# CMB-BNU/PloidyFrost

Hardware: AMD Instinct MI355X
Metric: unitigs/s through superbubble+SeqAlign (k=25, z=8) (higher is better)
Workload: dtype u64

## Files before the change

### include/ploidyfrost_hip.h

```cpp
#ifndef PLOIDYFROST_HIP_H_
#define PLOIDYFROST_HIP_H_

#include <stddef.h>
#include <stdint.h>

#ifdef __cplusplus
extern "C" {
#endif

#define PF_NONE 0xFFFFFFFFu

enum pf_status {
    PF_OK = 0,
    PF_ERR_ARG = 1,
    PF_ERR_HIP = 2,
    PF_ERR_NO_DEVICE = 3,
    PF_ERR_OVERFLOW = 4,
    PF_ERR_MISSING_KMER = 5
};

typedef struct pf_ctx pf_ctx;

int pf_create(int device, pf_ctx **out);
int pf_warmup(int device);
// ... 190 lines not shown
                                uint64_t bytes_used[2], pf_trim_stats trim_stats[2], pf_count_stats *stats, uint64_t *bad_record);
int pf_maskcount_fastq_trimmed(pf_ctx *, const char *text, uint64_t n_bytes, int final, const pf_trim_plan *plan, uint32_t low, uint32_t up,
                               uint64_t *bytes_used, pf_trim_stats *trim_stats, pf_maskcount_stats *stats, uint64_t *bad_record);
int pf_maskcount_fastq_pair_trimmed(pf_ctx *, const char *text1, uint64_t n1, const char *text2, uint64_t n2, int final, const pf_trim_plan *plan,
                                    uint32_t low, uint32_t up, uint64_t bytes_used[2], pf_trim_stats trim_stats[2], pf_maskcount_stats *stats,
                                    uint64_t *bad_record);
typedef struct pf_clip_stats {
    uint64_t reads_clipped[2];
    uint64_t reads_dropped[2];
    uint64_t bases_clipped[2];
    uint64_t candidates_scored[2];
} pf_clip_stats;
int pf_clip_begin(pf_ctx *, const char *bases, const uint32_t *adapter_off, const uint8_t *side, uint32_t n_adapters, uint32_t seed, uint32_t score);
int pf_clip_stats_get(pf_ctx *, pf_clip_stats *stats);
int pf_clip_last_ends(pf_ctx *, int file, uint32_t *clip_end, uint64_t n_records);
int pf_clip_end(pf_ctx *);
typedef struct pf_clip_pair_stats {
    uint64_t pairs_clipped;
    uint64_t pairs_dropped;
    uint64_t pairs_too_long;
    uint64_t candidates_scored;
    uint64_t bases_clipped[2];
} pf_clip_pair_stats;
int pf_clip_begin_pairs(pf_ctx *, const char *bases, const uint32_t *adapter_off, const uint8_t *side, uint32_t n_adapters ,
                        const char *prefix_bases, const uint32_t *prefix_off , uint32_t n_pairs,
                        uint32_t seed, uint32_t score, uint32_t pair_score, uint32_t pair_min, int keep_both);
int pf_clip_pair_stats_get(pf_ctx *, pf_clip_pair_stats *stats);
#define PF_QC_TABLE_WORDS 9515u
#define PF_QC_CLIP_WORDS 1025u
enum { PF_QC_RAW = 0, PF_QC_KEPT = 1 };
int pf_qc_begin(pf_ctx *, uint32_t phred);
int pf_qc_get(pf_ctx *, int side, int stage, uint64_t *words);
int pf_qc_clip_get(pf_ctx *, int side, uint64_t *words);
int pf_qc_fastq(pf_ctx *, int side, const char *text, uint64_t n_bytes, int final, uint64_t *bytes_used, uint64_t *n_records, uint64_t *bad_record);
int pf_qc_end(pf_ctx *);
typedef struct pf_inflate_stats {
    uint64_t members, bytes_in, bytes_out, blocks_stored, blocks_fixed, blocks_dynamic;
} pf_inflate_stats;
int pf_inflate_bgzf(pf_ctx *, const uint8_t *comp, uint64_t n_bytes, const uint64_t *member_off, uint64_t n_members,
                    char *out, uint64_t out_cap, uint64_t *out_bytes, pf_inflate_stats *stats, uint64_t *bad_member);

typedef struct pf_deflate_stats { uint64_t members, bytes_in, bytes_out, blocks_stored, blocks_fixed, blocks_dynamic, literals, matches; } pf_deflate_stats;
int pf_deflate_bgzf(pf_ctx *, const char *text, uint64_t n_bytes, uint32_t member_text, uint8_t *out, uint64_t out_cap,
                    uint64_t *out_bytes, uint64_t *member_off, pf_deflate_stats *stats);

typedef struct pf_gunzip_result {
    uint64_t out_bytes;
    uint64_t end_bit;
    uint32_t final;
    uint32_t n_window;
    uint32_t crc_raw;
    uint32_t clause;
    uint64_t clause_bit;
} pf_gunzip_result;
typedef struct pf_gunzip_stats {
    uint64_t pieces_found, pieces_live, pieces_dead, markers, blocks_stored, blocks_fixed, blocks_dynamic, bytes_in, bytes_out;
    double stage_ms[5];
} pf_gunzip_stats;
int pf_inflate_gzip(pf_ctx *, const uint8_t *comp, uint64_t n_bytes, uint64_t start_bit, const uint8_t *window, uint32_t n_window,
                    uint32_t piece_bytes, char *out, uint64_t out_cap, uint8_t *new_window, pf_gunzip_result *res, pf_gunzip_stats *stats);

typedef struct pf_hetpair_stats {
    uint64_t kmers;
    uint64_t in_range;
    uint64_t one_partner;
    uint64_t many_partners;
    uint64_t pairs;
} pf_hetpair_stats;
int pf_hetpairs(pf_ctx *, const uint64_t *kmers, const uint32_t *counts, uint64_t n, uint32_t k, uint32_t lo, uint32_t hi,
                uint64_t *table, uint64_t **pair_x_dev, uint64_t **pair_y_dev, uint32_t **cov_x_dev, uint32_t **cov_y_dev,
                uint64_t *n_pairs, pf_hetpair_stats *stats);
int pf_hetpair_table(pf_ctx *, const uint32_t *cov_x_dev, const uint32_t *cov_y_dev, uint64_t n_pairs, uint32_t lo, uint32_t hi, uint64_t *table);

int pf_copy_to_host(pf_ctx *, void *dst, const void *src_dev, size_t bytes);
int pf_device_alloc(pf_ctx *, size_t bytes, void **out);
int pf_copy(pf_ctx *, void *dst, const void *src, size_t bytes);

int pf_upload_counts(pf_ctx *, const uint64_t *kmers, const uint32_t *counts, uint64_t n, uint32_t k, uint64_t min_count,
                     uint64_t max_count, int both_strands);
int pf_release_counts(pf_ctx *);
int pf_join_counts(pf_ctx *);
int pf_join_counts_begin(pf_ctx *);
int pf_join_counts_end(pf_ctx *);
int pf_lookup_kmers(pf_ctx *, const uint64_t *kmers, uint64_t n, uint32_t *counts, uint8_t *found);

int pf_unitig_cov(pf_ctx *, uint32_t u0, uint32_t u1, uint64_t *sum, uint32_t *min, uint8_t *miss);
int pf_unitig_cov_probe(pf_ctx *, uint32_t u0, uint32_t u1, uint64_t *sum, uint32_t *min, uint8_t *miss);
int pf_unitig_cov_exact(pf_ctx *, uint32_t u0, uint32_t u1, int reverse, uint64_t *sum, uint32_t *min, uint8_t *miss);

typedef struct pf_bfs_record {
    uint32_t entrance;
    uint32_t exit;
    uint32_t n_seen;
    uint32_t n_list;
    uint64_t list_off;
    uint8_t outcome;
    uint8_t flag_cycle;
    uint8_t flag_tip;
    uint8_t strict;
    uint32_t pad_;
} pf_bfs_record;

enum pf_bfs_outcome {
    PF_BFS_NONE = 0,
    PF_BFS_CYCLE_EXIT = 1,
    PF_BFS_REJECT = 2,
    PF_BFS_ACCEPT = 3
};

int pf_count_candidates(pf_ctx *, uint32_t u0, uint32_t u1, uint64_t *n_candidates);
int pf_bfs_candidates(pf_ctx *, uint32_t u0, uint32_t u1, pf_bfs_record *records, uint64_t rec_cap,
                      uint32_t *pool, uint64_t pool_cap, uint64_t *n_records, uint64_t *pool_used);
int pf_bfs_candidates_split(pf_ctx *, uint32_t u0, uint32_t u1, pf_bfs_record *records, uint64_t rec_cap, uint32_t *pool,
                            uint64_t pool_cap, uint64_t *n_records, uint64_t *pool_used, uint32_t *deferred, uint64_t deferred_cap,
                            uint64_t *n_deferred);
int pf_bfs_candidates_begin(pf_ctx *, uint32_t u0, uint32_t u1, pf_bfs_record *records, uint64_t rec_cap, uint32_t *pool, uint64_t pool_cap,
                            uint64_t *n_records, uint64_t *pool_used, uint32_t *deferred, uint32_t *deferred_entrance, uint64_t deferred_cap,
                            uint64_t *n_deferred);
int pf_bfs_candidates_end(pf_ctx *);

typedef struct pf_align_job {
    uint64_t a_off, b_off;
    uint32_t a_len, b_len;
} pf_align_job;

typedef struct pf_align_hit {
    uint64_t text_off;
    uint64_t gap_off;
    uint32_t len;
    uint32_t n_gaps;
    int64_t score;
    uint32_t n_pos;
    uint32_t n_indel;
} pf_align_hit;

int pf_align_batch(pf_ctx *, const char *text, uint64_t text_len, const pf_align_job *jobs, uint32_t n_jobs,
                   double match, double mismatch, double gap, uint64_t *hit_first, uint32_t *hit_count,
                   pf_align_hit *hits, uint64_t hit_cap, char *out_text, uint64_t text_cap, uint32_t *out_gaps,
                   uint64_t gap_cap, uint64_t used[3]);

typedef struct pf_bubble_path {
    uint64_t text_off;
    uint32_t len;
    uint32_t ov;
} pf_bubble_path;

typedef struct pf_bubble_task {
    uint64_t path_first;
    uint32_t n_paths;
    uint32_t pad_;
} pf_bubble_task;

typedef struct pf_bubble_site {
    uint32_t col;
    uint8_t is_indel;
    uint8_t maxnum;
    uint16_t pad_;
} pf_bubble_site;

typedef struct pf_bubble_result {
    uint64_t rows_off;
    uint64_t site_off;
    uint64_t group_off;
    uint64_t ilen_off;
    uint32_t n_rows;
    uint32_t n_cols;
// ... 178 lines not shown
```

### ploidyfrost_amd/csrc/host/pf_cdbg.hpp

```cpp
#pragma once
#include <chrono>
#include <memory>
#include <condition_variable>
#include <mutex>

#include "pf_bfs_host.hpp"
#include <cstdint>
#include <memory>
#include <string>
#include <thread>
#include <utility>
#include <vector>

#include "pf_gmm_model.hpp"
#include "pf_host_colors.hpp"
#include "pf_host_graph.hpp"
#include "pf_pinned.hpp"
#include "pf_replay_par.hpp"
#include "pf_state.hpp"
#include "ploidyfrost_hip.h"

namespace pfh {

struct Scoring {
// ... 97 lines not shown
    bool model_was_each_color() const { return last_each_; }
    const std::vector<GmmModel::Fit> &model_fits() const { return model_fits_; }
    double model_ploidy() const { return model_ploidy_; }
    const std::string &model_last_line() const { return model_last_line_; }
    uint64_t model_count() const { return model_n_; }
    uint64_t text_bytes_fetched() const { return text_fetched_; }
    int find_shard(uint32_t u0, uint32_t u1);
    const std::vector<pf_bfs_record> &shard_records() const { return shard_rec_; }
    const std::vector<uint32_t> &shard_pool() const { return shard_pool_; }
    int find_replay(const std::string &outpre, uint32_t n_shards, const pf_bfs_record *const *records, const uint64_t *n_records,
                    const uint32_t *const *pools, bool write_file, const uint64_t *pool_lens = nullptr,
                    const pf_bfs_record *const *dev_records = nullptr, const uint32_t *const *dev_pools = nullptr);
    void set_replay_threads(int t) { replay_threads_ = t; }
    void set_write_super_bubble(bool on) { write_sb_ = on; }
    int ploidy_select(int lower, int upper, uint64_t &n_bubbles);
    int ploidy_select(const std::vector<std::pair<int, int>> &cutoff, uint64_t &n_bubbles);
    int ploidy_align(uint64_t t0, uint64_t t1, uint64_t &n_called);
    int ploidy_text(uint64_t var_count_base, uint64_t sizes[PF_CALL_STREAMS], uint64_t counters[8]);
    int ploidy_write(const std::string &outpre, const uint64_t offsets[PF_CALL_STREAMS], const uint64_t totals[PF_CALL_STREAMS], bool truncate);
    pf_ctx *device() { return ctx_; }
    const PhaseTimes &times() const { return times_; }
    uint64_t allele_sites(int arity) const { return allele_[arity - 2]; }
    uint64_t core_cov() const { return core_cov_; }
    uint64_t core_num() const { return core_num_; }
    uint64_t n_superbubbles() const { return n_super_bubble_; }
    const std::vector<uint8_t> &state_flags() { sync_state_to_host(); return flags_; }
    const std::vector<uint32_t> &state_plus() { sync_state_to_host(); return plus_; }
    const std::vector<uint32_t> &state_minus() { sync_state_to_host(); return minus_; }
    int sync_state_to_host();
    uint64_t output_bytes() const { return out_bytes_; }
    const std::string &last_allele_frequency() const;

protected:
    struct NoCounts {};
    CDBG(UnitigSet &graph, const size_t &complexsize, double &m, double &d, double &g, int device, bool quiet, NoCounts, pf_ctx *adopt = nullptr);
    int init_device(int device, pf_ctx *adopt = nullptr, bool colored = false);
    void start_prealloc();
    int ploidy_estimation(const std::string &outpre, const std::vector<std::pair<int, int>> &cutoff, const size_t &thr);
    int ploidy_estimation_resident(const std::string &outpre, const std::vector<std::pair<int, int>> &cutoff, const size_t &thr);
    int call_select(const std::vector<std::pair<int, int>> &cutoff, uint64_t &n_tasks);
    bool resident_path() const { return resident_ && (col_ == nullptr || colored_resident_); }
    const ColorSets *col_ = nullptr;
    const char *tag_ = "CDBG";

    struct Task;
    using clk_time = std::chrono::steady_clock::time_point;
    int finish_find(const std::string &outpre, const FindTrace &tr, bool write_file, bool timing_lines);
    std::vector<pf_bfs_record> shard_rec_;
    std::vector<uint32_t> shard_pool_;
    ModelOptions model_;
    unsigned density_points_ = 0;
    double density_adjust_ = 1.0;
    Density density_;
    bool density_done_ = false;
    std::vector<int> color_no_density_;
    bool filter_on_ = false;
    pf_filter_opts filter_ = {};
    bool multi_on_ = false, multi_each_ = false;
    pf_filter_multi_opts multi_ = {};
    std::vector<ColorFit> color_fits_;
    std::vector<int> color_none_, color_empty_;
    std::vector<double> pooled_values_;
    bool last_each_ = false;
    std::vector<GmmModel::Fit> model_fits_;
    double model_ploidy_ = 0;
    std::string model_last_line_;
    uint64_t model_n_ = 0, text_fetched_ = 0;
    pf_call_result slice_res_ = {};
    uint64_t slice_nb_ = 0, slice_var_base_ = 0;
    int fail(int st, const std::string &msg);
    int join_pending_write();
    int join_pending_ids();
    std::thread prealloc_, prealloc_walkers_, prealloc_call_, prealloc_align_;
    void join_prealloc() {
        if (prealloc_.joinable()) prealloc_.join();
        if (prealloc_walkers_.joinable()) prealloc_walkers_.join();
        if (prealloc_call_.joinable()) prealloc_call_.join();
        if (prealloc_align_.joinable()) prealloc_align_.join();
    }
    std::thread pending_ids_;
    int pending_ids_rc_ = 0;
    uint64_t ids_bytes_ = 0;
    int launch_coverage();
    uint64_t find_passes_ = 0;
    bool cov_ready_ = false;
    std::string cov_err_;
    bool overlap_output_ = false;
    std::thread pending_write_;
    int pending_rc_ = 0;
    int ensure_dir();
    int write_file(const std::string &name, const std::string &data);
    int write_pieces(const std::string &name, const std::vector<const std::string *> &pieces, uint64_t &bytes) const;
    int write_many(const std::vector<std::pair<std::string, std::vector<const std::string *>>> &files, unsigned threads);
    void replay(const pf_bfs_record &r, const uint32_t *list) { st_.replay(r, list); }

    UnitigSet &g_;
    size_t complex_size_;
    Scoring sc_;
    std::string outdir_ = "PloidyFrost_output";
    pf_ctx *ctx_ = nullptr;
    int status_ = 0;
    std::string err_;
    bool quiet_ = false, write_files_ = true;
    bool both_strands_ = true;
    unsigned threads_ = 0;
    int replay_threads_ = -1;
    bool write_sb_ = true;
    bool state_host_stale_ = false;
    bool colours_on_device_ = false;
    bool colored_resident_ = false;
    std::vector<uint8_t> big_f2_;
    bool commits_on_device() const;
    ParallelReplay par_;
    unsigned replay_threads(size_t thr) const;
    size_t host_threads(size_t thr) const;
    unsigned walk_threads(size_t thr) const;
    void set_record_stats(const ReplayStats &s);
    struct EarlyWalks; struct DeviceFind; struct SlicedFind;
    int find_superbubbles_device(const std::string &outpre, const size_t &thr);
    int traverse_resident(EarlyWalks &early, DeviceFind &df, const FindTrace &tr);
    void walk_remaining(EarlyWalks &early, DeviceFind &df, const FindTrace &tr, unsigned threads);
    void walked_into_candidate_order(DeviceFind &df);
    int commit_large_on_host(DeviceFind &df, const FindTrace &tr, unsigned threads);
    int patch_device_state(const std::vector<uint32_t> &sides, const FindTrace &tr, unsigned threads);
    void traverse_slices(SlicedFind &sf, const FindTrace &tr);
    int traverse_slice(SlicedFind &sf, int i, const FindTrace &tr);
    void walk_long(const FindTrace &tr, bool say_start, uint32_t entrance, pf_bfs_record &r, std::vector<uint32_t> &out);
    template <class Call> int with_deferred(uint64_t &n_deferred, Call call);
    template <class ListOf> void replay_sequential(const pf_bfs_record *rec, uint64_t n, ListOf list_of, ReplayStats &stats);
    bool third_tier_on_host_ = true;
    WalkerPool walkers_;
    std::vector<uint32_t> deferred_;
    std::vector<uint32_t> deferred_ent_;
    std::vector<std::vector<uint32_t>> huge_lists_[4];

    std::vector<uint32_t> succ_, pred_;
    UnitigState st_;
    std::vector<uint8_t> &flags_ = st_.flags;
    std::vector<uint32_t> &plus_ = st_.plus, &minus_ = st_.minus;

    struct AlignExchange {
        PinnedBuf<char> text, otext;
        PinnedBuf<pf_bubble_path> paths;
        PinnedBuf<pf_bubble_task> tasks;
        PinnedBuf<pf_bubble_result> res;
        PinnedBuf<pf_bubble_site> osites;
        PinnedBuf<uint8_t> ogroups;
        PinnedBuf<uint32_t> oilen;
        void release_all() {
            text.release(); otext.release(); paths.release(); tasks.release(); res.release(); osites.release();
            ogroups.release(); oilen.release();
        }
    } ax_[3];
    size_t batch_bubbles_ = 32768, align_pieces_ = 64;
    struct BubbleExchange {
        PinnedBuf<pf_bfs_record> bfs_rec;
        PinnedBuf<uint32_t> bfs_pool;
        PinnedBuf<uint32_t> bfs_order;
        PinnedBuf<uint64_t> cov_sum;
        PinnedBuf<uint32_t> cov_min;
        PinnedBuf<uint8_t> cov_miss;
        PinnedBuf<uint32_t> cov_max;
        void release_all() {
            cov_max.release();
            bfs_rec.release(); bfs_pool.release(); bfs_order.release(); cov_sum.release(); cov_min.release();
            cov_miss.release();
// ... 65 lines not shown
```

### ploidyfrost_amd/csrc/host/pf_cdbg_call.cpp

```cpp
#include <fcntl.h>
#include <sys/stat.h>
#include <unistd.h>

#include <algorithm>
#include <atomic>
#include <condition_variable>
#include <cstdio>
#include <cstring>
#include <ctime>
#include <deque>
#include <memory>
#include <mutex>
#include <sstream>
#include <thread>

#include "../pf_alnpack.hpp"
#include "../pf_nibble.hpp"
#include "pf_cdbg_impl.hpp"
#include "pf_parallel.hpp"

namespace pfh {

namespace {
const char *kStreamSuffix[PF_CALL_STREAMS] = {"_allele_frequency.txt", "_alignseq.txt", "_bifre.txt",    "_trifre.txt",   "_tetrafre.txt",
// ... 136 lines not shown
    std::vector<pf_call_result> pres((size_t)n_pieces);
    uint64_t running[PF_CALL_STREAMS];
    for (int s = 0; s < PF_CALL_STREAMS; ++s) running[s] = offsets[s];
    last_allfre_.clear();
    last_allfre_file_.clear();
    int st = PF_OK;
    auto format = [&](uint64_t i) {
        const uint64_t first = i * CHUNK, count = std::min<uint64_t>(CHUNK, slice_nb_ - first);
        return pf_call_text_range_lane(ctx_, 0, (int)(i % PF_CALL_SLABS), first, count, slice_var_base_, &pres[(size_t)i]);
    };
    auto piece_bytes = [&](uint64_t i) {
        uint64_t all = 0;
        for (int s = 0; s < PF_CALL_STREAMS; ++s) all += pres[(size_t)i].text_len[s];
        return all;
    };
    auto fetch = [&](uint64_t i) {
        PinnedBuf<char> &hb = cx_.slab[i & 1];
        const uint64_t all = piece_bytes(i);
        hb.ensure(ctx_, std::max<uint64_t>(all, 1));
        return pf_call_fetch_range(ctx_, (int)(i % PF_CALL_SLABS), 0, hb.p, all, (int)(i & 1));
    };
    if (n_pieces) st = format(0);
    if (st == PF_OK && n_pieces) st = fetch(0);
    for (uint64_t i = 0; i < n_pieces && st == PF_OK; ++i) {
        if (i + 1 < n_pieces) st = format(i + 1);
        if (st == PF_OK) st = pf_call_fetch_wait(ctx_, (int)(i & 1));
        if (st == PF_OK && i + 1 < n_pieces) st = fetch(i + 1);
        if (st != PF_OK) break;
        const pf_call_result &r = pres[(size_t)i];
        const char *src = cx_.slab[i & 1].p;
        CopySpan spans[PF_CALL_STREAMS];
        size_t n_spans = 0;
        uint64_t at = 0;
        for (int s = 0; s < PF_CALL_STREAMS; ++s) {
            const uint64_t len = r.text_len[s];
            if (len) {
                char *dst = maps[s].prepare(running[s], len);
                if (dst) spans[n_spans++] = CopySpan{dst, src + at, len};
                else rc |= maps[s].write(running[s], src + at, len, T);
            }
            if (s == 0) last_allfre_.append(src + at, len);
            running[s] += len;
            at += len;
            out_bytes_ += len;
        }
        copy_spans(spans, n_spans, T);
    }
    if (st != PF_OK) return fail(st, std::string(tag_) + "::PloidyEstimation(): " + pf_last_error(ctx_));
    for (int s = 0; s < PF_CALL_STREAMS; ++s)
        if (running[s] - offsets[s] != (slice_nb_ ? slice_res_.text_len[s] : 0)) return fail(PF_ERR_ARG, std::string(tag_) + "::PloidyEstimation(): the pieces of a slice do not add up to its size");
    times_.write_s = since(t);
    if (rc) return fail(PF_ERR_ARG, "CDBG:: write error on the result files");
    return 0;
}

int CDBG::ploidy_estimation_resident(const std::string &outpre, const std::vector<std::pair<int, int>> &cutoff, const size_t &thr) {
    const auto t_all = clk::now();
    clock_t c0 = clock();
    if (!quiet_) printf("%s::PloidyEstimation():  Analyzing superbubbles to generate sites' information\n", tag_);
    if (write_files_ && ensure_dir()) return status_;
    if (model_.on && ((col_ && !multi_on_) || !write_files_))
        return fail(PF_ERR_ARG, std::string(tag_) + "::PloidyEstimation(): the model in the same run needs the single-sample path (the colored one: a multi filter in front of it, set_filter_multi) and an output directory");
    const bool write_ten = write_files_ && !model_.only;
    model_fits_.clear();
    model_last_line_.clear();
    model_ploidy_ = 0;
    model_n_ = 0;
    color_fits_.clear();
    color_none_.clear();
    color_empty_.clear();
    color_no_density_.clear();
    density_done_ = false;
    pooled_values_.clear();
    last_each_ = false;
    const uint64_t fetched_before = pf_call_fetched_bytes(ctx_);
    const unsigned T = threads_ ? threads_ : (unsigned)std::max<size_t>(thr, 1);
    times_.cov_device_s = times_.tasks_s = times_.align_s = times_.sites_s = times_.format_s = times_.write_s = 0;
    times_.tasks = times_.align_jobs = times_.site_strings = 0;
    times_.snp_jobs = times_.pair_jobs = times_.wave_jobs = times_.stack_jobs = 0;
    times_.align_build_s = times_.align_device_s = times_.align_post_s = times_.align_choose_s = times_.scan_s = 0;
    allele_[0] = allele_[1] = allele_[2] = allele_[3] = 0;
    core_cov_ = core_num_ = 0;
    const bool trace = getenv("PF_TRACE_PLOIDY") != nullptr;
    auto tp = [&](const char *what) { if (trace) fprintf(stderr, "[ploidy] %-28s %.2f ms\n", what, since(t_all) * 1e3); };

    struct OutFile {
        std::string name;
        uint64_t bytes = 0;
        int rc = 0;
    };
    std::vector<OutFile> files(PF_CALL_STREAMS);
    for (int s = 0; s < PF_CALL_STREAMS; ++s) files[(size_t)s].name = outpre + kStreamSuffix[s];
    MappedOut *maps = out_maps_.get();
    int open_failed = -1;
    std::thread opener;
    if (write_ten)
        opener = std::thread([&] {
            for (size_t i = 0; i < files.size(); ++i)
                if (maps[i].open_for(outdir_ + "/" + files[i].name)) { open_failed = (int)i; return; }
        });
    struct OpenerGuard {
        std::thread &t;
        ~OpenerGuard() { if (t.joinable()) t.join(); }
    } opener_guard{opener};

    uint64_t n_tasks = 0;
    if (call_select(cutoff, n_tasks)) return status_;
    tp("scan + selection done");
    if (opener.joinable()) opener.join();
    if (open_failed >= 0) return fail(PF_ERR_ARG, "CDBG:: Open " + files[(size_t)open_failed].name + " file error");
    last_allfre_.clear();
    last_allfre_file_.clear();
    std::thread prefault0;
    std::atomic<bool> prefault0_stop{false};
    struct Prefault0Guard {
        std::thread &t;
        std::atomic<bool> &stop;
        ~Prefault0Guard() { stop.store(true); if (t.joinable()) t.join(); }
    } prefault0_guard{prefault0, prefault0_stop};
    if (write_ten && n_tasks) {
        const double nbub = 1.1 * (double)n_tasks;
        const double per_bubble[PF_CALL_STREAMS] = {20, 2.0 * (2 * g_.k + 26), 20, 0.5, 0.25, 0, 34, 0.75, 0.25, 0};
        std::vector<std::pair<int, uint64_t>> fresh;
        for (int s = 0; s < PF_CALL_STREAMS; ++s) {
            const uint64_t est = (uint64_t)(per_bubble[s] * nbub);
            if (est >= (1u << 20) && maps[s].reserve(est) == 0) fresh.push_back({s, est});
        }
        if (!fresh.empty())
            prefault0 = std::thread([maps, fresh, T, &prefault0_stop] {
                constexpr uint64_t STEP = 4u << 20;
                std::vector<std::pair<int, uint64_t>> spans;
                uint64_t longest = 0;
                for (auto &f : fresh) longest = std::max(longest, f.second);
                for (uint64_t at = 0; at < longest; at += STEP)
                    for (auto &f : fresh)
                        if (at < f.second) spans.push_back({f.first, at});
                parallel_chunks(spans.size(), 1, std::max(2u, T), [&](size_t i, size_t, size_t) {
                    if (prefault0_stop.load(std::memory_order_relaxed)) return;
                    const int s = spans[i].first;
                    uint64_t end = spans[i].second + STEP;
                    for (auto &f : fresh) if (f.first == s) end = std::min(end, f.second);
                    maps[s].populate(spans[i].second, end);
                });
            });
    }

    const bool aln_packed = !getenv("PF_ALIGNSEQ_ASCII");
    if (pf_call_set_alignseq_packed(ctx_, aln_packed ? 1 : 0) != PF_OK) return fail(PF_ERR_HIP, std::string(tag_) + "::PloidyEstimation(): " + pf_last_error(ctx_));
    const bool num_packed = !getenv("PF_NUMERIC_ASCII");
    if (pf_call_set_numeric_packed(ctx_, num_packed ? 1 : 0) != PF_OK) return fail(PF_ERR_HIP, std::string(tag_) + "::PloidyEstimation(): " + pf_last_error(ctx_));
    if (model_.on && (pf_call_model_begin(ctx_, model_.source, model_.q) != PF_OK || (filter_on_ && pf_call_model_filter(ctx_, &filter_) != PF_OK) ||
                      (multi_on_ && pf_call_model_filter_multi(ctx_, &multi_, multi_each_ ? 1 : 0) != PF_OK)))
        return fail(PF_ERR_ARG, std::string(tag_) + "::PloidyEstimation(): " + pf_last_error(ctx_));
    struct PackGuard {
        pf_ctx *c;
        ~PackGuard() { (void)pf_call_set_alignseq_packed(c, 0); (void)pf_call_set_numeric_packed(c, 0); }
    } pack_guard{ctx_};
    auto slab_len = [](const pf_call_result &r, int s) -> uint64_t {
        const uint64_t aln = (s == PF_OUT_ALIGNSEQ && r.alignseq_packed_len) ? r.alignseq_packed_len : r.text_len[s];
        if (!r.numeric_packed) return aln;
        return s == PF_OUT_ALIGNSEQ ? ((aln + 15) & ~15ull) : PF_NUMERIC_PACKED_LEN(r.text_len[s]);
    };

    const size_t batch_env = [] { const char *e = getenv("PF_BATCH_BUBBLES"); return e ? (size_t)std::max(1, atoi(e)) : (size_t)0; }();
    const size_t batch_now = batch_env ? batch_env : batch_bubbles_;
    const size_t CHUNK = std::min<size_t>(std::max<size_t>(batch_now ? batch_now * 4 : 1, 1), (size_t)1 << 24);
    struct Done {
// ... 470 lines not shown
```

### ploidyfrost_amd/csrc/host/pf_cdbg_find.cpp

```cpp
#include <algorithm>
#include <atomic>
#include <condition_variable>
#include <cstdio>
#include <cstring>
#include <mutex>
#include <stdexcept>
#include <thread>
#include <unordered_map>

#include "pf_cdbg_impl.hpp"
#include "pf_parallel.hpp"

namespace pfh {

size_t CDBG::host_threads(size_t thr) const { return threads_ ? threads_ : std::max<size_t>(thr, 1); }
unsigned CDBG::walk_threads(size_t thr) const {
    return (unsigned)std::max<uint64_t>(1, std::min<uint64_t>(host_threads(thr), (4ull << 30) / (4ull * std::max<uint32_t>(g_.n(), 1))));
}

unsigned CDBG::replay_threads(size_t thr) const {
    if (col_ != nullptr) return 0;
    static const char *env = getenv("PF_REPLAY");
    if (env && !strcmp(env, "seq")) return 0;
    static const int env_t = [] { const char *e = getenv("PF_REPLAY_THREADS"); return e ? atoi(e) : -1; }();
// ... 157 lines not shown
    }
    df.walked.swap(w2);
    std::copy(d2.begin(), d2.end(), deferred_.begin());
}

int CDBG::commit_large_on_host(DeviceFind &df, const FindTrace &tr, unsigned threads) {
    const uint32_t N = g_.n();
    const size_t n_big = (size_t)df.n_big, n_walked = (size_t)df.n_deferred;
    std::vector<uint32_t> big_idx(n_big);
    std::vector<pf_bfs_record> big_rec(n_big);
    std::vector<uint32_t> big_pool((size_t)df.big_entries + 1);
    const int st = pf_replay_big_fetch(ctx_, big_idx.data(), big_rec.data(), big_pool.data());
    if (st != PF_OK) return st;
    tr.step("large components fetched");
    if (big_f2_.size() != 2 * (size_t)N) big_f2_.assign(2 * (size_t)N, 0);
    if (!state_host_stale_)
        parallel_chunks(N, 1u << 19, threads, [&](size_t, size_t b, size_t e) {
            memset(plus_.data() + b, 0, (e - b) * 4);
            memset(minus_.data() + b, 0, (e - b) * 4);
        });
    const FlagsPerSideLogged acc{FlagsPerSide{big_f2_.data(), plus_.data(), minus_.data()}, &df.p_sides};
    Commits<FlagsPerSideLogged> cm{acc, complex_size_, NoColours{}};
    Commits<FlagsPerSideLogged, ColourGate> cmc{acc, complex_size_, col_ ? st_.colour_gate() : ColourGate{}};
    ReplayStats stats;
    auto commit = [&](const pf_bfs_record &r, const uint32_t *list) {
        const bool effective = record_effective(r) && cm.gate_open(r.entrance);
        stats.note(r, effective);
        if (effective) { if (col_) cmc.replay(r, list); else cm.replay(r, list); }
        return effective;
    };
    double t[2] = {0, 0};
    uint64_t eff[2] = {0, 0}, ent[2] = {0, 0};
    size_t a = 0, b = 0;
    while (a < n_big || b < n_walked) {
        const bool w = a >= n_big || (b < n_walked && deferred_[b] < big_idx[a]);
        const auto tc = tr.find ? clk::now() : clk::time_point();
        const pf_bfs_record &r = w ? df.walked[b++] : big_rec[a++];
        if (commit(r, (w ? df.xpool.data() : big_pool.data()) + r.list_off)) { ent[w] += r.n_list; ++eff[w]; }
        if (tr.find) t[w] += since(tc);
    }
    set_record_stats(stats);
    if (tr.find)
        fprintf(stderr, "[find]   replayed here: %zu walked records (%llu take effect, %llu list entries) %.3f ms, %llu records of large components (%llu, %llu) %.3f ms\n",
                n_walked, (unsigned long long)eff[1], (unsigned long long)ent[1], t[1] * 1e3, (unsigned long long)df.n_big, (unsigned long long)eff[0], (unsigned long long)ent[0], t[0] * 1e3);
    tr.step("large components replayed");
    return PF_OK;
}

int CDBG::patch_device_state(const std::vector<uint32_t> &sides, const FindTrace &tr, unsigned threads) {
    std::vector<uint32_t> links(sides.size());
    std::vector<uint8_t> bytes(sides.size());
    parallel_chunks(sides.size(), 1u << 14, threads, [&](size_t, size_t b, size_t e) {
        for (size_t i = b; i < e; ++i) {
            const uint32_t s = sides[i];
            links[i] = (s & 1) ? minus_[s >> 1] : plus_[s >> 1];
            bytes[i] = big_f2_[s];
        }
    });
    tr.step("patch gathered");
    std::thread undo([&] {
        parallel_chunks(sides.size(), 1u << 14, threads, [&](size_t, size_t b, size_t e) {
            for (size_t i = b; i < e; ++i) {
                const uint32_t s = sides[i];
                __atomic_store_n(&((s & 1) ? minus_ : plus_)[s >> 1], 0u, __ATOMIC_RELAXED);
                __atomic_store_n(&big_f2_[s], (uint8_t)0, __ATOMIC_RELAXED);
            }
        });
    });
    const int st = pf_replay_finish(ctx_, sides.data(), links.data(), bytes.data(), sides.size());
    undo.join();
    return st;
}

int CDBG::find_superbubbles_device(const std::string &outpre, const size_t &thr) {
    const FindTrace tr;
    auto failed = [&](int st) { return fail(st, std::string("CDBG::findSuperBubble(): ") + pf_last_error(ctx_)); };
    out_bytes_ = 0;
    state_on_device_ = false;
    cov_ready_ = false;
    for (auto &hl : huge_lists_) hl.clear();
    const unsigned wt = walk_threads(thr), few = (unsigned)std::min<size_t>(host_threads(thr), 8);
    DeviceFind df;
    EarlyWalks early(*this, tr, wt);
    int st = traverse_resident(early, df, tr);
    if (st != PF_OK) return failed(st);
    tr.step("traversed on the device");
    df.walked.resize((size_t)df.n_deferred);
    df.lists.resize((size_t)df.n_deferred);
    std::string walk_err;
    std::thread walk([&] { try { walk_remaining(early, df, tr, wt); } catch (const std::exception &e) { walk_err = e.what(); } });
    st = pf_side_components(ctx_, 1, nullptr, df.n_rec, nullptr, 0, nullptr, 0, nullptr, 0);
    tr.step("  components of the device's records");
    if (st == PF_OK && overlap_output_) cov_ready_ = launch_coverage() == PF_OK;
    tr.step("  coverage launched");
    walk.join();
    if (!walk_err.empty()) return fail(PF_ERR_HIP, "CDBG::findSuperBubble(): walk of a long traversal: " + walk_err);
    if (st != PF_OK) return failed(st);
    tr.step("long traversals walked");
    walked_into_candidate_order(df);
    tr.step("  walked records in candidate order");
    if (!df.walked.empty()) st = pf_side_components(ctx_, 0, nullptr, df.n_rec, nullptr, 0, df.walked.data(), df.walked.size(), df.xpool.data(), df.xpool.size());
    tr.step("  their components");
    static const uint32_t small_limit = [] { const char *e = getenv("PF_REPLAY_SMALL_LIMIT"); return e ? (uint32_t)atoi(e) : 256u; }();
    if (st == PF_OK) st = pf_replay_device(ctx_, (uint32_t)std::min<size_t>(complex_size_, 0xFFFFFFFFu), small_limit, &df.n_big, &df.big_entries);
    if (st != PF_OK) return failed(st);
    tr.step("components + commits on the device");
    st = commit_large_on_host(df, tr, few);
    if (st != PF_OK) return failed(st);
    st = patch_device_state(df.p_sides, tr, few);
    if (st != PF_OK) return failed(st);
    if (tr.find) fprintf(stderr, "[find] %zu sides patched on the device %.2f ms\n", df.p_sides.size(), since(tr.t_all) * 1e3);
    state_host_stale_ = true;
    state_on_device_ = true;
    tr.step("large components committed here");
    times_.bfs_device_s = since(tr.t_all);
    times_.candidates = df.n_rec;
    times_.bfs_deferred = df.n_deferred;
    times_.host_commit_records = df.n_big + df.n_deferred;
    times_.host_walk_vertices = 0;
    for (const auto &w : df.walked) times_.host_walk_vertices += w.n_seen;
    times_.replay_s = 0;
    return finish_find(outpre, tr, write_sb_, true);
}

struct CDBG::SlicedFind {
    static constexpr int kMaxSlices = 4;
    int n_slices = 1;
    unsigned rt = 0, walk_threads = 1;
    uint32_t u0[kMaxSlices + 1];
    uint64_t rec0[kMaxSlices + 1], pool0[kMaxSlices + 1], n_rec[kMaxSlices], used[kMaxSlices];
    uint32_t class_off[kMaxSlices][kReplayClasses + 1];
    std::unique_ptr<PinnedBuf<uint32_t>> own_pool[kMaxSlices];
    const uint32_t *pool[kMaxSlices];
    std::mutex mu; std::condition_variable cv;
    int done = 0, dev_st = PF_OK;
    std::string dev_err;
    double bfs_s = 0;
    uint64_t n_deferred_total = 0;
};

int CDBG::traverse_slice(SlicedFind &sf, int i, const FindTrace &tr) {
    const auto tb = clk::now();
    pf_bfs_record *rec = bx_.bfs_rec.p + sf.rec0[i];
    const uint64_t rec_cap = sf.rec0[i + 1] - sf.rec0[i];
    uint32_t *pl = bx_.bfs_pool.p + sf.pool0[i];
    uint64_t cap = sf.pool0[i + 1] - sf.pool0[i];
    uint64_t n_deferred = 0;
    int st1;
    for (;;) {
        if (third_tier_on_host_)
            st1 = with_deferred(n_deferred, [&] {
                return pf_bfs_candidates_begin(ctx_, sf.u0[i], sf.u0[i + 1], rec, rec_cap, pl, cap, &sf.n_rec[i], &sf.used[i], deferred_.data(), deferred_ent_.data(), deferred_.size(), &n_deferred);
            });
        else
            st1 = pf_bfs_candidates(ctx_, sf.u0[i], sf.u0[i + 1], rec, rec_cap, pl, cap, &sf.n_rec[i], &sf.used[i]);
        if (st1 != PF_ERR_OVERFLOW || sf.used[i] <= cap) break;
        sf.own_pool[i] = std::make_unique<PinnedBuf<uint32_t>>();
        sf.own_pool[i]->ensure(ctx_, sf.used[i] + sf.used[i] / 8);
        pl = sf.own_pool[i]->p;
        cap = sf.own_pool[i]->cap;
    }
    sf.pool[i] = pl;
    sf.n_deferred_total += n_deferred;
    if (tr.bfs) fprintf(stderr, "[bfs] device tiers of slice %d: %.2f ms, %llu candidates left for the third tier\n", i, since(tb) * 1e3, (unsigned long long)n_deferred);
    std::vector<pf_bfs_record> walked((size_t)n_deferred);
    std::string walk_err;
    std::thread walk;
    if (st1 == PF_OK && n_deferred) {
        huge_lists_[i].assign((size_t)n_deferred, std::vector<uint32_t>());
        walk = std::thread([&] {
            try {
                parallel_chunks((size_t)n_deferred, 1, sf.walk_threads, [&](size_t d, size_t, size_t) {
                    walk_long(tr, false, deferred_ent_[d], walked[d], huge_lists_[i][d]);
                    walked[d].list_off = d; walked[d].pad_ = 1;
                });
            } catch (const std::exception &e) { walk_err = e.what(); }
        });
    }
    if (st1 == PF_OK && sf.rt) st1 = pf_side_components(ctx_, i == 0, nullptr, sf.n_rec[i], nullptr, 0, nullptr, 0, nullptr, 0);
    if (walk.joinable()) walk.join();
    if (!walk_err.empty()) throw std::runtime_error("walk of a long traversal: " + walk_err);
    if (third_tier_on_host_) {
        const int ste = pf_bfs_candidates_end(ctx_);
        if (st1 == PF_OK) st1 = ste;
    }
    if (st1 == PF_OK)
        for (uint64_t d = 0; d < n_deferred; ++d) rec[deferred_[d]] = walked[(size_t)d];
    const auto t_cc = clk::now();
    if (tr.find) fprintf(stderr, "[find]   slice %d traversed (%llu records, %llu walked on host cores) %.2f ms (+%.2f)\n", i, (unsigned long long)sf.n_rec[i],
                         (unsigned long long)n_deferred, since(tr.t_all) * 1e3, since(tb) * 1e3);
    if (st1 == PF_OK && sf.rt) {
        std::vector<pf_bfs_record> xrec;
        std::vector<uint32_t> xpool;
        for (uint64_t d = 0; d < n_deferred; ++d) {
            pf_bfs_record r = rec[deferred_[d]];
            const std::vector<uint32_t> &l = huge_lists_[i][(size_t)d];
            r.list_off = xpool.size();
// ... 206 lines not shown
    return 0;
}

int CDBG::find_replay(const std::string &outpre, uint32_t n_shards, const pf_bfs_record *const *records, const uint64_t *n_records,
                      const uint32_t *const *pools, bool write_file, const uint64_t *pool_lens, const pf_bfs_record *const *dev_records,
                      const uint32_t *const *dev_pools) {
    if (status_) return status_;
    if (join_pending_write()) return status_;
    if (write_file && write_files_ && ensure_dir()) return status_;
    const FindTrace tr;
    out_bytes_ = 0;
    state_on_device_ = false;
    state_host_stale_ = false;
    std::fill(flags_.begin(), flags_.end(), 0);
    std::fill(plus_.begin(), plus_.end(), 0);
    std::fill(minus_.begin(), minus_.end(), 0);
    cov_ready_ = false;
    ReplayStats stats;
    set_record_stats(stats);
    const auto t0 = clk::now();
    uint64_t total = 0;
    uint32_t last = 0;
    const unsigned rt = pool_lens ? replay_threads(1) : 0;
    if (rt) par_.begin(g_.n(), plus_.data(), minus_.data(), complex_size_, rt);
    std::vector<uint32_t> order;
    std::vector<const pf_bfs_record *> h_rec(n_shards);
    std::vector<const uint32_t *> h_pool(n_shards);
    {
        uint64_t need_rec = 0, need_pool = 0;
        for (uint32_t sh = 0; sh < n_shards; ++sh) {
            h_rec[sh] = records ? records[sh] : nullptr;
            h_pool[sh] = pools ? pools[sh] : nullptr;
            if (!h_rec[sh] || !h_pool[sh]) {
                if (!pool_lens || !dev_records || !dev_pools || !dev_records[sh] || !dev_pools[sh])
                    return fail(PF_ERR_ARG, "CDBG::find_replay(): a shard has neither host nor device arrays");
                need_rec += n_records[sh];
                need_pool += pool_lens[sh];
            }
        }
        if (need_rec) {
            bx_.bfs_rec.ensure(ctx_, need_rec + 1);
            bx_.bfs_pool.ensure(ctx_, need_pool + 1);
            uint64_t ar = 0, ap = 0;
            for (uint32_t sh = 0; sh < n_shards; ++sh) {
                if (h_rec[sh] && h_pool[sh]) continue;
                int st = pf_fetch(ctx_, bx_.bfs_rec.p + ar, dev_records[sh], n_records[sh] * sizeof(pf_bfs_record));
                if (st == PF_OK) st = pf_fetch(ctx_, bx_.bfs_pool.p + ap, dev_pools[sh], pool_lens[sh] * 4);
                if (st != PF_OK) return fail(st, std::string("CDBG::find_replay(): ") + pf_last_error(ctx_));
                h_rec[sh] = bx_.bfs_rec.p + ar;
                h_pool[sh] = bx_.bfs_pool.p + ap;
                ar += n_records[sh];
                ap += pool_lens[sh];
            }
        }
    }
    for (uint32_t sh = 0; sh < n_shards; ++sh) {
        const pf_bfs_record *rec = h_rec[sh];
        const uint32_t *pool = h_pool[sh];
        const uint64_t n = n_records[sh];
        total += n;
        for (uint64_t i = 0; i < n; ++i) {
            const pf_bfs_record &r = rec[i];
            if ((r.entrance >> 1) >= g_.n() || r.entrance < last) return fail(PF_ERR_ARG, "CDBG::find_replay(): records out of order");
            last = r.entrance;
        }
        auto list_of = [&](const pf_bfs_record &r) { return pool + r.list_off; };
        if (!rt) { replay_sequential(rec, n, list_of, stats); continue; }
        const bool on_dev = dev_records && dev_pools && dev_records[sh] && dev_pools[sh];
        int st = pf_side_components(ctx_, sh == 0, on_dev ? dev_records[sh] : rec, n, on_dev ? dev_pools[sh] : pool, pool_lens[sh], nullptr, 0, nullptr, 0);
        uint32_t class_off[kReplayClasses + 1];
        order.resize(std::max<uint64_t>(n, 1));
        if (st == PF_OK) st = pf_replay_order(ctx_, kReplayClasses, order.data(), class_off, nullptr);
        if (st != PF_OK) return fail(st, std::string("CDBG::find_replay(): ") + pf_last_error(ctx_));
        par_.run(rec, list_of, order.data(), class_off, kReplayClasses, rt, stats);
    }
    if (rt) par_.finish(flags_.data(), rt);
    stats.large_used = stats.large_used_max = 0;
    set_record_stats(stats);
    times_.replay_s = since(t0);
    times_.candidates = total;
    return finish_find(outpre, tr, write_file, false);
}

int CDBG::launch_coverage() {
    if (resident_path()) {
        const int st = pf_call_coverage(ctx_);
        if (st != PF_OK) cov_err_ = pf_last_error(ctx_);
        return st;
    }
    const uint32_t N = g_.n();
    const uint32_t C = col_ ? col_->n_colors : (both_strands_ ? 1 : 2);
    bx_.cov_sum.ensure(ctx_, (size_t)N * C);
    bx_.cov_min.ensure(ctx_, (size_t)N * C);
    bx_.cov_miss.ensure(ctx_, (size_t)N * C);
    if (col_) bx_.cov_max.ensure(ctx_, (size_t)N * C);
    int st;
    if (col_) st = pf_unitig_cov_colored(ctx_, 0, N, bx_.cov_sum.p, bx_.cov_min.p, bx_.cov_max.p, bx_.cov_miss.p);
    else if (both_strands_) st = pf_unitig_cov(ctx_, 0, N, bx_.cov_sum.p, bx_.cov_min.p, bx_.cov_miss.p);
    else {
        st = pf_unitig_cov_exact(ctx_, 0, N, 0, bx_.cov_sum.p, bx_.cov_min.p, bx_.cov_miss.p);
        if (st == PF_OK || st == PF_ERR_MISSING_KMER) st = pf_unitig_cov_exact(ctx_, 0, N, 1, bx_.cov_sum.p + N, bx_.cov_min.p + N, bx_.cov_miss.p + N);
    }
    if (st != PF_OK && st != PF_ERR_MISSING_KMER) { cov_err_ = pf_last_error(ctx_); return st; }
    return PF_OK;
}

}
```

### ploidyfrost_amd/csrc/pf_bfs.hip

```cpp
#include <hip/hip_runtime.h>

#include <algorithm>
#include <cstring>

#include "pf_bfs.hpp"
#include "pf_bfs_huge.hpp"
#include "pf_ctx.hpp"

using namespace pf;


constexpr uint32_t BFS_LDS_CAP = 128;
constexpr uint32_t BFS_BIG_CAP = 1u << 12;

struct BfsOut {
    pf_bfs_record *rec;
    uint32_t *pool;
    uint64_t pool_cap;
    unsigned long long *pool_head;
    uint32_t *deferred;
    unsigned int *n_deferred;
    uint32_t *deferred2;
    unsigned int *n_deferred2;
    unsigned long long *live;
// ... 220 lines not shown
    pf_bfs_record *records; uint64_t rec_cap;
    uint32_t *pool; uint64_t pool_cap;
    uint64_t *n_records, *pool_used;
    uint32_t *deferred, *deferred_entrance; uint64_t deferred_cap, *n_deferred;
};

struct BfsCounters {
    unsigned long long pool_head;
    unsigned int n_deferred;
    unsigned int n_deferred2;
    unsigned int n_wave_list;
    unsigned int n_live;
};

struct BfsPlan {
    uint64_t c0, c1, n;
    BfsOut o;
    BfsCounters *d_cnt; uint32_t *d_wlist;
};

void cand_range(const pf_ctx *ctx, uint32_t u0, uint32_t u1, uint64_t *c0, uint64_t *c1) {
    const auto &v = ctx->h_cand;
    *c0 = std::lower_bound(v.begin(), v.end(), u0 * 2) - v.begin();
    *c1 = std::lower_bound(v.begin(), v.end(), u1 * 2) - v.begin();
}

uint32_t env_hint_at() { const char *e = getenv("PF_BFS_HINT_AT"); return e ? (uint32_t)std::max(9, atoi(e)) : 48u; }
uint32_t env_wave_cap() { const char *e = getenv("PF_BFS_WAVE_CAP"); return e ? (uint32_t)std::max(16, std::min((int)BFS_LDS_CAP, atoi(e))) : BFS_LDS_CAP; }

int want_host_records(pf_ctx *ctx, const void *records, const char *entry_point) {
    if (!ctx || !is_device_ptr(records)) return PF_OK;
    pf::CtxErr{ctx} = std::string(entry_point) + " fills host records";
    return PF_ERR_ARG;
}

void mark_deferred(const pf_ctx *ctx, pf_bfs_record *records, uint64_t c0, const uint32_t *deferred, uint64_t n_deferred) {
    for (uint64_t d = 0; d < n_deferred; ++d) {
        pf_bfs_record &r = records[deferred[d]];
        memset(&r, 0, sizeof r);
        r.entrance = ctx->h_cand[c0 + deferred[d]];
        r.exit = NONE;
    }
}

int bfs_plan(pf_ctx *ctx, const BfsRequest &q, BfsPlan &p) {
    cand_range(ctx, q.u0, q.u1, &p.c0, &p.c1);
    const uint64_t n = p.n = p.c1 - p.c0;
    *q.n_records = n; *q.pool_used = 0;
    if (n > q.rec_cap) { pf::CtxErr{ctx} = "record buffer too small"; return PF_ERR_OVERFLOW; }
    if (n == 0) return PF_OK;
    pf_bfs_record *d_rec = q.records; uint32_t *d_pool = q.pool;
    if (q.mode.deliver != Deliver::ON_DEVICE) {
        d_rec = (pf_bfs_record *)ctx_ws(ctx, WS_BFS_REC, n * sizeof(pf_bfs_record));
        d_pool = (uint32_t *)ctx_ws(ctx, WS_BFS_POOL, (q.pool_cap ? q.pool_cap : 1) * 4);
    }
    BfsCounters *c = p.d_cnt = (BfsCounters *)ctx_ws(ctx, WS_BFS_SMALL, sizeof(BfsCounters));
    uint32_t *d_def = (uint32_t *)ctx_ws(ctx, WS_BFS_DEF, (n * 2 + 8) * 4);
    p.d_wlist = (uint32_t *)ctx_ws(ctx, WS_BFS_WLIST, (n + 8) * 4);
    if (!d_rec || !d_pool || !c || !d_def || !p.d_wlist) return PF_ERR_HIP;
    PF_HIP(hipMemsetAsync(c, 0, sizeof(BfsCounters), ctx->stream));
    p.o = BfsOut{d_rec, d_pool, q.pool_cap, &c->pool_head, d_def, &c->n_deferred, d_def + n + 4, &c->n_deferred2, nullptr, 0, &c->n_live, 0};
    return PF_OK;
}

void bfs_arm_live(pf_ctx *ctx, const BfsRequest &q, BfsPlan &p) {
    ctx->bfs_live_n = 0;
    if (!ctx->h_live || q.mode.long_walks != LongWalks::BY_CALLER) return;
    p.o.live = ctx->h_live; p.o.live_cap = (uint32_t)ctx->live_cap; p.o.hint_at = env_hint_at();
}

int bfs_read_counters(pf_ctx *ctx, const BfsPlan &p, BfsCounters &cnt) {
    PF_HIP(hipMemcpyAsync(&cnt, p.d_cnt, sizeof cnt, hipMemcpyDeviceToHost, ctx->stream));
    PF_HIP(hipStreamSynchronize(ctx->stream));
    return PF_OK;
}

int bfs_short_tiers(pf_ctx *ctx, const BfsPlan &p, BfsCounters &cnt) {
    ctx_begin(ctx, PF_K_BFS_THREAD);
    k_bfs_thread<<<(unsigned)((p.n + 255) / 256), 256, 0, ctx->stream>>>(ctx->d_succ, ctx->d_pred, ctx->d_cand, p.c0, p.c1, p.o, p.d_wlist, &p.d_cnt->n_wave_list);
    ctx_end(ctx);
    ctx_begin(ctx, PF_K_BFS);
    k_bfs<<<ctx_grid(ctx, (p.n / 4 + 64) * 64, 256, 8), 256, 0, ctx->stream>>>(ctx->d_succ, ctx->d_pred, ctx->d_cand, p.c0, p.c1, p.o, p.d_wlist, &p.d_cnt->n_wave_list, env_wave_cap());
    ctx_end(ctx);
    if (const int st = bfs_read_counters(ctx, p, cnt)) return st;
    ctx->bfs_live_n = cnt.n_live;
    ctx_units(ctx, PF_K_BFS, cnt.n_wave_list);
    ctx_units(ctx, PF_K_BFS_THREAD, p.n);
    return PF_OK;
}

int bfs_long_tiers(pf_ctx *ctx, const BfsPlan &p, BfsCounters &cnt) {
    const unsigned int waves = std::min<unsigned int>(cnt.n_deferred, 256);
    DevTmp<uint32_t> sc32; DevTmp<uint8_t> sc8;
    PF_HIP(sc32.alloc((size_t)waves * 3 * BFS_BIG_CAP * 4));
    PF_HIP(sc8.alloc((size_t)waves * BFS_BIG_CAP));
    ctx_begin(ctx, PF_K_BFS_BIG);
    k_bfs_big<<<waves, 64, 0, ctx->stream>>>(ctx->d_succ, ctx->d_pred, ctx->d_cand, p.c0, cnt.n_deferred, sc32.p, sc8.p, p.o);
    ctx_end(ctx);
    const int st = bfs_read_counters(ctx, p, cnt);
    if (st != PF_OK || cnt.n_deferred2 == 0) return st;
    const unsigned int hw = (unsigned int)std::max<size_t>(1, std::min<size_t>(std::min<size_t>(cnt.n_deferred2, 64), (16ull << 30) / (36 * (size_t)ctx->N + 64)));
    const size_t per = 9 * (size_t)ctx->N + 16;
    DevTmp<uint32_t> hs;
    PF_HIP(hs.alloc(per * hw * 4));
    PF_HIP(hipMemsetAsync(hs.p, 0, per * hw * 4, ctx->stream));
    ctx_begin(ctx, PF_K_BFS_BIG);
    if (!ctx->d_pred16) {
        PF_HIP(hipMalloc(&ctx->d_pred16, (size_t)ctx->N * 2 * 16 * 4));
        k_pred16<<<ctx_grid(ctx, (uint64_t)ctx->N * 8, 256, 8), 256, 0, ctx->stream>>>(ctx->d_succ, ctx->d_pred, ctx->N * 2, ctx->d_pred16);
    }
    k_bfs_huge<<<hw, 64, 0, ctx->stream>>>(ctx->d_succ, ctx->d_pred16, ctx->d_cand, p.c0, cnt.n_deferred2, hs.p, ctx->N, p.o);
    ctx_end(ctx);
    return bfs_read_counters(ctx, p, cnt);
}

void bfs_publish(pf_ctx *ctx, const BfsRequest &q, const BfsPlan &p) {
    ctx->bfs_last_rec = p.o.rec; ctx->bfs_last_pool = p.o.pool; ctx->bfs_last_n = p.n; ctx->bfs_last_pool_len = q.pool_cap;
    ctx->bfs_call_id++;
}

int bfs_deliver(pf_ctx *ctx, const BfsRequest &q, const BfsPlan &p, uint64_t pool_used) {
    const uint64_t n_deferred = q.n_deferred ? *q.n_deferred : 0;
    const size_t rec_bytes = p.n * sizeof(pf_bfs_record), pool_bytes = (size_t)pool_used * 4;
    if (q.mode.deliver == Deliver::TO_HOST) {
        PF_HIP(hipMemcpy(q.records, p.o.rec, rec_bytes, hipMemcpyDeviceToHost));
        PF_HIP(hipMemcpy(q.pool, p.o.pool, pool_bytes, hipMemcpyDeviceToHost));
        mark_deferred(ctx, q.records, p.c0, q.deferred, n_deferred);
        if (std::any_of(q.records, q.records + p.n, [](const pf_bfs_record &r) { return r.outcome == BFS_TOO_LARGE; })) {
            pf::CtxErr{ctx} = "a traversal exceeded the direct-indexed tier (internal limit)";
            return PF_ERR_OVERFLOW;
        }
    } else if (q.mode.deliver == Deliver::TO_HOST_ASYNC) {
        if (!ctx->copy_stream) PF_HIP(hipStreamCreateWithFlags(&ctx->copy_stream, hipStreamNonBlocking));
        PF_HIP(hipMemcpyAsync(q.records, p.o.rec, rec_bytes, hipMemcpyDeviceToHost, ctx->copy_stream));
        PF_HIP(hipMemcpyAsync(q.pool, p.o.pool, pool_bytes, hipMemcpyDeviceToHost, ctx->copy_stream));
        ctx->bfs_pending.active = true; ctx->bfs_pending.records = q.records; ctx->bfs_pending.c0 = p.c0;
        ctx->bfs_pending.deferred.assign(q.deferred, q.deferred + n_deferred);
    }
    if (q.deferred_entrance) for (uint64_t d = 0; d < n_deferred; ++d) q.deferred_entrance[d] = ctx->h_cand[p.c0 + q.deferred[d]];
    return PF_OK;
}

int bfs_run(pf_ctx *ctx, const BfsRequest &q) {
    if (!ctx || !ctx->has_adj || q.u0 > q.u1 || q.u1 > ctx->N || !q.records || !q.pool || !q.n_records || !q.pool_used) return PF_ERR_ARG;
    if (ctx->bfs_pending.active) { pf::CtxErr{ctx} = "pf_bfs_candidates_end first"; return PF_ERR_ARG; }
    if (q.n_deferred) *q.n_deferred = 0;
    PF_HIP(hipSetDevice(ctx->device));
    BfsPlan p; BfsCounters cnt;
    int st = bfs_plan(ctx, q, p), status = PF_OK;
    if (st != PF_OK || p.n == 0) return st;
    bfs_arm_live(ctx, q, p);
    if ((st = bfs_short_tiers(ctx, p, cnt)) != PF_OK) return st;
    if (cnt.n_deferred && q.mode.long_walks == LongWalks::BY_CALLER) {
        *q.n_deferred = cnt.n_deferred;
        if (cnt.n_deferred > q.deferred_cap) { pf::CtxErr{ctx} = "deferred-candidate buffer too small"; status = PF_ERR_OVERFLOW; }
        else PF_HIP(hipMemcpy(q.deferred, p.o.deferred, (size_t)cnt.n_deferred * 4, hipMemcpyDeviceToHost));
    } else if (cnt.n_deferred) {
        if ((st = bfs_long_tiers(ctx, p, cnt)) != PF_OK) return st;
    }
    bfs_publish(ctx, q, p);
    *q.pool_used = cnt.pool_head;
    if (cnt.pool_head > q.pool_cap) { pf::CtxErr{ctx} = "vertex pool too small"; status = PF_ERR_OVERFLOW; }
    return status == PF_OK ? bfs_deliver(ctx, q, p, cnt.pool_head) : status;
}

}

extern "C" {

int pf_count_candidates(pf_ctx *ctx, uint32_t u0, uint32_t u1, uint64_t *n) {
    if (!ctx || !ctx->has_adj || u0 > u1 || u1 > ctx->N || !n) return PF_ERR_ARG;
    uint64_t c0, c1;
    cand_range(ctx, u0, u1, &c0, &c1);
    *n = c1 - c0;
    return PF_OK;
}

int pf_bfs_candidates(pf_ctx *ctx, uint32_t u0, uint32_t u1, pf_bfs_record *records, uint64_t rec_cap, uint32_t *pool,
                      uint64_t pool_cap, uint64_t *n_records, uint64_t *pool_used) {
    return bfs_run(ctx, {{is_device_ptr(records) ? Deliver::ON_DEVICE : Deliver::TO_HOST, LongWalks::ON_DEVICE}, u0, u1, records, rec_cap, pool, pool_cap,
                         n_records, pool_used, nullptr, nullptr, 0, nullptr});
}

int pf_bfs_candidates_split(pf_ctx *ctx, uint32_t u0, uint32_t u1, pf_bfs_record *records, uint64_t rec_cap, uint32_t *pool,
                            uint64_t pool_cap, uint64_t *n_records, uint64_t *pool_used, uint32_t *deferred, uint64_t deferred_cap,
                            uint64_t *n_deferred) {
    if (!deferred || !n_deferred) return PF_ERR_ARG;
    if (want_host_records(ctx, records, "pf_bfs_candidates_split")) return PF_ERR_ARG;
    return bfs_run(ctx, {{Deliver::TO_HOST, LongWalks::BY_CALLER}, u0, u1, records, rec_cap, pool, pool_cap, n_records, pool_used,
                         deferred, nullptr, deferred_cap, n_deferred});
}

int pf_bfs_candidates_begin(pf_ctx *ctx, uint32_t u0, uint32_t u1, pf_bfs_record *records, uint64_t rec_cap, uint32_t *pool,
                            uint64_t pool_cap, uint64_t *n_records, uint64_t *pool_used, uint32_t *deferred, uint32_t *deferred_entrance,
                            uint64_t deferred_cap, uint64_t *n_deferred) {
    if (!deferred || !deferred_entrance || !n_deferred) return PF_ERR_ARG;
    if (want_host_records(ctx, records, "pf_bfs_candidates_begin")) return PF_ERR_ARG;
    return bfs_run(ctx, {{Deliver::TO_HOST_ASYNC, LongWalks::BY_CALLER}, u0, u1, records, rec_cap, pool, pool_cap, n_records, pool_used,
                         deferred, deferred_entrance, deferred_cap, n_deferred});
}

int pf_bfs_candidates_end(pf_ctx *ctx) {
    if (!ctx) return PF_ERR_ARG;
    auto &pending = ctx->bfs_pending;
    if (!pending.active) return PF_OK;
    pending.active = false;
    PF_HIP(hipSetDevice(ctx->device));
    PF_HIP(hipStreamSynchronize(ctx->copy_stream));
    mark_deferred(ctx, pending.records, pending.c0, pending.deferred.data(), pending.deferred.size());
    return PF_OK;
}

int pf_bfs_candidates_resident(pf_ctx *ctx, uint32_t u0, uint32_t u1, uint64_t *n_records, uint64_t *pool_used, uint32_t *deferred,
                               uint32_t *deferred_entrance, uint64_t deferred_cap, uint64_t *n_deferred) {
    if (!ctx || !n_records || !pool_used || !deferred || !deferred_entrance || !n_deferred || !ctx->has_adj || u0 > u1 || u1 > ctx->N) return PF_ERR_ARG;
    uint64_t c0, c1;
    cand_range(ctx, u0, u1, &c0, &c1);
    const uint64_t n = c1 - c0;
    uint64_t cap = std::max<uint64_t>(ctx->bfs_res_pool_cap, n * 6 + (1u << 20));
    for (int attempt = 0; attempt < 4; ++attempt) {
        pf_bfs_record *d_rec = (pf_bfs_record *)ctx_ws(ctx, WS_BFS_RES_REC, (n + 1) * sizeof(pf_bfs_record));
        uint32_t *d_pool = (uint32_t *)ctx_ws(ctx, WS_BFS_RES_POOL, (cap + 1) * 4);
        if (!d_rec || !d_pool) return PF_ERR_HIP;
        const int st = bfs_run(ctx, {{Deliver::ON_DEVICE, LongWalks::BY_CALLER}, u0, u1, d_rec, n + 1, d_pool, cap, n_records, pool_used,
                                     deferred, deferred_entrance, deferred_cap, n_deferred});
        if (st == PF_ERR_OVERFLOW && *pool_used > cap) { cap = *pool_used + *pool_used / 8 + 1024; continue; }
        if (st == PF_OK) ctx->bfs_res_pool_cap = cap;
        return st;
    }
    pf::CtxErr{ctx} = "pf_bfs_candidates_resident: the vertex pool does not converge";
    return PF_ERR_OVERFLOW;
}

// ... 26 lines not shown
```

### ploidyfrost_amd/csrc/pf_call.hip

```cpp
#include "pf_call_kernels.hpp"
#include "pf_scan.hpp"

using namespace pf;

#define PF_TRY(call) do { const int s_ = (call); if (s_ != PF_OK) return s_; } while (0)

using namespace pf_call;

struct Need { DevBuf *buf; size_t bytes; };
static int need(pf_ctx *ctx, const char *who, std::initializer_list<Need> list) {
    for (const Need &n : list)
        if (!n.buf->ensure(n.bytes)) { pf::CtxErr{ctx} = std::string(who) + ": out of device memory"; return PF_ERR_HIP; }
    return PF_OK;
}

namespace pf {

void call_state_create(pf_ctx *ctx) { (void)state_of(ctx); }
void call_destroy(pf_ctx *ctx) {
    if (!ctx->call) return;
    ctx->call->release_all();
    delete ctx->call;
    ctx->call = nullptr;
}
// ... 182 lines not shown
    }
    PF_HIP(hipSetDevice(ctx->device));
    CallState *S = ctx->call;
    PF_HIP(hipMemcpyAsync(S->col_low.p, lower, (size_t)n_colors * 4, hipMemcpyDefault, ctx->stream));
    PF_HIP(hipMemcpyAsync(S->col_up.p, upper, (size_t)n_colors * 4, hipMemcpyDefault, ctx->stream));
    PF_HIP(hipStreamSynchronize(ctx->stream));
    return PF_OK;
}

int pf_call_coverage(pf_ctx *ctx) {
    if (ctx && ctx->call && ctx->call->n_colors) {
        if (!ctx->d_seq || !ctx->d_ctab) { pf::CtxErr{ctx} = "pf_call_coverage: graph and count tables first"; return PF_ERR_ARG; }
        PF_HIP(hipSetDevice(ctx->device));
        CallState *S = ctx->call;
        const size_t n = (size_t)ctx->N * S->n_colors;
        if (!S->ccov_sum.ensure(n * 8) || !S->ccov_min.ensure(n * 4) || !S->ccov_max.ensure(n * 4) || !S->ccov_miss.ensure(n)) {
            pf::CtxErr{ctx} = "pf_call_coverage: out of device memory";
            return PF_ERR_HIP;
        }
        const int st = pf_unitig_cov_colored(ctx, 0, ctx->N, S->ccov_sum.as<uint64_t>(), S->ccov_min.as<uint32_t>(), S->ccov_max.as<uint32_t>(), S->ccov_miss.as<uint8_t>());
        if (st != PF_OK) return st;
        S->per_strand = false;
        S->have_cov = true;
        return PF_OK;
    }
    if (!ctx || !ctx->d_seq || !ctx->d_tab) { if (ctx) pf::CtxErr{ctx} = "pf_call_coverage: graph and count table first"; return PF_ERR_ARG; }
    PF_HIP(hipSetDevice(ctx->device));
    CallState *S = state_of(ctx);
    const size_t N = ctx->N;
    const int slots = ctx->tab_exact ? 2 : 1;
    if (!S->cov_sum.ensure(N * slots * 8) || !S->cov_min.ensure(N * slots * 4) || !S->cov_miss.ensure(N * slots)) {
        pf::CtxErr{ctx} = "pf_call_coverage: out of device memory";
        return PF_ERR_HIP;
    }
    int st;
    if (!ctx->tab_exact) {
        st = pf_unitig_cov(ctx, 0, (uint32_t)N, S->cov_sum.as<uint64_t>(), S->cov_min.as<uint32_t>(), S->cov_miss.as<uint8_t>());
    } else {
        st = pf_unitig_cov_exact(ctx, 0, (uint32_t)N, 0, S->cov_sum.as<uint64_t>(), S->cov_min.as<uint32_t>(), S->cov_miss.as<uint8_t>());
        if (st == PF_OK || st == PF_ERR_MISSING_KMER)
            st = pf_unitig_cov_exact(ctx, 0, (uint32_t)N, 1, S->cov_sum.as<uint64_t>() + N, S->cov_min.as<uint32_t>() + N, S->cov_miss.as<uint8_t>() + N);
    }
    if (st != PF_OK && st != PF_ERR_MISSING_KMER) return st;
    S->per_strand = ctx->tab_exact;
    S->have_cov = true;
    return PF_OK;
}

int pf_call_scan(pf_ctx *ctx, uint32_t lower, uint32_t upper, uint64_t *n_sides) {
    if (!ctx || !n_sides) return PF_ERR_ARG;
    CallState *S = ctx->call;
    if (!S || !S->have_state || !S->have_cov) { pf::CtxErr{ctx} = "pf_call_scan: pf_call_set_state and pf_call_coverage first"; return PF_ERR_ARG; }
    PF_HIP(hipSetDevice(ctx->device));
    hipStream_t st = ctx->stream;
    const uint32_t N = ctx->N;
    if (!S->side_cnt.ensure(((size_t)N + 1) * 4) || !S->side_base.ensure(((size_t)N + 1) * 4)) { pf::CtxErr{ctx} = "pf_call_scan: out of device memory"; return PF_ERR_HIP; }
    k_call_count_sides<<<(N + 1 + 255) / 256, 256, 0, st>>>(S->flags.as<uint8_t>(), N, S->side_cnt.as<uint32_t>());
    if (!S->scan_tmp.ensure(scan_scratch_bytes((uint64_t)N + 1))) { pf::CtxErr{ctx} = "pf_call_scan: out of device memory"; return PF_ERR_HIP; }
    PF_HIP(scan_exclusive_u32(S->side_cnt.as<uint32_t>(), S->side_base.as<uint32_t>(), (uint64_t)N + 1, S->scan_tmp.p, st));
    uint32_t total = 0;
    PF_HIP(hipMemcpyAsync(&total, S->side_base.as<uint32_t>() + N, 4, hipMemcpyDeviceToHost, st));
    PF_HIP(hipStreamSynchronize(st));
    S->n_sides = total;
    S->n_tasks = 0;
    S->low = lower;
    S->up = upper;
    *n_sides = total;
    if (total == 0) return PF_OK;
    if (!S->sides.ensure((size_t)total * sizeof(pf_call_side)) || !S->ctask.ensure((size_t)total * sizeof(CallTask)) ||
        !S->target.ensure((size_t)total * 4)) {
        pf::CtxErr{ctx} = "pf_call_scan: out of device memory";
        return PF_ERR_HIP;
    }
    ScanArgs a;
    a.flags = S->flags.as<uint8_t>(); a.plus = S->plus.as<uint32_t>(); a.minus = S->minus.as<uint32_t>();
    a.succ = ctx->d_succ; a.pred = ctx->d_pred; a.seq = ctx->d_seq; a.off = ctx->d_off; a.len = ctx->d_len; a.N = N; a.k = ctx->k;
    a.cov_sum = S->cov_sum.as<uint64_t>(); a.cov_min = S->cov_min.as<uint32_t>(); a.cov_miss = S->cov_miss.as<uint8_t>();
    a.per_strand = S->per_strand; a.low = lower; a.up = upper;
    a.side_base = S->side_base.as<uint32_t>(); a.sides = S->sides.as<pf_call_side>(); a.tasks = S->ctask.as<CallTask>();
    a.target = S->target.as<uint32_t>();
    a.n_colors = S->n_colors;
    a.ccov_sum = S->ccov_sum.as<uint64_t>(); a.ccov_min = S->ccov_min.as<uint32_t>(); a.ccov_max = S->ccov_max.as<uint32_t>(); a.ccov_miss = S->ccov_miss.as<uint8_t>();
    a.clow = S->col_low.as<uint32_t>(); a.cup = S->col_up.as<uint32_t>(); a.full = S->col_full.as<uint64_t>(); a.cwords = S->col_words; a.size_total = S->col_size.as<uint64_t>();
    ctx_begin(ctx, PF_K_CALL_SCAN);
    if (S->n_colors) k_call_sides<true><<<(N + 255) / 256, 256, 0, st>>>(a);
    else k_call_sides<false><<<(N + 255) / 256, 256, 0, st>>>(a);
    ctx_end(ctx);
    ctx_units(ctx, PF_K_CALL_SCAN, N);
    PF_HIP(hipGetLastError());
    return PF_OK;
}

int pf_call_resolve(pf_ctx *ctx, uint64_t *n_bubbles, uint32_t *err, uint32_t *err_unitig) {
    if (!ctx || !ctx->call || !n_bubbles || !err || !err_unitig) return PF_ERR_ARG;
    CallState *S = ctx->call;
    *n_bubbles = 0;
    *err = 0;
    *err_unitig = 0;
    S->n_tasks = 0;
    const uint64_t n = S->n_sides;
    if (n == 0) return PF_OK;
    PF_HIP(hipSetDevice(ctx->device));
    hipStream_t st = ctx->stream;
    if (!S->pending.ensure(n * 4) || !S->killed.ensure(n) || !S->rstate.ensure(n) || !S->rflag.ensure(n * 4) || !S->rsmall.ensure(64) ||
        !S->kept.ensure(n * 4)) {
        pf::CtxErr{ctx} = "pf_call_resolve: out of device memory";
        return PF_ERR_HIP;
    }
    PF_HIP(hipMemsetAsync(S->pending.p, 0, n * 4, st));
    PF_HIP(hipMemsetAsync(S->killed.p, 0, n, st));
    PF_HIP(hipMemsetAsync(S->rstate.p, 0, n, st));
    unsigned int *small = S->rsmall.as<unsigned int>();
    ResolveArgs a;
    a.sides = S->sides.as<pf_call_side>(); a.target = S->target.as<uint32_t>(); a.n = (uint32_t)n; a.pending = S->pending.as<int>();
    a.killed = S->killed.as<uint8_t>(); a.state = S->rstate.as<uint8_t>(); a.flag = S->rflag.as<uint32_t>();
    a.undecided = small; a.first_err = small + 1;
    const unsigned int init[3] = {0, 0xFFFFFFFFu, 0};
    PF_HIP(hipMemcpyAsync(small, init, 12, hipMemcpyHostToDevice, st));
    const unsigned grid = (unsigned)((n + 255) / 256);
    k_call_pending<<<grid, 256, 0, st>>>(a);
    for (uint64_t round = 0;; ++round) {
        if (round > n + 2) { pf::CtxErr{ctx} = "pf_call_resolve: the driver pass does not settle"; return PF_ERR_ARG; }
        k_call_resolve<<<grid, 256, 0, st>>>(a);
        PF_HIP(hipMemsetAsync(small, 0, 4, st));
        k_call_resolve<<<grid, 256, 0, st>>>(a);
        unsigned int h[2];
        PF_HIP(hipMemcpyAsync(h, small, 8, hipMemcpyDeviceToHost, st));
        PF_HIP(hipStreamSynchronize(st));
        if (h[1] != 0xFFFFFFFFu && h[0] == 0) {
            pf_call_side bad;
            PF_HIP(hipMemcpy(&bad, S->sides.as<pf_call_side>() + h[1], sizeof(bad), hipMemcpyDeviceToHost));
            *err = bad.err;
            *err_unitig = bad.err_unitig;
            return PF_OK;
        }
        if (h[0] == 0) break;
    }
    if (!S->scan_tmp.ensure(scan_scratch_bytes(n))) { pf::CtxErr{ctx} = "pf_call_resolve: out of device memory"; return PF_ERR_HIP; }
    PF_HIP(select_flagged_u32(S->rflag.as<uint32_t>(), S->kept.as<uint32_t>(), small + 2, nullptr, n, S->scan_tmp.p, st));
    unsigned int sel = 0;
    PF_HIP(hipMemcpyAsync(&sel, small + 2, 4, hipMemcpyDeviceToHost, st));
    PF_HIP(hipStreamSynchronize(st));
    S->n_tasks = sel;
    *n_bubbles = sel;
    return PF_OK;
}

int pf_call_sides(pf_ctx *ctx, pf_call_side *out, uint64_t cap) {
    if (!ctx || !ctx->call) return PF_ERR_ARG;
    CallState *S = ctx->call;
    if (cap < S->n_sides || (S->n_sides && !out)) return PF_ERR_OVERFLOW;
    if (S->n_sides == 0) return PF_OK;
    PF_HIP(hipSetDevice(ctx->device));
    PF_HIP(hipMemcpyAsync(out, S->sides.p, (size_t)S->n_sides * sizeof(pf_call_side), hipMemcpyDefault, ctx->stream));
    PF_HIP(hipStreamSynchronize(ctx->stream));
    return PF_OK;
}

int pf_call_select(pf_ctx *ctx, const uint32_t *side_index, uint64_t n_tasks) {
    if (!ctx || !ctx->call || (n_tasks && !side_index)) return PF_ERR_ARG;
    CallState *S = ctx->call;
    if (n_tasks > S->n_sides) { pf::CtxErr{ctx} = "pf_call_select: more bubbles than open sides"; return PF_ERR_ARG; }
    PF_HIP(hipSetDevice(ctx->device));
    if (!S->kept.ensure(std::max<size_t>(n_tasks, 1) * 4)) { pf::CtxErr{ctx} = "pf_call_select: out of device memory"; return PF_ERR_HIP; }
    if (n_tasks) PF_HIP(hipMemcpyAsync(S->kept.p, side_index, (size_t)n_tasks * 4, hipMemcpyDefault, ctx->stream));
    PF_HIP(hipStreamSynchronize(ctx->stream));
// ... 818 lines not shown
```

### ploidyfrost_amd/csrc/pf_colored.hip

```cpp
#include <hip/hip_runtime.h>

#include <algorithm>
#include <cstdlib>
#include <cstring>
#include <string>
#include <vector>

#include "pf_colored_dev.hpp"
#include "pf_cov_stream.hpp"
#include "pf_ctx.hpp"
#include "pf_device_common.hpp"
#include "ploidyfrost_hip.h"

using namespace pf;

namespace {

constexpr uint32_t MISSING = pf::CTAB_MISSING;

__global__ void k_ctab_build(uint8_t *base, uint64_t mask, uint32_t line_bytes, int k, const uint64_t *__restrict__ kmers,
                             const uint32_t *__restrict__ counts, uint64_t n, uint64_t min_count, uint64_t max_count, uint32_t colour,
                             unsigned int *noncanon) {
    uint64_t i = (uint64_t)blockIdx.x * blockDim.x + threadIdx.x;
    const uint64_t stride = (uint64_t)gridDim.x * blockDim.x;
// ... 204 lines not shown
            bool open;
            const int at = line_slot(s4_keys, s4_first, open);
            s5_miss = at < 0;
            s5_fwd = s4_fwd;
            const uint32_t *cnt = ctab_counts(t, s4_line, at < 0 ? 0 : at);
#pragma unroll
            for (int c = 0; c < JOINC_MAX; ++c) s5_val[c] = (uint32_t)c < n_colors ? cnt[LINE_KEYS * c] : 0;
        }
        {
            uint64_t x = s3_w0 << s3_s;
            x |= s3_s ? s3_w1 >> (64 - s3_s) : 0;
            const uint64_t fwd = x >> (64 - 2 * k);
            const uint64_t rc = rc_kmer(fwd, k);
            const LineSeq sq = kmer_lines(fwd, rc, k, t.mask);
            s4_first = rc < fwd ? rc : fwd;
            s4_fwd = fwd;
            s4_line = sq.line;
            s4_keys = ctab_keys(t, sq.line);
        }
        {
            uint64_t g = row_of(it - 1) * 64 + lane;
            g = g < n_kmers ? g : n_kmers - 1;
            const uint32_t p = (uint32_t)(g - s2_pre);
            const uint64_t *w = seq + s2_wo + (p >> 5);
            s3_s = (int)(p & 31) * 2;
            s3_w0 = w[0];
            s3_w1 = w[1];
        }
        {
            const uint64_t r = row_of(it);
            uint64_t hd = s1_hd & below;
            hd &= r == n_rows - 1 ? (2ull << ((n_kmers - 1) & 63)) - 1 : ~0ull;
            const uint32_t u = s1_kr + (uint32_t)__popcll(hd);
            s2_pre = kpre[u];
            s2_wo = off[u];
        }
        {
            s1_hd = s0_hd;
            s1_kr = s0_kr;
            const uint64_t r = row_of(it + 2);
            s0_hd = khead[r];
            s0_kr = krow[r];
        }
    }
    if (lane == 0) rest_n[wave] = n_rest;
}

__global__ __launch_bounds__(256) void k_cov_join_colored_rest(CTab t, int k, uint32_t n_colors, const JoinRestC *__restrict__ rest,
                                                               const uint32_t *__restrict__ rest_n, uint32_t rest_cap, uint32_t *__restrict__ gcov,
                                                               uint64_t g_stride, const uint64_t *__restrict__ seq, const uint64_t *__restrict__ off,
                                                               const uint64_t *__restrict__ kpre, const uint64_t *__restrict__ khead,
                                                               const uint32_t *__restrict__ krow, uint64_t n_kmers, uint32_t rows_per_wave) {
    const uint64_t wave = ((uint64_t)blockIdx.x * blockDim.x + threadIdx.x) >> 6;
    const int lane = lane_id();
    const uint32_t n = rest_n[wave];
    auto look_up = [&](uint64_t g, uint64_t fwd) {
        for (uint32_t c0 = 0; c0 < n_colors; c0 += CPP) {
            const uint32_t n_here = min((uint32_t)CPP, n_colors - c0);
            uint32_t cnt[CPP];
            colored_counts(t, fwd, k, true, c0, n_here, cnt);
#pragma unroll
            for (int j = 0; j < CPP; ++j)
                if ((uint32_t)j < n_here) gcov[(uint64_t)(c0 + j) * g_stride + g] = cnt[j];
        }
    };
    if (n > rest_cap) {
        const uint64_t n_rows = (n_kmers + 63) >> 6;
        const uint64_t below = lane == 63 ? ~1ull : (((2ull << lane) - 1) & ~1ull);
        for (uint64_t r = wave * rows_per_wave; r < (wave + 1) * rows_per_wave && r < n_rows; ++r) {
            const uint64_t g = r * 64 + lane;
            if (g >= n_kmers) break;
            const uint32_t u = krow[r] + (uint32_t)__popcll(khead[r] & below);
            look_up(g, kmer_at(seq + off[u], (uint32_t)(g - kpre[u]), k));
        }
        return;
    }
    const JoinRestC *mine = rest + wave * (rest_cap + 1);
    for (uint32_t e = lane; e < n; e += WAVE) look_up(mine[e].g, mine[e].fwd);
}

}

namespace pf {
int join_graph_counts_colored_begin(pf_ctx *ctx) {
    ctx->gcov_c_valid = false;
    ctx->join_c_inflight = false;
    if (!ctx->d_seq || !ctx->d_ctab || !ctx->n_colors || !ctx->d_kpre || ctx->n_kmers == 0 || ctx->ctab_max_count >= MISSING) return PF_OK;
    PF_HIP(hipSetDevice(ctx->device));
    const uint64_t stride = (ctx->n_krow + 4) * 64;
    if (!ctx->d_gcov_c || ctx->gcov_c_stride != stride) {
        if (ctx->d_gcov_c) { (void)hipFree(ctx->d_gcov_c); ctx->d_gcov_c = nullptr; }
        if (hipMalloc(reinterpret_cast<void **>(&ctx->d_gcov_c), stride * ctx->n_colors * sizeof(uint32_t)) != hipSuccess) {
            (void)hipGetLastError();
            ctx->d_gcov_c = nullptr;
            return PF_OK;
        }
        ctx->gcov_c_stride = stride;
    }
    const CTab t{ctx->d_ctab, ctx->ctab_cap - 1, ctx->ctab_line_bytes};
    if (!ctx->join_c_done) PF_HIP(hipEventCreateWithFlags(&ctx->join_c_done, hipEventDisableTiming));
    const hipStream_t st = join_stream(ctx);
    size_t at = 0;
    if (ctx->ctab_one_strand && ctx->n_colors <= (uint32_t)JOINC_MAX && ctx->ctab_unread == 0) {
        constexpr uint32_t ROWS = 64;
        const uint64_t n_rows = (ctx->n_kmers + 63) / 64;
        const uint64_t n_waves = ((n_rows + ROWS - 1) / ROWS + 3) / 4 * 4;
        const int blocks = (int)(n_waves / 4);
        const uint32_t rest_cap = ROWS * 64 / 2;
        JoinRestC *rest = (JoinRestC *)ctx_ws(ctx, WS_JOIN_REST, n_waves * (rest_cap + 1) * sizeof(JoinRestC));
        uint32_t *rest_n = (uint32_t *)ctx_ws(ctx, WS_JOIN_REST_N, n_waves * 4);
        if (!rest || !rest_n) { pf::CtxErr{ctx} = "no room for K-COV-C-JOIN's hand-over list"; return PF_ERR_HIP; }
        (void)ctx_begin_at(ctx, PF_K_COV_JOIN, st, &at);
#define PF_JOINC_LAUNCH(KK) k_cov_join_colored<KK><<<blocks, 256, 0, st>>>(t, ctx->k, ctx->d_seq, ctx->d_off, ctx->d_kpre, ctx->d_khead, ctx->d_krow, \
        ctx->n_colors, ctx->n_kmers, ctx->d_gcov_c, stride, rest, rest_n, rest_cap, ROWS)
        if (ctx->k == 25) PF_JOINC_LAUNCH(25);
        else if (ctx->k == 31) PF_JOINC_LAUNCH(31);
        else PF_JOINC_LAUNCH(0);
#undef PF_JOINC_LAUNCH
        ctx_end_at(ctx, at, st);
        (void)ctx_begin_at(ctx, PF_K_COV_JOIN_REST, st, &at);
        k_cov_join_colored_rest<<<blocks, 256, 0, st>>>(t, ctx->k, ctx->n_colors, rest, rest_n, rest_cap, ctx->d_gcov_c, stride, ctx->d_seq, ctx->d_off,
                                                                  ctx->d_kpre, ctx->d_khead, ctx->d_krow, ctx->n_kmers, ROWS);
        ctx_end_at(ctx, at, st);
    } else {
        (void)ctx_begin_at(ctx, PF_K_COV_JOIN, st, &at);
        k_cov_colored<<<ctx_grid(ctx, (uint64_t)ctx->N * 64, 256, 16), 256, 0, st>>>(t, ctx->d_seq, ctx->d_off, ctx->d_len, ctx->k, ctx->ctab_one_strand,
                                                                                            ctx->n_colors, 0, ctx->N, ctx->d_unread, nullptr, nullptr,
                                                                                            nullptr, nullptr, ctx->d_kpre, ctx->d_gcov_c, stride);
        ctx_end_at(ctx, at, st);
    }
    PF_HIP(hipGetLastError());
    PF_HIP(hipEventRecord(ctx->join_c_done, st));
    ctx->join_c_inflight = true;
    return PF_OK;
}

int join_colored_finish(pf_ctx *ctx) {
    if (!ctx->join_c_inflight) return PF_OK;
    ctx->join_c_inflight = false;
    PF_HIP(hipSetDevice(ctx->device));
    PF_HIP(hipEventSynchronize(ctx->join_c_done));
    ctx->gcov_c_valid = true;
    return PF_OK;
}

int join_graph_counts_colored(pf_ctx *ctx) {
    const int rc = join_graph_counts_colored_begin(ctx);
    return rc ? rc : join_colored_finish(ctx);
}
}

extern "C" {

uint32_t pf_num_colors(const pf_ctx *ctx) { return ctx ? ctx->n_colors : 0; }

int pf_upload_counts_colored(pf_ctx *ctx, uint32_t n_colors, const uint64_t *const *kmers, const uint32_t *const *counts,
                             const uint64_t *n, const uint64_t *min_count, const uint64_t *max_count, const int *both_strands) {
    if (!ctx || n_colors == 0 || !kmers || !counts || !n || !min_count || !max_count || !both_strands) return PF_ERR_ARG;
    if (n_colors > PF_MAX_COLORS_TABLE) { pf::CtxErr{ctx} = "more colours than the device table holds (PF_MAX_COLORS_TABLE)"; return PF_ERR_ARG; }
    if (!ctx->d_seq || !ctx->k) { pf::CtxErr{ctx} = "pf_upload_counts_colored: the graph comes first (the table is addressed by minimizers of length-k keys)"; return PF_ERR_ARG; }
    uint64_t total = 0, biggest = 0;
    for (uint32_t c = 0; c < n_colors; ++c) {
        if (n[c] && (!kmers[c] || !counts[c])) return PF_ERR_ARG;
        if (!both_strands[c]) continue;
        total += n[c];
        biggest = std::max(biggest, n[c]);
    }
    ctx->ctab_unread = 0;
    ctx->ctab_max_count = 0;
    std::vector<uint8_t> unread(n_colors, 0);
    for (uint32_t c = 0; c < n_colors; ++c) {
        if (!both_strands[c]) { unread[c] = 1; if (c < 64) ctx->ctab_unread |= 1ull << c; }
        else ctx->ctab_max_count = std::max<uint64_t>(ctx->ctab_max_count, max_count[c]);
    }
    (void)join_colored_finish(ctx);
    if (ctx->d_gcov_c) { (void)hipFree(ctx->d_gcov_c); ctx->d_gcov_c = nullptr; }
    ctx->gcov_c_valid = false;
    PF_HIP(hipSetDevice(ctx->device));
    if (ctx->d_ctab) { (void)hipFree(ctx->d_ctab); ctx->d_ctab = nullptr; }
    if (ctx->d_unread) { (void)hipFree(ctx->d_unread); ctx->d_unread = nullptr; }
    PF_HIP(hipMalloc(reinterpret_cast<void **>(&ctx->d_unread), n_colors));
    PF_HIP(hipMemcpy(ctx->d_unread, unread.data(), n_colors, hipMemcpyHostToDevice));
    ctx->n_colors = 0;
    uint64_t cap = 128;
    while (cap * 4 < biggest || cap * LINE_KEYS < total + total / 4 + 1) cap <<= 1;
    const uint32_t line_bytes = ctab_line_bytes(n_colors);
    PF_HIP(hipMalloc(reinterpret_cast<void **>(&ctx->d_ctab), cap * line_bytes));
    PF_HIP(hipMemsetAsync(ctx->d_ctab, 0xFF, cap * line_bytes, ctx->stream));
    ctx->ctab_cap = cap;
    ctx->ctab_line_bytes = line_bytes;
    DevTmp<unsigned int> noncanon_;
    PF_HIP(noncanon_.alloc(4));
    PF_HIP(hipMemsetAsync(noncanon_.p, 0, 4, ctx->stream));
    for (uint32_t c = 0; c < n_colors; ++c) {
        if (!n[c] || !both_strands[c]) continue;
        DevTmp<uint64_t> dk_;
        DevTmp<uint32_t> dc_;
        const uint64_t *pk = kmers[c];
        const uint32_t *pc = counts[c];
        if (!on_device(kmers[c])) {
            PF_HIP(dk_.alloc(n[c] * 8));
            PF_HIP(dc_.alloc(n[c] * 4));
            PF_HIP(hipMemcpyAsync(dk_.p, kmers[c], n[c] * 8, hipMemcpyDefault, ctx->stream));
            PF_HIP(hipMemcpyAsync(dc_.p, counts[c], n[c] * 4, hipMemcpyDefault, ctx->stream));
            pk = dk_.p;
            pc = dc_.p;
        }
        ctx_begin(ctx, PF_K_TABLE_BUILD);
        k_ctab_build<<<ctx_grid(ctx, n[c], 256, 8), 256, 0, ctx->stream>>>(ctx->d_ctab, cap - 1, line_bytes, ctx->k, pk, pc, n[c], min_count[c],
                                                                           max_count[c], c, noncanon_.p);
        ctx_end(ctx);
        PF_HIP(hipStreamSynchronize(ctx->stream));
    }
    {
        unsigned int h_noncanon = 0, h_flag = 0;
        PF_HIP(hipMemcpyAsync(&h_noncanon, noncanon_.p, 4, hipMemcpyDeviceToHost, ctx->stream));
        PF_HIP(hipStreamSynchronize(ctx->stream));
        if (total && h_noncanon) {
            DevTmp<unsigned int> flag_;
            PF_HIP(flag_.alloc(4));
            PF_HIP(hipMemsetAsync(flag_.p, 0, 4, ctx->stream));
            k_ctab_two_strands<<<ctx_grid(ctx, cap * LINE_KEYS, 256, 8), 256, 0, ctx->stream>>>(ctx->d_ctab, cap, line_bytes, ctx->k, flag_.p);
            PF_HIP(hipMemcpyAsync(&h_flag, flag_.p, 4, hipMemcpyDeviceToHost, ctx->stream));
            PF_HIP(hipStreamSynchronize(ctx->stream));
        }
        ctx->ctab_one_strand = total ? h_flag == 0 : false;
    }
    ctx->n_colors = n_colors;
    return join_graph_counts_colored(ctx);
}

static int unitig_cov_colored_impl(pf_ctx *ctx, uint32_t u0, uint32_t u1, uint64_t *sum, uint32_t *mn, uint32_t *mx, uint8_t *miss, bool probe) {
    if (!ctx || !ctx->d_seq || !ctx->d_ctab || !ctx->n_colors || u0 > u1 || u1 > ctx->N || !sum || !mn || !mx || !miss) return PF_ERR_ARG;
    if (u0 == u1) return PF_OK;
    PF_HIP(hipSetDevice(ctx->device));
    const size_t n = (size_t)(u1 - u0) * ctx->n_colors;
    const bool dev_out = on_device(sum);
    uint64_t *ds = sum;
    uint32_t *dlo = mn, *dhi = mx;
    uint8_t *dx = miss;
    if (!dev_out) {
        ds = (uint64_t *)ctx_ws(ctx, WS_CCOV_SUM, n * 8);
        dlo = (uint32_t *)ctx_ws(ctx, WS_CCOV_MIN, n * 4);
        dhi = (uint32_t *)ctx_ws(ctx, WS_CCOV_MAX, n * 4);
        dx = (uint8_t *)ctx_ws(ctx, WS_CCOV_MISS, n);
        if (!ds || !dlo || !dhi || !dx) return PF_ERR_HIP;
    }
    constexpr bool env_probe = false;
    probe = probe || env_probe;
    { const int rc = join_colored_finish(ctx); if (rc) return rc; }
    if (!probe && !ctx->gcov_c_valid) {
        const int rc = join_graph_counts_colored(ctx);
        if (rc) return rc;
    }
    const bool stream = !probe && ctx->gcov_c_valid;
    uint64_t g_range[2] = {0, 0};
    if (stream) {
        PF_HIP(hipMemcpyAsync(&g_range[0], ctx->d_kpre + u0, 8, hipMemcpyDeviceToHost, ctx->stream));
        PF_HIP(hipMemcpyAsync(&g_range[1], ctx->d_kpre + u1, 8, hipMemcpyDeviceToHost, ctx->stream));
        PF_HIP(hipStreamSynchronize(ctx->stream));
    }
    ctx_begin(ctx, PF_K_COV_COLORED);
    if (stream) {
        k_ccov_init<<<ctx_grid(ctx, n, 256, 8), 256, 0, ctx->stream>>>(n, ds, dlo, dhi, dx);
        Kc4Args a{ctx->d_gcov_c, ctx->gcov_c_stride, ctx->d_unread, ctx->d_khead, ctx->d_krow, u0, u1 - u0, g_range[0], g_range[1],
                  g_range[0] / 256, (g_range[1] + 255) / 256, ds, dlo, dhi, dx};
        const int rc = launch_cov_stream(ctx, a, ctx->n_colors, ctx->ctab_max_count >= (1ull << 20), true);
        if (rc) return rc;
    } else {
        const CTab t{ctx->d_ctab, ctx->ctab_cap - 1, ctx->ctab_line_bytes};
        const int grid = ctx_grid(ctx, (uint64_t)(u1 - u0) * 64, 256, 16);
        k_cov_colored<<<grid, 256, 0, ctx->stream>>>(t, ctx->d_seq, ctx->d_off, ctx->d_len, ctx->k, ctx->ctab_one_strand, ctx->n_colors, u0, u1,
                                                     ctx->d_unread, ds, dlo, dhi, dx, nullptr, nullptr, 0);
    }
    ctx_end(ctx);
    if (!dev_out) {
        PF_HIP(hipMemcpyAsync(sum, ds, n * 8, hipMemcpyDeviceToHost, ctx->stream));
        PF_HIP(hipMemcpyAsync(mn, dlo, n * 4, hipMemcpyDeviceToHost, ctx->stream));
        PF_HIP(hipMemcpyAsync(mx, dhi, n * 4, hipMemcpyDeviceToHost, ctx->stream));
        PF_HIP(hipMemcpyAsync(miss, dx, n, hipMemcpyDeviceToHost, ctx->stream));
        PF_HIP(hipStreamSynchronize(ctx->stream));
    }
    return PF_OK;
}

int pf_unitig_cov_colored(pf_ctx *ctx, uint32_t u0, uint32_t u1, uint64_t *sum, uint32_t *mn, uint32_t *mx, uint8_t *miss) {
    return unitig_cov_colored_impl(ctx, u0, u1, sum, mn, mx, miss, false);
}

int pf_unitig_cov_colored_probe(pf_ctx *ctx, uint32_t u0, uint32_t u1, uint64_t *sum, uint32_t *mn, uint32_t *mx, uint8_t *miss) {
    return unitig_cov_colored_impl(ctx, u0, u1, sum, mn, mx, miss, true);
}

int pf_string_cov_colored(pf_ctx *ctx, const char *text, const uint64_t *str_off, uint32_t n_str, const uint32_t *low,
                          const uint32_t *up, uint64_t *sum, uint8_t *ok) {
    if (!ctx || !ctx->d_ctab || !ctx->n_colors || !low || !up || (n_str && (!text || !str_off || !sum || !ok))) return PF_ERR_ARG;
    if (n_str == 0) return PF_OK;
    PF_HIP(hipSetDevice(ctx->device));
    const uint32_t C = ctx->n_colors;
    uint64_t total = 0;
    PF_HIP(hipMemcpy(&total, str_off + n_str, 8, hipMemcpyDefault));
    char *dt = (char *)ctx_ws(ctx, WS_STR_TEXT, (size_t)total + 1);
    uint64_t *doff = (uint64_t *)ctx_ws(ctx, WS_STR_OFF, ((size_t)n_str + 1) * 8);
    uint64_t *ds = (uint64_t *)ctx_ws(ctx, WS_STR_SUM, (size_t)n_str * C * 8);
    uint8_t *dk = (uint8_t *)ctx_ws(ctx, WS_STR_OK, (size_t)n_str * C);
    uint32_t *dcut = (uint32_t *)ctx_ws(ctx, WS_STR_MISS, (size_t)C * 8);
    if (!dt || !doff || !ds || !dk || !dcut) return PF_ERR_HIP;
    PF_HIP(hipMemcpyAsync(dt, text, (size_t)total, hipMemcpyDefault, ctx->stream));
    PF_HIP(hipMemcpyAsync(doff, str_off, ((size_t)n_str + 1) * 8, hipMemcpyDefault, ctx->stream));
    PF_HIP(hipMemcpyAsync(dcut, low, (size_t)C * 4, hipMemcpyDefault, ctx->stream));
    PF_HIP(hipMemcpyAsync(dcut + C, up, (size_t)C * 4, hipMemcpyDefault, ctx->stream));
    const CTab t{ctx->d_ctab, ctx->ctab_cap - 1, ctx->ctab_line_bytes};
    ctx_begin(ctx, PF_K_STRCOV_COLORED);
    k_strcov_colored<<<ctx_grid(ctx, (uint64_t)n_str * C, 256, 8), 256, 0, ctx->stream>>>(t, ctx->k, ctx->ctab_one_strand, C, ctx->d_unread, dt, doff, n_str,
                                                                                          dcut, dcut + C, ds, dk);
    ctx_end(ctx);
    PF_HIP(hipMemcpyAsync(sum, ds, (size_t)n_str * C * 8, hipMemcpyDefault, ctx->stream));
    PF_HIP(hipMemcpyAsync(ok, dk, (size_t)n_str * C, hipMemcpyDefault, ctx->stream));
    PF_HIP(hipStreamSynchronize(ctx->stream));
    return PF_OK;
}

}
```

### ploidyfrost_amd/csrc/pf_ctx.hpp

```cpp
#pragma once
#include <hip/hip_runtime.h>
#include <stdint.h>

#include <mutex>
#include <string>
#include <vector>

#include "pf_device_common.hpp"
#include "ploidyfrost_hip.h"

namespace pf {
template <typename T>
struct DevTmp {
    T *p = nullptr;
    DevTmp() = default;
    DevTmp(const DevTmp &) = delete;
    DevTmp &operator=(const DevTmp &) = delete;
    ~DevTmp() { if (p) (void)hipFree(p); }
    hipError_t alloc(size_t bytes) { return hipMalloc(reinterpret_cast<void **>(&p), bytes ? bytes : 1); }
};

struct TimedLaunch {
    int kernel;
    hipEvent_t a, b;
    bool closed;
};
struct CallState;

inline bool is_device_ptr(const void *p) {
    hipPointerAttribute_t at;
    const bool dev = p && hipPointerGetAttributes(&at, p) == hipSuccess && at.type == hipMemoryTypeDevice;
    (void)hipGetLastError();
    return dev;
}
}

struct pf_ctx {
    int device = 0;
    int n_cu = 256;
    std::string name;
    std::string err;
    hipStream_t own_stream = nullptr, stream = nullptr;

    uint64_t *d_seq = nullptr;
    uint64_t *d_off = nullptr;
    uint32_t *d_len = nullptr;
    uint32_t N = 0;
    int k = 0;
    uint64_t n_words = 0, n_kmers = 0;
    uint64_t *d_kpre = nullptr;
    uint32_t *d_kwin = nullptr;
    uint64_t n_kwin = 0;
    uint32_t *d_succ = nullptr, *d_pred = nullptr;
    uint32_t *d_pred16 = nullptr;
    bool has_adj = false;
    uint32_t *d_cand = nullptr;
    std::vector<uint32_t> h_cand;
    std::vector<uint32_t> h_len;

    pf::CountLine *d_tab = nullptr;
    uint64_t tab_cap = 0, tab_n = 0;
    hipStream_t join_stream = nullptr;
    hipEvent_t join_done = nullptr;
    bool join_inflight = false;
    hipEvent_t join_c_done = nullptr;
    bool join_c_inflight = false;
    int tab_k = 0;
    bool tab_one_strand = false;
    bool tab_exact = false;
    uint64_t tab_max_count = 0;

    uint32_t *d_gcov = nullptr;
    uint64_t *d_khead = nullptr;
    uint32_t *d_krow = nullptr;
    uint64_t n_krow = 0;
    bool gcov_valid = false;

    uint8_t *d_ctab = nullptr;
    uint64_t ctab_cap = 0;
    uint32_t ctab_line_bytes = 128, n_colors = 0;
    bool ctab_one_strand = false;
    uint64_t ctab_unread = 0;
    uint8_t *d_unread = nullptr;
    uint64_t ctab_max_count = 0;
    uint32_t *d_gcov_c = nullptr;
    uint64_t gcov_c_stride = 0;
    bool gcov_c_valid = false;

    uint64_t *d_cov_sum = nullptr;
    uint32_t *d_cov_min = nullptr;
    uint8_t *d_cov_miss = nullptr;
    uint32_t cov_cap = 0;

    uint64_t gmm_n = 0;
    bool gmm_loaded = false;

    pf::CallState *call = nullptr;
    hipStream_t bub_streams[PF_CALL_LANES][12] = {};
    hipEvent_t bub_events[PF_CALL_LANES][13] = {};

    void *cc = nullptr;
    void *gfa = nullptr;
    void *count = nullptr;
    void *clip = nullptr;
    void *qc = nullptr;
    void *unitig = nullptr;
    void *comm = nullptr;
    const void *cc_rec = nullptr;
    const uint32_t *cc_pool = nullptr;
    const pf_bfs_record *bfs_last_rec = nullptr;
    const uint32_t *bfs_last_pool = nullptr;
    uint64_t bfs_last_n = 0, bfs_last_pool_len = 0;
    uint64_t bfs_call_id = 0;
    uint64_t bfs_res_pool_cap = 0;
    hipStream_t copy_stream = nullptr;
    struct {
        bool active = false;
        pf_bfs_record *records = nullptr;
        uint64_t c0 = 0;
        std::vector<uint32_t> deferred;
    } bfs_pending;

    unsigned int bfs_live_n = 0;
    unsigned long long *h_live = nullptr;
    uint64_t live_cap = 0;

    std::vector<std::pair<void *, size_t>> ws;

    bool timing = false;
    uint64_t timing_mask = ~0ull;
    std::vector<hipEvent_t> event_pool;
    std::vector<pf::TimedLaunch> launches;
    size_t side_launch = (size_t)-1;
    size_t main_launch = (size_t)-1;
    std::mutex launch_mu;
    uint64_t units[PF_K_COUNT_] = {};
};

namespace pf {
struct CtxErr {
    pf_ctx *c;
    void operator=(std::string s) const {
        std::lock_guard<std::mutex> lk(c->launch_mu);
        c->err = std::move(s);
    }
};
#define PF_HIP(call)                                                                         \
    do {                                                                                     \
        hipError_t e_ = (call);                                                              \
        if (e_ != hipSuccess) {                                                              \
            pf::CtxErr{ctx} = std::string(#call) + ": " + hipGetErrorString(e_);                   \
            return PF_ERR_HIP;                                                               \
        }                                                                                    \
    } while (0)
struct Kc4Args;
int launch_cov_stream(pf_ctx *ctx, Kc4Args a, uint32_t n_colors, bool wide, bool colored);
int ctx_begin(pf_ctx *ctx, int kernel);
void ctx_end(pf_ctx *ctx);
int ctx_begin_on(pf_ctx *ctx, int kernel, hipStream_t stream);
void ctx_end_on(pf_ctx *ctx, hipStream_t stream);
int ctx_begin_at(pf_ctx *ctx, int kernel, hipStream_t stream, size_t *at);
void ctx_end_at(pf_ctx *ctx, size_t at, hipStream_t stream);
struct Timed {
    pf_ctx *ctx;
    Timed(pf_ctx *c, int kernel) : ctx(c) { ctx_begin(ctx, kernel); }
    ~Timed() { ctx_end(ctx); }
};
inline void ctx_units(pf_ctx *ctx, int kernel, uint64_t n) { if (ctx->timing) __atomic_fetch_add(&ctx->units[kernel], n, __ATOMIC_RELAXED); }
int ctx_grid(const pf_ctx *ctx, uint64_t work_items, int block, int per_cu);
inline size_t up256(size_t n) { return (n + 255) & ~(size_t)255; }
int join_graph_counts(pf_ctx *ctx);
int join_graph_counts_begin(pf_ctx *ctx);
int join_finish(pf_ctx *ctx);
int join_graph_counts_colored_begin(pf_ctx *ctx);
int join_colored_finish(pf_ctx *ctx);
hipStream_t join_stream(pf_ctx *ctx);
int join_graph_counts_colored(pf_ctx *ctx);
void *ctx_ws(pf_ctx *ctx, int slot, size_t bytes);
hipError_t lane_stream_create(hipStream_t *s, int lane);
struct DevLoadTrace {
    bool on = getenv("PF_TRACE_LOAD") != nullptr;
    std::chrono::steady_clock::time_point t = std::chrono::steady_clock::now();
    void mark(const char *what) {
        if (!on) return;
        const auto now = std::chrono::steady_clock::now();
        fprintf(stderr, "[load]   . %-42s %.3fs\n", what, std::chrono::duration<double>(now - t).count());
        t = now;
    }
};
void call_state_create(pf_ctx *ctx);
void call_destroy(pf_ctx *ctx);
void cc_destroy(pf_ctx *ctx);
void gfa_destroy(pf_ctx *ctx);
void comm_destroy(pf_ctx *ctx);
void count_destroy(pf_ctx *ctx);
void unitig_destroy(pf_ctx *ctx);
void clip_destroy(pf_ctx *ctx);
void qc_destroy(pf_ctx *ctx);
void call_invalidate(pf_ctx *ctx);
int call_state_arrays(pf_ctx *ctx, uint8_t **flags, uint32_t **plus, uint32_t **minus);
void call_state_resident(pf_ctx *ctx);
enum WsSlot {
    WS_ALN_TEXT = 0, WS_ALN_JOBS, WS_ALN_SMALL, WS_ALN_RETRY, WS_ALN_IDX, WS_ALN_OFIRST, WS_ALN_OCOUNT, WS_ALN_OHITS, WS_ALN_OTEXT,
    WS_ALN_OGAPS, WS_ALN_STTEXT, WS_ALN_STGAPS, WS_ALN_STHITS, WS_ALN_WORK, WS_BFS_REC, WS_BFS_POOL, WS_BFS_SMALL, WS_BFS_DEF, WS_BFS_WLIST,
    WS_BFS_RES_REC, WS_BFS_RES_POOL,
    WS_STR_TEXT, WS_STR_OFF, WS_STR_SUM, WS_STR_OK, WS_STR_MISS,
    WS_BUB_TEXT, WS_BUB_PATHS, WS_BUB_TASKS, WS_BUB_SMALL, WS_BUB_RETRY, WS_BUB_IDX, WS_BUB_RES, WS_BUB_OTEXT, WS_BUB_OSITES,
    WS_BUB_OGROUPS, WS_BUB_OILEN, WS_BUB_SCRATCH, WS_BUB_WORK, WS_BUB_IDX2, WS_CCOV_SUM, WS_CCOV_MIN, WS_CCOV_MAX, WS_CCOV_MISS, WS_GMM_X, WS_GMM_STATE, WS_GMM_PART,
    WS_JOIN_REST, WS_JOIN_REST_N,
    WS_DENSITY,
    WS_MASK_TEXT, WS_MASK_OUT, WS_MASK_BITS, WS_MASK_TABLE, WS_MASK_INDEX,
    WS_TRIM_TEXT2, WS_TRIM_INDEX2, WS_TRIM_TABLE2, WS_TRIM_WORK, WS_TRIM_OUT,
    WS_FASTA_WORK, WS_FASTA_LINES, WS_FASTA_TEXT, WS_FASTA_TABLE,
    WS_HETPAIR,
    WS_BUB_LANES,
    WS_COUNT_ = WS_BUB_LANES + 5 * (PF_CALL_LANES - 1)
};
inline int bub_ws(int slot, int lane) {
    if (lane == 0) return slot;
    const int j = slot == WS_BUB_SMALL ? 0 : slot == WS_BUB_RETRY ? 1 : slot == WS_BUB_SCRATCH ? 2 : slot == WS_BUB_WORK ? 3 : 4;
    return WS_BUB_LANES + 5 * (lane - 1) + j;
}
}
```

### ploidyfrost_amd/csrc/pf_device.hip

```cpp
#include <hip/hip_runtime.h>
#include <sys/mman.h>

#include <algorithm>
#include <cstdio>
#include <cstring>
#include <string>
#include <type_traits>
#include <vector>

#include "pf_cov_stream.hpp"
#include "pf_ctx.hpp"
#include "pf_device_common.hpp"
#include "pf_scan.hpp"
#include "ploidyfrost_hip.h"

using namespace pf;

static std::string g_create_err;


__global__ void k_fill_slots(Slot *t, uint64_t n) {
    uint64_t i = (uint64_t)blockIdx.x * blockDim.x + threadIdx.x;
    const uint64_t stride = (uint64_t)gridDim.x * blockDim.x;
    for (; i < n; i += stride) {
// ... 436 lines not shown
    }
    constexpr unsigned ev_flags = hipEventDisableSystemFence;
    if (!tl.a && (hipEventCreateWithFlags(&tl.a, ev_flags) != hipSuccess || hipEventCreateWithFlags(&tl.b, ev_flags) != hipSuccess)) return (size_t)-1;
    hipEventRecord(tl.a, stream);
    tl.closed = false;
    std::lock_guard<std::mutex> lk(ctx->launch_mu);
    ctx->launches.push_back(tl);
    return ctx->launches.size() - 1;
}
static void launch_close(pf_ctx *ctx, size_t at, hipStream_t stream) {
    hipEvent_t b;
    {
        std::lock_guard<std::mutex> lk(ctx->launch_mu);
        if (at >= ctx->launches.size()) return;
        b = ctx->launches[at].b;
        ctx->launches[at].closed = true;
    }
    hipEventRecord(b, stream);
}
int ctx_begin(pf_ctx *ctx, int kernel) {
    if (!ctx->timing) return 0;
    ctx->main_launch = launch_push(ctx, kernel, ctx->stream);
    return ctx->main_launch == (size_t)-1;
}
void ctx_end(pf_ctx *ctx) {
    if (!ctx->timing) return;
    launch_close(ctx, ctx->main_launch, ctx->stream);
}
int ctx_begin_on(pf_ctx *ctx, int kernel, hipStream_t stream) {
    if (!ctx->timing) return 0;
    ctx->side_launch = launch_push(ctx, kernel, stream);
    return ctx->side_launch == (size_t)-1;
}
void ctx_end_on(pf_ctx *ctx, hipStream_t stream) {
    if (!ctx->timing) return;
    launch_close(ctx, ctx->side_launch, stream);
    ctx->side_launch = (size_t)-1;
}
int ctx_begin_at(pf_ctx *ctx, int kernel, hipStream_t stream, size_t *at) {
    *at = (size_t)-1;
    if (!ctx->timing) return 0;
    *at = launch_push(ctx, kernel, stream);
    return *at == (size_t)-1;
}
void ctx_end_at(pf_ctx *ctx, size_t at, hipStream_t stream) {
    if (!ctx->timing) return;
    launch_close(ctx, at, stream);
}

void *ctx_ws(pf_ctx *ctx, int slot, size_t bytes) {
    {
        std::lock_guard<std::mutex> lk(ctx->launch_mu);
        if (ctx->ws.size() < (size_t)WS_COUNT_) ctx->ws.resize(WS_COUNT_, {nullptr, 0});
    }
    auto &w = ctx->ws[slot];
    if (w.second >= bytes && w.first) return w.first;
    if (w.first) { hipFree(w.first); w.first = nullptr; w.second = 0; }
    const size_t want = bytes + bytes / 4 + 256;
    void *p = nullptr;
    if (hipMalloc(&p, want) != hipSuccess) { pf::CtxErr{ctx} = "hipMalloc of a workspace failed"; return nullptr; }
    w.first = p;
    w.second = want;
    return p;
}

hipError_t lane_stream_create(hipStream_t *s, int lane) {
    if (lane == 0) return hipStreamCreateWithFlags(s, hipStreamNonBlocking);
    int least = 0, greatest = 0;
    const hipError_t e = hipDeviceGetStreamPriorityRange(&least, &greatest);
    if (e != hipSuccess) return e;
    return hipStreamCreateWithPriority(s, hipStreamNonBlocking, least);
}

int ctx_grid(const pf_ctx *ctx, uint64_t work_items, int block, int per_cu) {
    uint64_t want = (work_items + block - 1) / block;
    uint64_t cap = (uint64_t)ctx->n_cu * per_cu;
    if (want < 1) want = 1;
    return (int)std::min<uint64_t>(want, cap);
}

}

namespace pf {
int launch_cov_stream(pf_ctx *ctx, Kc4Args a, uint32_t n_colors, bool wide, bool colored) {
    const uint64_t n_sr = a.sr_end - a.sr_begin;
    const dim3 grid((unsigned)(((n_sr + KC4_SR - 1) / KC4_SR + 3) / 4), n_colors);
    if (colored) {
        if (wide) k_cov_stream4<true, true><<<grid, 256, 0, ctx->stream>>>(a);
        else k_cov_stream4<false, true><<<grid, 256, 0, ctx->stream>>>(a);
    } else {
        if (wide) k_cov_stream4<true, false><<<grid, 256, 0, ctx->stream>>>(a);
        else k_cov_stream4<false, false><<<grid, 256, 0, ctx->stream>>>(a);
    }
    PF_HIP(hipGetLastError());
    return PF_OK;
}
}

namespace pf {
hipStream_t join_stream(pf_ctx *ctx) {
    if (!ctx->join_stream) {
        int least = 0, greatest = 0;
        (void)hipDeviceGetStreamPriorityRange(&least, &greatest);
        if (hipStreamCreateWithPriority(&ctx->join_stream, hipStreamNonBlocking, least) != hipSuccess) { (void)hipGetLastError(); ctx->join_stream = nullptr; }
    }
    return ctx->join_stream ? ctx->join_stream : ctx->stream;
}

int join_graph_counts_begin(pf_ctx *ctx) {
    ctx->gcov_valid = false;
    ctx->join_inflight = false;
    if (!ctx->d_seq || !ctx->d_tab || ctx->tab_exact || ctx->tab_max_count >= GCOV_MISSING || ctx->n_kmers == 0) return PF_OK;
    PF_HIP(hipSetDevice(ctx->device));
    if (!ctx->d_gcov && hipMalloc(&ctx->d_gcov, ((ctx->n_krow + 4) * 64) * sizeof(uint32_t)) != hipSuccess) {
        (void)hipGetLastError();
        ctx->d_gcov = nullptr;
        return PF_OK;
    }
    constexpr uint32_t JOIN_ROWS_PER_WAVE = 64;
    const uint64_t n_rows = (ctx->n_kmers + 63) / 64;
    const uint64_t n_waves = ((n_rows + JOIN_ROWS_PER_WAVE - 1) / JOIN_ROWS_PER_WAVE + 3) / 4 * 4;
    const int blocks = (int)(n_waves / 4);
    const uint32_t rest_cap = JOIN_ROWS_PER_WAVE * 64 / 2;
    JoinRest *rest = (JoinRest *)ctx_ws(ctx, WS_JOIN_REST, n_waves * (rest_cap + 1) * sizeof(JoinRest));
    uint32_t *rest_n = (uint32_t *)ctx_ws(ctx, WS_JOIN_REST_N, n_waves * 4);
    if (!rest || !rest_n) { pf::CtxErr{ctx} = "no room for K-COV-JOIN's hand-over list"; return PF_ERR_HIP; }
    if (!ctx->join_done) PF_HIP(hipEventCreateWithFlags(&ctx->join_done, hipEventDisableTiming));
    const hipStream_t st = join_stream(ctx);
    size_t at = 0;
    (void)ctx_begin_at(ctx, PF_K_COV_JOIN, st, &at);
#define PF_JOIN_LAUNCH(KK) k_cov_join<KK><<<blocks, 256, 0, st>>>(ctx->d_tab, ctx->tab_cap - 1, ctx->k, ctx->d_seq, ctx->d_off, ctx->d_kpre, ctx->d_khead, \
        ctx->d_krow, ctx->tab_one_strand, ctx->n_kmers, ctx->d_gcov, rest, rest_n, rest_cap, JOIN_ROWS_PER_WAVE)
    if (ctx->k == 25) PF_JOIN_LAUNCH(25);
    else if (ctx->k == 31) PF_JOIN_LAUNCH(31);
    else PF_JOIN_LAUNCH(0);
#undef PF_JOIN_LAUNCH
    ctx_end_at(ctx, at, st);
    (void)ctx_begin_at(ctx, PF_K_COV_JOIN_REST, st, &at);
    k_cov_join_rest<<<blocks, 256, 0, st>>>(ctx->d_tab, ctx->tab_cap - 1, ctx->k, ctx->tab_one_strand, rest, rest_n, rest_cap, ctx->d_gcov, ctx->d_seq, ctx->d_off,
                                            ctx->d_kpre, ctx->d_khead, ctx->d_krow, ctx->n_kmers, JOIN_ROWS_PER_WAVE);
    ctx_end_at(ctx, at, st);
    PF_HIP(hipGetLastError());
    PF_HIP(hipEventRecord(ctx->join_done, st));
    ctx->join_inflight = true;
    return PF_OK;
}

int join_finish(pf_ctx *ctx) {
    if (!ctx->join_inflight) return PF_OK;
    ctx->join_inflight = false;
    PF_HIP(hipSetDevice(ctx->device));
    PF_HIP(hipEventSynchronize(ctx->join_done));
    ctx->gcov_valid = true;
    return PF_OK;
}

int join_graph_counts(pf_ctx *ctx) {
    const int rc = join_graph_counts_begin(ctx);
    return rc ? rc : join_finish(ctx);
}
}

template <typename T>
static int stage_in(pf_ctx *ctx, const T *src, size_t n, T **dev, bool *owned) {
    *owned = false;
    if (n == 0) { *dev = nullptr; return PF_OK; }
    if (is_device_ptr(src)) {
        *dev = const_cast<T *>(src);
        return PF_OK;
    }
    PF_HIP(hipMalloc(dev, n * sizeof(T)));
    *owned = true;
    PF_HIP(hipMemcpyAsync(*dev, src, n * sizeof(T), hipMemcpyDefault, ctx->stream));
    return PF_OK;
}

extern "C" {

const char *pf_kernel_name(int kernel) { return (kernel >= 0 && kernel < PF_K_COUNT_) ? kKernelNames[kernel] : "?"; }

const char *pf_last_error(const pf_ctx *ctx) {
    if (!ctx) return g_create_err.c_str();
    static thread_local std::string mine;
    {
        std::lock_guard<std::mutex> lk(const_cast<pf_ctx *>(ctx)->launch_mu);
        mine = ctx->err;
    }
    return mine.c_str();
}

int pf_warmup(int device) {
    if (hipSetDevice(device) != hipSuccess) { (void)hipGetLastError(); return PF_ERR_NO_DEVICE; }
    if (hipFree(nullptr) != hipSuccess) { (void)hipGetLastError(); return PF_ERR_HIP; }
    return PF_OK;
}

int pf_create(int device, pf_ctx **out) {
    if (!out) return PF_ERR_ARG;
    *out = nullptr;
    int n = 0;
    if (hipGetDeviceCount(&n) != hipSuccess || n <= 0) {
        g_create_err = "no HIP device visible: the PloidyFrost device layer has no CPU fallback";
        return PF_ERR_NO_DEVICE;
    }
    if (device < 0 || device >= n) { g_create_err = "device index out of range"; return PF_ERR_ARG; }
    hipDeviceProp_t prop;
    if (hipSetDevice(device) != hipSuccess || hipGetDeviceProperties(&prop, device) != hipSuccess) {
        g_create_err = "hipSetDevice / hipGetDeviceProperties failed";
        return PF_ERR_HIP;
    }
    if (std::string(prop.gcnArchName).rfind("gfx950", 0) != 0) {
        g_create_err = std::string("device is ") + prop.gcnArchName + ", this library is built for gfx950 only";
        return PF_ERR_NO_DEVICE;
    }
    pf_ctx *ctx = new pf_ctx();
    ctx->device = device;
    ctx->n_cu = prop.multiProcessorCount;
    ctx->name = prop.name;
    if (hipStreamCreateWithFlags(&ctx->own_stream, hipStreamNonBlocking) != hipSuccess) {
        g_create_err = "hipStreamCreate failed";
        delete ctx;
        return PF_ERR_HIP;
    }
    ctx->stream = ctx->own_stream;
    ctx->ws.resize(WS_COUNT_, {nullptr, 0});
    call_state_create(ctx);
    *out = ctx;
    return PF_OK;
}

static void free_graph(pf_ctx *ctx) {
    call_invalidate(ctx);
    hipFree(ctx->d_seq); hipFree(ctx->d_off); hipFree(ctx->d_len); hipFree(ctx->d_succ); hipFree(ctx->d_pred);
    hipFree(ctx->d_cand);
    hipFree(ctx->d_pred16);
    hipFree(ctx->d_kpre);
    hipFree(ctx->d_kwin);
    hipFree(ctx->d_gcov); hipFree(ctx->d_khead); hipFree(ctx->d_krow); hipFree(ctx->d_gcov_c);
    ctx->d_gcov = nullptr;
    ctx->d_gcov_c = nullptr;
    ctx->gcov_c_valid = false;
    ctx->d_khead = nullptr;
    ctx->d_krow = nullptr;
    ctx->gcov_valid = false;
    ctx->d_kpre = nullptr;
    ctx->d_kwin = nullptr;
    ctx->d_pred16 = nullptr;
    ctx->d_seq = ctx->d_off = nullptr;
    ctx->d_len = ctx->d_succ = ctx->d_pred = ctx->d_cand = nullptr;
    ctx->h_cand.clear();
    ctx->has_adj = false;
}

void pf_destroy(pf_ctx *ctx) {
    if (!ctx) return;
    hipSetDevice(ctx->device);
    hipStreamSynchronize(ctx->stream);
    if (ctx->join_stream) { hipStreamSynchronize(ctx->join_stream); hipStreamDestroy(ctx->join_stream); }
    if (ctx->join_done) hipEventDestroy(ctx->join_done);
    if (ctx->join_c_done) hipEventDestroy(ctx->join_c_done);
    for (auto &tl : ctx->launches) { hipEventDestroy(tl.a); hipEventDestroy(tl.b); }
    for (auto &e : ctx->event_pool) hipEventDestroy(e);
    call_destroy(ctx);
    cc_destroy(ctx);
    gfa_destroy(ctx);
    comm_destroy(ctx);
    count_destroy(ctx);
    unitig_destroy(ctx);
    clip_destroy(ctx);
    qc_destroy(ctx);
    free_graph(ctx);
    hipFree(ctx->d_tab);
    hipFree(ctx->d_ctab);
    hipFree(ctx->d_unread);
    hipFree(ctx->d_cov_sum); hipFree(ctx->d_cov_min); hipFree(ctx->d_cov_miss);
    for (auto &w : ctx->ws) hipFree(w.first);
    if (ctx->h_live) hipHostFree(ctx->h_live);
    if (ctx->copy_stream) { hipStreamSynchronize(ctx->copy_stream); hipStreamDestroy(ctx->copy_stream); }
    for (auto &lane : ctx->bub_streams) for (auto &s : lane) if (s) hipStreamDestroy(s);
    for (auto &lane : ctx->bub_events) for (auto &e : lane) if (e) hipEventDestroy(e);
    hipStreamDestroy(ctx->own_stream);
    delete ctx;
}

int pf_set_stream(pf_ctx *ctx, void *s) {
    if (!ctx) return PF_ERR_ARG;
    ctx->stream = s ? (hipStream_t)s : ctx->own_stream;
    return PF_OK;
}

int pf_synchronize(pf_ctx *ctx) {
    if (!ctx) return PF_ERR_ARG;
    PF_HIP(hipStreamSynchronize(ctx->stream));
    return PF_OK;
}

int pf_enable_timing(pf_ctx *ctx, int on) {
    if (!ctx) return PF_ERR_ARG;
    ctx->timing = on != 0;
    return PF_OK;
}

int pf_timing_select(pf_ctx *ctx, uint64_t kernel_mask) {
    if (!ctx) return PF_ERR_ARG;
    ctx->timing_mask = kernel_mask;
    return PF_OK;
}

int pf_reset_timing(pf_ctx *ctx) {
    if (!ctx) return PF_ERR_ARG;
    PF_HIP(hipSetDevice(ctx->device));
    PF_HIP(hipDeviceSynchronize());
    std::lock_guard<std::mutex> lk(ctx->launch_mu);
    for (auto &tl : ctx->launches) { ctx->event_pool.push_back(tl.a); ctx->event_pool.push_back(tl.b); }
    ctx->launches.clear();
    memset(ctx->units, 0, sizeof(ctx->units));
    return PF_OK;
}

int pf_kernel_units(pf_ctx *ctx, int kernel, uint64_t *units) {
    if (!ctx || kernel < 0 || kernel >= PF_K_COUNT_ || !units) return PF_ERR_ARG;
    *units = ctx->units[kernel];
    return PF_OK;
}

int pf_kernel_time(pf_ctx *ctx, int kernel, double *total_ms, uint64_t *launches) {
    if (!ctx || kernel < 0 || kernel >= PF_K_COUNT_) return PF_ERR_ARG;
    PF_HIP(hipStreamSynchronize(ctx->stream));
    double tot = 0;
    uint64_t n = 0;
    for (auto &tl : ctx->launches) {
        if (tl.kernel != kernel || !tl.closed) continue;
        float ms = 0;
        PF_HIP(hipEventElapsedTime(&ms, tl.a, tl.b));
        tot += ms;
        n++;
    }
    if (total_ms) *total_ms = tot;
    if (launches) *launches = n;
    return PF_OK;
}

static int busy_union(pf_ctx *ctx, uint64_t kernel_mask, double *busy_ms, double *span_ms) {
// ... 308 lines not shown
    PF_HIP(flag_.alloc(4));
    PF_HIP(hipMemsetAsync(flag_.p, 0, 4, ctx->stream));
    k_table_two_strands<<<ctx_grid(ctx, ctx->tab_cap * LINE_KEYS, 256, 8), 256, 0, ctx->stream>>>(ctx->d_tab, ctx->tab_cap, ctx->tab_k, flag_.p);
    PF_HIP(hipMemcpyAsync(&h_flag, flag_.p, 4, hipMemcpyDeviceToHost, ctx->stream));
    PF_HIP(hipStreamSynchronize(ctx->stream));
    ctx->tab_one_strand = h_flag == 0;
    return PF_OK;
}

int pf_upload_counts(pf_ctx *ctx, const uint64_t *kmers, const uint32_t *counts, uint64_t n, uint32_t k, uint64_t min_count,
                     uint64_t max_count, int both_strands) {
    if (!ctx || (n && (!kmers || !counts)) || k < 3 || k > 31) return PF_ERR_ARG;
    if (ctx->d_seq && (int)k != ctx->k) { pf::CtxErr{ctx} = "pf_upload_counts: k differs from the k of the resident graph"; return PF_ERR_ARG; }
    (void)join_finish(ctx);
    ctx->tab_exact = !both_strands;
    ctx->tab_max_count = max_count;
    call_invalidate(ctx);
    PF_HIP(hipSetDevice(ctx->device));
    hipFree(ctx->d_tab);
    ctx->d_tab = nullptr;
    hipFree(ctx->d_gcov);
    ctx->d_gcov = nullptr;
    ctx->gcov_valid = false;
    uint64_t cap = 128;
    while (cap * 4 < n) cap <<= 1;
    PF_HIP(hipMalloc(&ctx->d_tab, cap * sizeof(CountLine)));
    ctx->tab_cap = cap;
    ctx->tab_n = n;
    ctx->tab_k = (int)k;
    PF_HIP(hipMemsetAsync(ctx->d_tab, 0xFF, cap * sizeof(CountLine), ctx->stream));
    const bool on_dev = n && is_device_ptr(kmers);
    DevTmp<uint64_t> dk_;
    DevTmp<uint32_t> dc_;
    const uint64_t *pk = kmers;
    const uint32_t *pc = counts;
    if (!on_dev && n) {
        PF_HIP(dk_.alloc(n * 8));
        PF_HIP(dc_.alloc(n * 4));
        PF_HIP(hipMemcpyAsync(dk_.p, kmers, n * 8, hipMemcpyDefault, ctx->stream));
        PF_HIP(hipMemcpyAsync(dc_.p, counts, n * 4, hipMemcpyDefault, ctx->stream));
        pk = dk_.p;
        pc = dc_.p;
    }
    DevTmp<unsigned int> noncanon_;
    unsigned int h_noncanon = 0;
    PF_HIP(noncanon_.alloc(4));
    PF_HIP(hipMemsetAsync(noncanon_.p, 0, 4, ctx->stream));
    if (n) {
        ctx_begin(ctx, PF_K_TABLE_BUILD);
        k_table_build<<<ctx_grid(ctx, n, 256, 8), 256, 0, ctx->stream>>>(ctx->d_tab, cap - 1, (int)k, pk, pc, n, min_count, max_count, noncanon_.p);
        ctx_end(ctx);
    }
    PF_HIP(hipMemcpyAsync(&h_noncanon, noncanon_.p, 4, hipMemcpyDeviceToHost, ctx->stream));
    PF_HIP(hipStreamSynchronize(ctx->stream));
    const int rc = check_table_strands(ctx, h_noncanon == 0);
    if (rc) return rc;
    if (ctx->d_seq && !ctx->tab_exact) return pf::join_graph_counts(ctx);
    return PF_OK;
}

int pf_release_counts(pf_ctx *ctx) {
    if (!ctx) return PF_ERR_ARG;
    (void)join_finish(ctx);
    call_invalidate(ctx);
    PF_HIP(hipSetDevice(ctx->device));
    hipFree(ctx->d_tab);
    ctx->d_tab = nullptr;
    hipFree(ctx->d_gcov);
    ctx->d_gcov = nullptr;
    ctx->gcov_valid = false;
    ctx->tab_cap = ctx->tab_n = 0;
    return PF_OK;
}

int pf_join_counts_begin(pf_ctx *ctx) {
    if (!ctx || !ctx->d_seq) return PF_ERR_ARG;
    const bool single = ctx->d_tab && !ctx->tab_exact, colored = ctx->d_ctab && ctx->n_colors;
    if (!single && !colored) { pf::CtxErr{ctx} = "pf_join_counts: no canonical count table resident"; return PF_ERR_ARG; }
    { const int rc = pf::join_finish(ctx); if (rc) return rc; }
    { const int rc = pf::join_colored_finish(ctx); if (rc) return rc; }
    if (single) {
        const int rc = pf::join_graph_counts_begin(ctx);
        if (rc) return rc;
        if (!ctx->join_inflight) { pf::CtxErr{ctx} = "pf_join_counts: no joined coverage array for this table (max_count = 2^32 - 1, or no room)"; return PF_ERR_ARG; }
    }
    if (colored) {
        const int rc = pf::join_graph_counts_colored_begin(ctx);
        if (rc) return rc;
        if (!ctx->join_c_inflight) { pf::CtxErr{ctx} = "pf_join_counts: no joined coverage array for these databases (max_count = 2^32 - 1, or no room)"; return PF_ERR_ARG; }
    }
    return PF_OK;
}

int pf_join_counts_end(pf_ctx *ctx) {
    if (!ctx) return PF_ERR_ARG;
    const int rc = pf::join_finish(ctx);
    return rc ? rc : pf::join_colored_finish(ctx);
}

int pf_join_counts(pf_ctx *ctx) {
    const int rc = pf_join_counts_begin(ctx);
    return rc ? rc : pf_join_counts_end(ctx);
}

int pf_lookup_kmers(pf_ctx *ctx, const uint64_t *kmers, uint64_t n, uint32_t *counts, uint8_t *found) {
    if (!ctx || !ctx->d_tab || !kmers || !counts || !found) return PF_ERR_ARG;
    if (n == 0) return PF_OK;
    PF_HIP(hipSetDevice(ctx->device));
    uint64_t *dk;
    bool own;
    int rc = stage_in(ctx, kmers, n, &dk, &own);
    if (rc) return rc;
    DevTmp<uint64_t> own_;
    if (own) own_.p = dk;
    DevTmp<uint32_t> dc_;
    DevTmp<uint8_t> df_;
    PF_HIP(dc_.alloc(n * 4));
    PF_HIP(df_.alloc(n));
    uint32_t *dc = dc_.p;
    uint8_t *df = df_.p;
    k_lookup<<<ctx_grid(ctx, n, 256, 8), 256, 0, ctx->stream>>>(ctx->d_tab, ctx->tab_cap - 1, ctx->tab_k, ctx->tab_one_strand, dk, n, dc, df);
    PF_HIP(hipMemcpyAsync(counts, dc, n * 4, hipMemcpyDefault, ctx->stream));
    PF_HIP(hipMemcpyAsync(found, df, n, hipMemcpyDefault, ctx->stream));
    PF_HIP(hipStreamSynchronize(ctx->stream));
    return PF_OK;
}

static int unitig_cov_impl(pf_ctx *ctx, uint32_t u0, uint32_t u1, int exact, uint64_t *sum, uint32_t *mn, uint8_t *miss, bool probe = false) {
    if (!ctx || !ctx->d_seq || !ctx->d_tab || u0 > u1 || u1 > ctx->N || !sum || !mn || !miss) return PF_ERR_ARG;
    if (u0 == u1) return PF_OK;
    PF_HIP(hipSetDevice(ctx->device));
    const uint32_t n = u1 - u0;
    const bool dev_out = is_device_ptr(sum);
    uint64_t *ds = sum;
    uint32_t *dm = mn;
    uint8_t *dx = miss;
    if (!dev_out) {
        if (ctx->cov_cap < n) {
            hipFree(ctx->d_cov_sum); hipFree(ctx->d_cov_min); hipFree(ctx->d_cov_miss);
            ctx->d_cov_sum = nullptr; ctx->d_cov_min = nullptr; ctx->d_cov_miss = nullptr;
            PF_HIP(hipMalloc(&ctx->d_cov_sum, (size_t)n * 8));
            PF_HIP(hipMalloc(&ctx->d_cov_min, (size_t)n * 4));
            PF_HIP(hipMalloc(&ctx->d_cov_miss, (size_t)n));
            ctx->cov_cap = n;
        }
        ds = ctx->d_cov_sum; dm = ctx->d_cov_min; dx = ctx->d_cov_miss;
    }
    uint64_t g_range[2];
    PF_HIP(hipMemcpyAsync(&g_range[0], ctx->d_kpre + u0, 8, hipMemcpyDeviceToHost, ctx->stream));
    PF_HIP(hipMemcpyAsync(&g_range[1], ctx->d_kpre + u1, 8, hipMemcpyDeviceToHost, ctx->stream));
    PF_HIP(hipStreamSynchronize(ctx->stream));
    const uint64_t w_begin = g_range[0] / KCOV_WIN, w_end = (g_range[1] + KCOV_WIN - 1) / KCOV_WIN;
    static const bool env_probe = [] { const char *e = getenv("PF_KCOV_SCAN"); return e && !strcmp(e, "probe"); }();
    probe = probe || env_probe;
    { const int rc = join_finish(ctx); if (rc) return rc; }
    if (!exact && !probe && !ctx->gcov_valid) {
        const int rc = join_graph_counts(ctx);
        if (rc) return rc;
    }
    ctx_begin(ctx, PF_K_COV);
    k_cov_init<<<ctx_grid(ctx, n, 256, 8), 256, 0, ctx->stream>>>(n, ds, dm, dx);
    if (!exact && !probe && ctx->gcov_valid) {
        Kc4Args a{ctx->d_gcov, 0, nullptr, ctx->d_khead, ctx->d_krow, u0, n, g_range[0], g_range[1], g_range[0] / 256, (g_range[1] + 255) / 256,
                  ds, dm, nullptr, dx};
        const bool wide = ctx->tab_max_count >= (1ull << 20);
        const int rc = launch_cov_stream(ctx, a, 1, wide, false);
        if (rc) return rc;
    } else {
        k_cov<<<ctx_grid(ctx, (w_end - w_begin) * 64, 256, 16), 256, 0, ctx->stream>>>(ctx->d_tab, ctx->tab_cap - 1, ctx->k, ctx->d_seq, ctx->d_off, ctx->d_kpre,
                                                                                     ctx->d_kwin, ctx->N, ctx->tab_one_strand, exact, u0, g_range[0],
                                                                                     g_range[1], w_begin, w_end - w_begin, ds, dm, dx, nullptr);
    }
    ctx_end(ctx);
    if (!dev_out) {
        PF_HIP(hipMemcpyAsync(sum, ds, (size_t)n * 8, hipMemcpyDeviceToHost, ctx->stream));
        PF_HIP(hipMemcpyAsync(mn, dm, (size_t)n * 4, hipMemcpyDeviceToHost, ctx->stream));
        PF_HIP(hipMemcpyAsync(miss, dx, (size_t)n, hipMemcpyDeviceToHost, ctx->stream));
        PF_HIP(hipStreamSynchronize(ctx->stream));
        for (uint32_t i = 0; i < n; ++i)
            if (miss[i]) { pf::CtxErr{ctx} = "a k-mer of the graph is missing from the count table"; return PF_ERR_MISSING_KMER; }
    }
    return PF_OK;
}

int pf_unitig_cov(pf_ctx *ctx, uint32_t u0, uint32_t u1, uint64_t *sum, uint32_t *mn, uint8_t *miss) {
    if (ctx && ctx->tab_exact) {
        pf::CtxErr{ctx} = "the count database was built without canonical counting: pf_unitig_cov_exact gives its per-orientation coverage";
        return PF_ERR_ARG;
    }
    return unitig_cov_impl(ctx, u0, u1, 0, sum, mn, miss);
}

int pf_unitig_cov_probe(pf_ctx *ctx, uint32_t u0, uint32_t u1, uint64_t *sum, uint32_t *mn, uint8_t *miss) {
    if (ctx && ctx->tab_exact) {
        pf::CtxErr{ctx} = "the count database was built without canonical counting: pf_unitig_cov_exact gives its per-orientation coverage";
        return PF_ERR_ARG;
    }
    return unitig_cov_impl(ctx, u0, u1, 0, sum, mn, miss, true);
}

int pf_unitig_cov_exact(pf_ctx *ctx, uint32_t u0, uint32_t u1, int reverse, uint64_t *sum, uint32_t *mn, uint8_t *miss) {
    return unitig_cov_impl(ctx, u0, u1, reverse ? 2 : 1, sum, mn, miss);
}

int pf_string_cov(pf_ctx *ctx, const char *text, const uint64_t *str_off, uint32_t n_str, uint32_t low, uint32_t up,
                  uint64_t *sum, uint8_t *ok, uint8_t *miss) {
    if (!ctx || !ctx->d_tab || (n_str && (!text || !str_off || !sum || !ok || !miss))) return PF_ERR_ARG;
    if (n_str == 0) return PF_OK;
    PF_HIP(hipSetDevice(ctx->device));
    if (ctx->tab_exact) {
        const bool dev_out = is_device_ptr(sum);
        if (dev_out) {
            PF_HIP(hipMemsetAsync(sum, 0, (size_t)n_str * 8, ctx->stream));
            PF_HIP(hipMemsetAsync(ok, 1, n_str, ctx->stream));
            PF_HIP(hipMemsetAsync(miss, 0, n_str, ctx->stream));
            PF_HIP(hipStreamSynchronize(ctx->stream));
        } else {
            memset(sum, 0, (size_t)n_str * 8);
            memset(ok, 1, n_str);
            memset(miss, 0, n_str);
        }
        return PF_OK;
    }
    uint64_t total = 0;
    PF_HIP(hipMemcpy(&total, str_off + n_str, 8, hipMemcpyDefault));
    char *dt = (char *)ctx_ws(ctx, WS_STR_TEXT, (size_t)total + 1);
    uint64_t *doff = (uint64_t *)ctx_ws(ctx, WS_STR_OFF, ((size_t)n_str + 1) * 8);
    uint64_t *ds = (uint64_t *)ctx_ws(ctx, WS_STR_SUM, (size_t)n_str * 8);
    uint8_t *dk = (uint8_t *)ctx_ws(ctx, WS_STR_OK, n_str);
    uint8_t *dm = (uint8_t *)ctx_ws(ctx, WS_STR_MISS, n_str);
    if (!dt || !doff || !ds || !dk || !dm) return PF_ERR_HIP;
    PF_HIP(hipMemcpyAsync(dt, text, (size_t)total, hipMemcpyDefault, ctx->stream));
    PF_HIP(hipMemcpyAsync(doff, str_off, ((size_t)n_str + 1) * 8, hipMemcpyDefault, ctx->stream));
    ctx_begin(ctx, PF_K_STRCOV);
    k_strcov<<<ctx_grid(ctx, n_str, 256, 8), 256, 0, ctx->stream>>>(ctx->d_tab, ctx->tab_cap - 1, ctx->tab_k, ctx->tab_one_strand, dt, doff, n_str, low, up, ds, dk, dm);
    ctx_end(ctx);
    PF_HIP(hipMemcpyAsync(sum, ds, (size_t)n_str * 8, hipMemcpyDefault, ctx->stream));
    PF_HIP(hipMemcpyAsync(ok, dk, n_str, hipMemcpyDefault, ctx->stream));
    PF_HIP(hipMemcpyAsync(miss, dm, n_str, hipMemcpyDefault, ctx->stream));
    PF_HIP(hipStreamSynchronize(ctx->stream));
    return PF_OK;
}
}
```

### ploidyfrost_amd/hipapi.py

```python
from __future__ import annotations

import ctypes as C
import os

import numpy as np

PKG = os.path.dirname(os.path.abspath(__file__))
LIB_PATH = os.path.join(PKG, "csrc", "libploidyfrost_hip.so")

NONE = 0xFFFFFFFF
PF_OK, PF_ERR_ARG, PF_ERR_HIP, PF_ERR_NO_DEVICE, PF_ERR_OVERFLOW, PF_ERR_MISSING_KMER = range(6)
KERNELS = ["k_table_build", "k_adj_insert", "k_adj_probe", "k_cov", "k_bfs", "k_bfs_big", "k_align", "k_align_big",
           "k_strcov", "k_bubble", "k_bubble_big", "k_cov_colored", "k_strcov_colored", "k_gmm", "k_kmc_decode", "k_minz_count", "k_cov_join",
           "k_call_sides", "k_call_prep", "k_call_paths", "k_call_sites", "k_call_format", "k_call_snp", "k_bfs_thread", "k_call_pair", "k_call_stack", "k_cov_join_rest", "copy_text_to_host", "k_call_model"]

K_DENSITY = len(KERNELS)
K_HIST = K_DENSITY + 1
HIST_MAX_BINS = 1 << 20
K_MASK = K_HIST + 1
MASK_STATS = np.dtype([(f, "<u8") for f in ("reads", "reads_changed", "bases", "bases_masked", "kmers", "kmers_bad")])
MASK_NO_UPPER = 0xFFFFFFFF
K_COUNT = K_MASK + 1
COUNT_STATS = np.dtype([(f, "<u8") for f in ("reads", "bases", "kmers", "kmers_bad", "unique", "below_min", "above_max", "written")])
K_TRIM = K_COUNT + 1
# ... 44 lines not shown
DENSITY_MIN_POINTS, DENSITY_MAX_POINTS = 2, 4096

BFS_RECORD = np.dtype([("entrance", "<u4"), ("exit", "<u4"), ("n_seen", "<u4"), ("n_list", "<u4"), ("list_off", "<u8"),
                       ("outcome", "u1"), ("flag_cycle", "u1"), ("flag_tip", "u1"), ("strict", "u1"), ("pad", "<u4")])
ALIGN_JOB = np.dtype([("a_off", "<u8"), ("b_off", "<u8"), ("a_len", "<u4"), ("b_len", "<u4")])
ALIGN_HIT = np.dtype([("text_off", "<u8"), ("gap_off", "<u8"), ("len", "<u4"), ("n_gaps", "<u4"), ("score", "<i8"),
                      ("n_pos", "<u4"), ("n_indel", "<u4")])
CALL_SIDE = np.dtype([("u", "<u4"), ("exit_ov", "<u4"), ("err_unitig", "<u4"), ("plus_side", "u1"), ("kind", "u1"), ("aligned", "u1"),
                      ("err", "u1")])
CALL_RESULT = np.dtype([("text_len", "<u8", (10,)), ("allele", "<u8", (4,)), ("core_cov", "<u8"), ("core_num", "<u8"), ("n_called", "<u8"),
                        ("align_jobs", "<u8"), ("site_strings", "<u8"), ("n_branching", "<u8"),
                        ("snp_jobs", "<u8"), ("pair_jobs", "<u8"), ("wave_jobs", "<u8"), ("stack_jobs", "<u8"),
                        ("alignseq_packed_len", "<u8"), ("numeric_packed", "<u8")])
CALL_STREAMS = ["allele_frequency", "alignseq", "bifre", "trifre", "tetrafre", "pentafre", "bicov", "tricov", "tetracov", "pentacov"]
BUBBLE_PATH = np.dtype([("text_off", "<u8"), ("len", "<u4"), ("ov", "<u4")])
BUBBLE_TASK = np.dtype([("path_first", "<u8"), ("n_paths", "<u4"), ("pad", "<u4")])
BUBBLE_SITE = np.dtype([("col", "<u4"), ("is_indel", "u1"), ("maxnum", "u1"), ("pad", "<u2")])
BUBBLE_RESULT = np.dtype([("rows_off", "<u8"), ("site_off", "<u8"), ("group_off", "<u8"), ("ilen_off", "<u8"), ("n_rows", "<u4"),
                          ("n_cols", "<u4"), ("n_sites", "<u4"), ("n_indel_len", "<u4")])
CALL_BUBBLE = np.dtype([("entrance_ov", "<u4"), ("exit_ov", "<u4"), ("strict", "<u4"), ("n_inner", "<u4"), ("inner", "<u4", (4,)),
                        ("cov", "<f8", (4,)), ("core_mean", "<f8"), ("cov_sum", "<f8")])
assert CALL_BUBBLE.itemsize == 80
assert BFS_RECORD.itemsize == 32 and ALIGN_JOB.itemsize == 24 and ALIGN_HIT.itemsize == 40
assert BUBBLE_PATH.itemsize == 16 and BUBBLE_TASK.itemsize == 16 and BUBBLE_SITE.itemsize == 8 and BUBBLE_RESULT.itemsize == 48

_lib = None


class DeviceError(RuntimeError):
    def __init__(self, status: int, msg: str):
        super().__init__("ploidyfrost_hip status %d: %s" % (status, msg))
        self.status = status


def load_library() -> C.CDLL:
    global _lib
    if _lib is not None:
        return _lib
    if not os.path.exists(LIB_PATH):
        raise RuntimeError("%s is missing: run `python -c 'import __graft_entry__ as g; g.build()'` "
                           "(there is no CPU fallback for the device layer)" % LIB_PATH)
    try:
        import torch
    except Exception:
        pass
    L = C.CDLL(LIB_PATH)
    vp, u32, u64, i = C.c_void_p, C.c_uint32, C.c_uint64, C.c_int
    sig = {
        "pf_create": (i, [i, C.POINTER(vp)]),
        "pf_warmup": (i, [i]),
        "pf_destroy": (None, [vp]),
        "pf_last_error": (C.c_char_p, [vp]),
        "pf_set_stream": (i, [vp, vp]),
        "pf_synchronize": (i, [vp]),
        "pf_enable_timing": (i, [vp, i]),
        "pf_kernel_time": (i, [vp, i, C.POINTER(C.c_double), C.POINTER(u64)]),
        "pf_reset_timing": (i, [vp]),
        "pf_device_busy": (i, [vp, vp, vp]),
        "pf_kernel_units": (i, [vp, i, C.POINTER(u64)]),
        "pf_side_components": (i, [vp, i, vp, u64, vp, u64, vp, u64, vp, u64]),
        "pf_bfs_candidates_begin": (i, [vp, C.c_uint32, C.c_uint32, vp, u64, vp, u64, C.POINTER(u64), C.POINTER(u64), vp, vp, u64, C.POINTER(u64)]),
        "pf_bfs_candidates_end": (i, [vp]),
        "pf_bfs_candidates_split": (i, [vp, C.c_uint32, C.c_uint32, vp, u64, vp, u64, C.POINTER(u64), C.POINTER(u64), vp, u64, C.POINTER(u64)]),
        "pf_fetch": (i, [vp, vp, vp, u64]),
        "pf_bfs_candidates_resident": (i, [vp, C.c_uint32, C.c_uint32, C.POINTER(u64), C.POINTER(u64), vp, vp, u64, C.POINTER(u64)]),
        "pf_replay_device": (i, [vp, C.c_uint32, C.c_uint32, C.POINTER(u64), C.POINTER(u64)]),
        "pf_replay_big_fetch": (i, [vp, vp, vp, vp]),
        "pf_replay_set_colours": (i, [vp, C.c_uint32, vp, vp, vp]),
        "pf_replay_finish": (i, [vp, vp, vp, vp, u64]),
        "pf_call_get_state": (i, [vp, vp, vp, vp]),
        "pf_gfa_ingest": (i, [vp, vp, u64, i, i, C.POINTER(C.c_uint32), C.POINTER(C.c_uint32)]),
        "pf_gfa_parse": (i, [vp, vp, u64, i, i, C.POINTER(C.c_uint32), C.POINTER(C.c_uint32)]),
        "pf_gfa_upload": (i, [vp]),
        "pf_gfa_error": (C.c_char_p, [vp]),
        "pf_gfa_segments": (i, [vp, vp, vp, vp, vp, vp, C.POINTER(C.c_int)]),
        "pf_replay_order": (i, [vp, C.c_uint32, vp, vp, vp]),
        "pf_kernel_name": (C.c_char_p, [i]),
        "pf_upload_graph": (i, [vp, vp, vp, vp, u32, i]),
        "pf_build_adjacency": (i, [vp, vp, vp]),
        "pf_upload_counts": (i, [vp, vp, vp, u64, u32, u64, u64, i]),
        "pf_join_counts": (i, [vp]),
        "pf_join_counts_begin": (i, [vp]),
        "pf_join_counts_end": (i, [vp]),
        "pf_lookup_kmers": (i, [vp, vp, u64, vp, vp]),
        "pf_unitig_cov": (i, [vp, u32, u32, vp, vp, vp]),
        "pf_unitig_cov_probe": (i, [vp, u32, u32, vp, vp, vp]),
        "pf_count_candidates": (i, [vp, u32, u32, C.POINTER(u64)]),
        "pf_bfs_candidates": (i, [vp, u32, u32, vp, u64, vp, u64, C.POINTER(u64), C.POINTER(u64)]),
        "pf_align_batch": (i, [vp, vp, u64, vp, u32, C.c_double, C.c_double, C.c_double, vp, vp, vp, u64, vp, u64, vp, u64,
                               C.POINTER(u64)]),
        "pf_align_bubbles": (i, [vp, vp, u64, vp, u64, vp, u32, C.c_double, C.c_double, C.c_double, vp, vp, u64, vp, u64, vp, u64,
                                 vp, u64, C.POINTER(u64)]),
        "pf_string_cov": (i, [vp, vp, vp, u32, u32, u32, vp, vp, vp]),
        "pf_host_alloc": (i, [vp, C.c_size_t, C.POINTER(vp)]),
        "pf_selftest_scan": (i, [vp, u64, C.c_uint32]),
        "pf_call_set_numeric_packed": (i, [vp, i]),
        "pf_call_fetch_text": (i, [vp, i, i, vp, u64]),
        "pf_host_free": (None, [vp, vp]),
        "pf_device_name": (i, [vp, C.c_char_p, C.c_size_t]),
        "pf_device_pci_bus_id": (i, [vp, C.c_char_p, C.c_size_t]),
        "pf_table_capacity": (u64, [vp]),
        "pf_num_kmers": (u64, [vp]),
        "pf_upload_counts_colored": (i, [vp, u32, vp, vp, vp, vp, vp, vp]),
        "pf_num_colors": (u32, [vp]),
        "pf_unitig_cov_colored": (i, [vp, u32, u32, vp, vp, vp, vp]),
        "pf_unitig_cov_colored_probe": (i, [vp, u32, u32, vp, vp, vp, vp]),
        "pf_string_cov_colored": (i, [vp, vp, vp, u32, vp, vp, vp, vp]),
        "pf_unitig_cov_exact": (i, [vp, u32, u32, i, vp, vp, vp]),
        "pf_minimizer_table_slots": (u64, [u64]),
        "pf_minimizer_crowding": (i, [vp, i, u32, vp, vp, vp]),
        "pf_minimizer_replay_inputs": (i, [vp, i, C.c_uint32, vp, vp]),
        "pf_kmc_decode": (i, [vp, vp, u64, u32, u32, vp, u64, u32, u32, vp, vp]),
        "pf_device_free": (None, [vp, vp]),
        "pf_copy_to_host": (i, [vp, vp, vp, C.c_size_t]),
        "pf_gmm_upload": (i, [vp, vp, u64]),
        "pf_gmm_count": (u64, [vp]),
        "pf_gmm_fit": (i, [vp, u32, C.c_double, C.c_double, C.c_int32, C.c_double, vp, vp, vp, vp, vp]),
        "pf_call_set_state": (i, [vp, vp, vp, vp]),
        "pf_call_coverage": (i, [vp]),
        "pf_call_set_format": (i, [vp, i]),
        "pf_superbubble_rows": (i, [vp, i, C.POINTER(u64), C.POINTER(u64)]),
        "pf_superbubble_fetch": (i, [vp, vp, u64]),
        "pf_call_scan": (i, [vp, u32, u32, C.POINTER(u64)]),
        "pf_call_sides": (i, [vp, vp, u64]),
        "pf_call_resolve": (i, [vp, C.POINTER(u64), C.POINTER(u32), C.POINTER(u32)]),
        "pf_call_select": (i, [vp, vp, u64]),
        "pf_call_run": (i, [vp, i, u64, u64, u64, u32, C.c_double, C.c_double, C.c_double, vp]),
        "pf_call_align": (i, [vp, u64, u64, u32, C.c_double, C.c_double, C.c_double, vp]),
        "pf_call_text": (i, [vp, i, u64, vp]),
        "pf_call_set_alignseq_packed": (i, [vp, i]),
        "pf_comm_unique_id": (i, [vp]),
        "pf_comm_init": (i, [vp, vp, i, i]),
        "pf_gather": (i, [vp, vp, C.c_uint32, vp]),
        "pf_comm_destroy": (None, [vp]),
        "pf_call_peek": (i, [vp, i, vp, vp, vp, u64, vp, vp, vp, vp, vp, vp, vp]),
        "pf_call_reserve": (i, [vp, u64, C.c_uint32]),
        "pf_call_reserve_lanes": (i, [vp, u64, C.c_uint32, C.c_int]),
        "pf_timing_select": (i, [vp, u64]),
        "pf_kernel_busy": (i, [vp, u64, C.POINTER(C.c_double)]),
        "pf_call_reserve_text": (i, [vp, u64]),
        "pf_find_reserve": (i, [vp, u64]),
        "pf_call_set_colours": (i, [vp, u32, vp, vp, vp, vp, vp, vp, u64, u64]),
        "pf_call_set_cutoffs": (i, [vp, u32, vp, vp]),
        "pf_call_text_range": (i, [vp, i, u64, u64, u64, vp]),
        "pf_call_align_lane": (i, [vp, i, u64, u64, u32, C.c_double, C.c_double, C.c_double, vp]),
        "pf_call_text_range_lane": (i, [vp, i, i, u64, u64, u64, vp]),
        "pf_call_text_sizes": (i, [vp, i, u64, u64, u64, vp]),
        "pf_bfs_live_deferred": (i, [vp, u64, vp]),
        "pf_bfs_live_count": (i, [vp, vp]),
        "pf_call_fetch": (i, [vp, i, i, vp, u64]),
        "pf_call_fetch_slab": (i, [vp, i, vp, vp]),
        "pf_call_fetch_range": (i, [vp, i, u64, vp, u64, i]),
        "pf_call_fetch_wait": (i, [vp, i]),
        "pf_format_doubles": (i, [vp, vp, u64, vp, vp]),
        "pf_gmm_values": (i, [vp, vp, u64]),
        "pf_call_model_begin": (i, [vp, i, C.c_double]),
        "pf_call_model_take": (i, [vp, i]),
        "pf_call_model_finish": (i, [vp, C.POINTER(u64)]),
        "pf_call_fetched_bytes": (u64, [vp]),
        "pf_call_model_filter": (i, [vp, vp]),
        "pf_call_model_take_text": (i, [vp, i, C.c_char_p, u64]),
        "pf_call_model_filter_multi": (i, [vp, vp, i]),
        "pf_call_model_color_count": (C.c_uint32, [vp]),
        "pf_call_model_color_select": (i, [vp, i, C.POINTER(u64)]),
        "pf_gmm_density": (i, [vp, u32, C.c_double, vp, vp, vp]),
        "pf_count_histogram": (i, [vp, vp, u64, u64, u64, u32, vp]),
        "pf_mask_reads": (i, [vp, vp, u64, vp, vp, u64, u32, u32, vp, vp]),
        "pf_mask_fastq": (i, [vp, vp, u64, i, u32, u32, vp, C.POINTER(u64), vp, C.POINTER(u64)]),
        "pf_count_begin": (i, [vp, u32, i, u64]),
        "pf_count_reads": (i, [vp, vp, u64, vp, vp, u64, vp]),
        "pf_count_fastq": (i, [vp, vp, u64, i, C.POINTER(u64), vp, C.POINTER(u64)]),
        "pf_count_finish": (i, [vp, u64, u64, u64, C.POINTER(vp), C.POINTER(vp), C.POINTER(u64), vp]),
        "pf_count_abort": (i, [vp]),
        "pf_kmc_encode": (i, [vp, vp, vp, u64, u32, u32, u32, vp, vp]),
        "pf_unitig_build": (i, [vp, vp, u64, u32, u32, i, i, vp]),
        "pf_unitig_fetch": (i, [vp, u64, u64, vp]),
        "pf_unitig_release": (i, [vp]),
        "pf_unitig_text": (i, [vp, C.POINTER(vp), C.POINTER(u64)]),
        "pf_maskcount_reads": (i, [vp, vp, u64, vp, vp, u64, u32, u32, vp]),
        "pf_maskcount_fastq": (i, [vp, vp, u64, i, u32, u32, C.POINTER(u64), vp, C.POINTER(u64)]),
        "pf_unitig_build_colored": (i, [vp, vp, u64, u32, u32, i, i, u32, vp, C.POINTER(u64)]),
        "pf_color_begin": (i, [vp, u32]),
        "pf_color_reads": (i, [vp, u32, vp, u64, vp, vp, u64, vp]),
        "pf_color_fastq": (i, [vp, u32, vp, u64, i, C.POINTER(u64), vp, C.POINTER(u64)]),
        "pf_color_finish": (i, [vp, vp]),
        "pf_color_kmers": (i, [vp, u32, vp, u64, vp]),
        "pf_release_counts": (i, [vp]),
        "pf_kmer_union": (i, [vp, u32, vp, vp, C.POINTER(vp), C.POINTER(u64)]),
        "pf_color_fetch": (i, [vp, vp, vp, vp, vp, vp]),
        "pf_trim_fastq": (i, [vp, vp, u64, i, vp, u32, u32, vp, C.POINTER(u64), C.POINTER(u64), vp, vp, C.POINTER(u64), vp, C.POINTER(u64)]),
        "pf_trim_fastq_pair": (i, [vp, vp, u64, vp, u64, i, vp, u32, u32, C.POINTER(vp), C.POINTER(u64), C.POINTER(u64), C.POINTER(vp), C.POINTER(vp),
                                   C.POINTER(u64), vp, C.POINTER(u64)]),
        "pf_device_alloc": (i, [vp, C.c_size_t, C.POINTER(vp)]),
        "pf_copy": (i, [vp, vp, vp, C.c_size_t]),
        "pf_inflate_bgzf": (i, [vp, vp, u64, vp, u64, vp, u64, C.POINTER(u64), vp, C.POINTER(u64)]),
        "pf_inflate_gzip": (i, [vp, vp, u64, u64, vp, u32, u32, vp, u64, vp, vp, vp]),
        "pf_deflate_bgzf": (i, [vp, vp, u64, u32, vp, u64, C.POINTER(u64), vp, vp]),
        "pf_fasta_index": (i, [vp, vp, u64, i, C.POINTER(u64), C.POINTER(u64), C.POINTER(u64), C.POINTER(vp), C.POINTER(vp), C.POINTER(vp)]),
        "pf_fasta_index_fetch": (i, [vp, vp, u64, i, C.POINTER(u64), C.POINTER(u64), C.POINTER(u64), vp, u64, vp, vp, u64]),
        "pf_count_fasta": (i, [vp, vp, u64, i, C.POINTER(u64), vp, C.POINTER(u64)]),
        "pf_maskcount_fasta": (i, [vp, vp, u64, i, u32, u32, C.POINTER(u64), vp, C.POINTER(u64)]),
        "pf_color_fasta": (i, [vp, u32, vp, u64, i, C.POINTER(u64), vp, C.POINTER(u64)]),
        "pf_trim_table_fastq": (i, [vp, vp, u64, i, vp, vp, vp, C.POINTER(u64), C.POINTER(u64), C.POINTER(u64), vp, C.POINTER(u64)]),
        "pf_trim_table_fastq_pair": (i, [vp, vp, u64, vp, u64, i, vp, C.POINTER(vp), C.POINTER(vp), C.POINTER(u64), C.POINTER(u64), C.POINTER(u64), vp,
                                         C.POINTER(u64)]),
        "pf_count_fastq_trimmed": (i, [vp, vp, u64, i, vp, C.POINTER(u64), vp, vp, C.POINTER(u64)]),
        "pf_count_fastq_pair_trimmed": (i, [vp, vp, u64, vp, u64, i, vp, C.POINTER(u64), vp, vp, C.POINTER(u64)]),
        "pf_maskcount_fastq_trimmed": (i, [vp, vp, u64, i, vp, u32, u32, C.POINTER(u64), vp, vp, C.POINTER(u64)]),
        "pf_maskcount_fastq_pair_trimmed": (i, [vp, vp, u64, vp, u64, i, vp, u32, u32, C.POINTER(u64), vp, vp, C.POINTER(u64)]),
        "pf_clip_begin": (i, [vp, vp, vp, vp, u32, u32, u32]),
        "pf_clip_begin_pairs": (i, [vp, vp, vp, vp, u32, vp, vp, u32, u32, u32, u32, u32, i]),
        "pf_clip_pair_stats_get": (i, [vp, vp]),
        "pf_clip_stats_get": (i, [vp, vp]),
        "pf_clip_end": (i, [vp]),
        "pf_clip_last_ends": (i, [vp, i, vp, u64]),
        "pf_qc_begin": (i, [vp, u32]),
        "pf_qc_get": (i, [vp, i, i, vp]),
        "pf_qc_clip_get": (i, [vp, i, vp]),
        "pf_qc_fastq": (i, [vp, i, vp, u64, i, C.POINTER(u64), C.POINTER(u64), C.POINTER(u64)]),
        "pf_qc_end": (i, [vp]),
        "pf_hetpairs": (i, [vp, vp, vp, u64, u32, u32, u32, vp, C.POINTER(vp), C.POINTER(vp), C.POINTER(vp), C.POINTER(vp), C.POINTER(u64), vp]),
        "pf_hetpair_table": (i, [vp, vp, vp, u64, u32, u32, vp]),
    }
    for name, (res, args) in sig.items():
        fn = getattr(L, name)
        fn.restype = res
        fn.argtypes = args
    _lib = L
    return L


DECLARED_SYMBOLS = ["pf_create", "pf_warmup", "pf_destroy", "pf_last_error", "pf_set_stream", "pf_synchronize", "pf_enable_timing",
                    "pf_kernel_time", "pf_reset_timing", "pf_device_busy", "pf_kernel_units", "pf_side_components", "pf_replay_order", "pf_bfs_candidates_begin", "pf_bfs_candidates_end", "pf_fetch", "pf_bfs_candidates_resident", "pf_bfs_live_deferred", "pf_bfs_live_count", "pf_replay_device", "pf_replay_big_fetch", "pf_replay_set_colours", "pf_replay_finish", "pf_call_get_state", "pf_gfa_ingest", "pf_gfa_segments", "pf_gfa_parse", "pf_gfa_upload", "pf_gfa_error", "pf_kernel_name", "pf_upload_graph", "pf_build_adjacency",
                    "pf_upload_counts", "pf_join_counts", "pf_join_counts_begin", "pf_join_counts_end", "pf_lookup_kmers", "pf_unitig_cov", "pf_count_candidates", "pf_bfs_candidates",
                    "pf_align_batch", "pf_align_bubbles", "pf_string_cov", "pf_host_alloc", "pf_host_free", "pf_device_name", "pf_device_pci_bus_id", "pf_table_capacity", "pf_num_kmers",
                    "pf_upload_counts_colored", "pf_num_colors", "pf_unitig_cov_colored", "pf_string_cov_colored",
                    "pf_gmm_upload", "pf_gmm_count", "pf_gmm_fit", "pf_kmc_decode", "pf_device_free", "pf_copy_to_host",
                    "pf_minimizer_table_slots", "pf_minimizer_crowding", "pf_minimizer_replay_inputs", "pf_bfs_candidates_split", "pf_unitig_cov_exact", "pf_unitig_cov_probe", "pf_unitig_cov_colored_probe",
                    "pf_call_set_state", "pf_call_set_format", "pf_superbubble_rows", "pf_superbubble_fetch", "pf_call_coverage", "pf_call_scan", "pf_call_sides", "pf_call_resolve", "pf_call_select", "pf_call_run", "pf_call_align",
                    "pf_call_text", "pf_call_set_alignseq_packed", "pf_comm_unique_id", "pf_comm_init", "pf_gather", "pf_comm_destroy", "pf_call_reserve", "pf_call_reserve_lanes", "pf_timing_select", "pf_kernel_busy", "pf_call_reserve_text", "pf_selftest_scan", "pf_call_set_numeric_packed", "pf_call_fetch_text", "pf_find_reserve", "pf_call_set_colours", "pf_call_set_cutoffs", "pf_call_peek", "pf_call_text_range", "pf_call_align_lane", "pf_call_text_range_lane", "pf_call_text_sizes", "pf_call_fetch", "pf_call_fetch_slab", "pf_call_fetch_range", "pf_call_fetch_wait", "pf_format_doubles",
                    "pf_gmm_values", "pf_call_model_begin", "pf_call_model_take", "pf_call_model_finish", "pf_call_fetched_bytes",
                    "pf_call_model_filter", "pf_call_model_take_text",
                    "pf_call_model_filter_multi", "pf_call_model_color_count", "pf_call_model_color_select",
                    "pf_gmm_density", "pf_count_histogram", "pf_mask_reads", "pf_mask_fastq",
                    "pf_count_begin", "pf_count_reads", "pf_count_fastq", "pf_count_finish", "pf_count_abort", "pf_kmc_encode",
                    "pf_trim_fastq", "pf_trim_fastq_pair", "pf_unitig_build", "pf_unitig_fetch", "pf_unitig_release",
                    "pf_unitig_build_colored", "pf_color_begin", "pf_color_reads", "pf_color_fastq", "pf_color_finish", "pf_color_fetch",
                    "pf_maskcount_reads", "pf_maskcount_fastq", "pf_unitig_text",
                    "pf_kmer_union", "pf_color_kmers", "pf_release_counts",
                    "pf_trim_table_fastq", "pf_trim_table_fastq_pair", "pf_count_fastq_trimmed", "pf_count_fastq_pair_trimmed",
                    "pf_maskcount_fastq_trimmed", "pf_maskcount_fastq_pair_trimmed", "pf_inflate_bgzf", "pf_inflate_gzip", "pf_device_alloc", "pf_copy",
                    "pf_fasta_index", "pf_fasta_index_fetch", "pf_count_fasta", "pf_maskcount_fasta", "pf_color_fasta", "pf_deflate_bgzf",
                    "pf_clip_begin", "pf_clip_stats_get", "pf_clip_end", "pf_clip_last_ends",
                    "pf_clip_begin_pairs", "pf_clip_pair_stats_get",
                    "pf_qc_begin", "pf_qc_get", "pf_qc_clip_get", "pf_qc_fastq", "pf_qc_end",
                    "pf_hetpairs", "pf_hetpair_table"]


class TrimPlan(C.Structure):
    _fields_ = [("steps", C.c_void_p), ("n_steps", C.c_uint32), ("phred", C.c_uint32)]


def trim_steps(steps) -> np.ndarray:
    if isinstance(steps, np.ndarray) and steps.dtype == TRIM_STEP:
        return np.ascontiguousarray(steps)
    if isinstance(steps, str):
        steps = steps.split()
    out = np.zeros(len(steps), dtype=TRIM_STEP)
    for j, s in enumerate(steps):
        if isinstance(s, str):
            name, *fields = s.split(":")
            s = (TRIM_KINDS[name],) + tuple(int(x) for x in fields)
        out[j] = tuple(s) + (0,) * (3 - len(s))
    return out


def density_dict(x: np.ndarray, density: np.ndarray, info: np.ndarray) -> dict:
    r = info[0]
    return {"x": x, "density": density, "bw": float(r["bw"]), "n": int(r["n"]), "min": float(r["min"]), "max": float(r["max"]),
            "sd": float(r["sd"]), "q1": float(r["q1"]), "q3": float(r["q3"]), "order": np.array(r["order"], dtype=np.float64)}


def call_peek(ctx_handle, lane: int = 0):
    L = load_library()
    h = C.c_void_p(ctx_handle)
    used = (C.c_uint64 * 6)()
    st = L.pf_call_peek(h, lane, None, None, None, 0, None, None, None, None, None, None, used)
    if st != PF_OK:
        raise DeviceError(st, L.pf_last_error(h).decode())
    nb = int(used[0])
    if nb == 0:
        return []
    cap = (C.c_uint64 * 5)(*[int(used[x + 1]) for x in range(5)])
    bub = np.zeros(nb, dtype=CALL_BUBBLE)
    res = np.zeros(nb, dtype=BUBBLE_RESULT)
    sv_off = np.zeros(nb, dtype=np.uint64)
    text = np.zeros(max(1, cap[0]), dtype=np.uint8)
    sites = np.zeros(max(1, cap[1]), dtype=BUBBLE_SITE)
    groups = np.zeros(max(1, cap[2]), dtype=np.uint8)
    ilen = np.zeros(max(1, cap[3]), dtype=np.uint32)
    sv = np.zeros(max(1, cap[4]), dtype=np.float64)
    st = L.pf_call_peek(h, lane, bub.ctypes.data, res.ctypes.data, sv_off.ctypes.data, nb, text.ctypes.data, sites.ctypes.data,
                        groups.ctypes.data, ilen.ctypes.data, sv.ctypes.data, cap, used)
    if st != PF_OK:
        raise DeviceError(st, L.pf_last_error(h).decode())
    tb = text.tobytes()
    out = []
    for j in range(nb):
        b, r = bub[j], res[j]
        d = dict(entrance_ov=int(b["entrance_ov"]), exit_ov=int(b["exit_ov"]), strict=bool(b["strict"]),
                 inner=[int(x) for x in b["inner"][: int(b["n_inner"])]], cov=[float(x) for x in b["cov"][: int(b["n_inner"])]],
                 core_mean=float(b["core_mean"]), cov_sum=float(b["cov_sum"]), rows=None)
        R, Lc = int(r["n_rows"]), int(r["n_cols"])
        if R:
            o = int(r["rows_off"])
            d["rows"] = [tb[o + i * Lc: o + (i + 1) * Lc] for i in range(R)]
            d["sites"] = []
# ... 1035 lines not shown
```

Baseline: 244.3 million.

## Defer count-join launch and queue coverage behind it on a side stream

The join of k-mer counts into per-k-mer coverage arrays is no longer launched eagerly in join_begin. It is marked pending and launched through join_flush, either at begin time or after the BFS kernel, depending on an environment variable. Whole-graph coverage no longer blocks the host on join completion; it is queued on a stream gated by the join event, and the call stage waits on a cov_done event. This also skips the kpre range readback when the whole range is requested, and adds a pf_join_status tracing hook, at the cost of more event and stream bookkeeping and ordering risk.

New measurement: 240.6 million. -1.5%, worse.

```diff
diff --git a/include/ploidyfrost_hip.h b/include/ploidyfrost_hip.h
--- a/include/ploidyfrost_hip.h
+++ b/include/ploidyfrost_hip.h
@@ -296,6 +296,7 @@
 int pf_join_counts(pf_ctx *);
 int pf_join_counts_begin(pf_ctx *);
 int pf_join_counts_end(pf_ctx *);
+int pf_join_status(pf_ctx *, int *join, int *cov);
 int pf_lookup_kmers(pf_ctx *, const uint64_t *kmers, uint64_t n, uint32_t *counts, uint8_t *found);
 
 int pf_unitig_cov(pf_ctx *, uint32_t u0, uint32_t u1, uint64_t *sum, uint32_t *min, uint8_t *miss);
diff --git a/ploidyfrost_amd/csrc/host/pf_cdbg.hpp b/ploidyfrost_amd/csrc/host/pf_cdbg.hpp
--- a/ploidyfrost_amd/csrc/host/pf_cdbg.hpp
+++ b/ploidyfrost_amd/csrc/host/pf_cdbg.hpp
@@ -203,6 +203,8 @@
     int pending_ids_rc_ = 0;
     uint64_t ids_bytes_ = 0;
     int launch_coverage();
+    void trace_join(const char *tag, double ms);
+    bool join_seen_ = false, cov_seen_ = false;
     uint64_t find_passes_ = 0;
     bool cov_ready_ = false;
     std::string cov_err_;
diff --git a/ploidyfrost_amd/csrc/host/pf_cdbg_call.cpp b/ploidyfrost_amd/csrc/host/pf_cdbg_call.cpp
--- a/ploidyfrost_amd/csrc/host/pf_cdbg_call.cpp
+++ b/ploidyfrost_amd/csrc/host/pf_cdbg_call.cpp
@@ -242,7 +242,7 @@
     allele_[0] = allele_[1] = allele_[2] = allele_[3] = 0;
     core_cov_ = core_num_ = 0;
     const bool trace = getenv("PF_TRACE_PLOIDY") != nullptr;
-    auto tp = [&](const char *what) { if (trace) fprintf(stderr, "[ploidy] %-28s %.2f ms\n", what, since(t_all) * 1e3); };
+    auto tp = [&](const char *what) { if (trace) { fprintf(stderr, "[ploidy] %-28s %.2f ms\n", what, since(t_all) * 1e3); trace_join("[ploidy]", since(t_all) * 1e3); } };
 
     struct OutFile {
         std::string name;
diff --git a/ploidyfrost_amd/csrc/host/pf_cdbg_find.cpp b/ploidyfrost_amd/csrc/host/pf_cdbg_find.cpp
--- a/ploidyfrost_amd/csrc/host/pf_cdbg_find.cpp
+++ b/ploidyfrost_amd/csrc/host/pf_cdbg_find.cpp
@@ -263,9 +263,11 @@
     const unsigned wt = walk_threads(thr), few = (unsigned)std::min<size_t>(host_threads(thr), 8);
     DeviceFind df;
     EarlyWalks early(*this, tr, wt);
+    join_seen_ = cov_seen_ = false;
+    const auto tj = [&] { if (tr.find) trace_join("[find]", since(tr.t_all) * 1e3); };
     int st = traverse_resident(early, df, tr);
     if (st != PF_OK) return failed(st);
-    tr.step("traversed on the device");
+    tr.step("traversed on the device"); tj();
     df.walked.resize((size_t)df.n_deferred);
     df.lists.resize((size_t)df.n_deferred);
     std::string walk_err;
@@ -273,11 +275,11 @@
     st = pf_side_components(ctx_, 1, nullptr, df.n_rec, nullptr, 0, nullptr, 0, nullptr, 0);
     tr.step("  components of the device's records");
     if (st == PF_OK && overlap_output_) cov_ready_ = launch_coverage() == PF_OK;
-    tr.step("  coverage launched");
+    tr.step("  coverage launched"); tj();
     walk.join();
     if (!walk_err.empty()) return fail(PF_ERR_HIP, "CDBG::findSuperBubble(): walk of a long traversal: " + walk_err);
     if (st != PF_OK) return failed(st);
-    tr.step("long traversals walked");
+    tr.step("long traversals walked"); tj();
     walked_into_candidate_order(df);
     tr.step("  walked records in candidate order");
     if (!df.walked.empty()) st = pf_side_components(ctx_, 0, nullptr, df.n_rec, nullptr, 0, df.walked.data(), df.walked.size(), df.xpool.data(), df.xpool.size());
@@ -285,7 +287,7 @@
     static const uint32_t small_limit = [] { const char *e = getenv("PF_REPLAY_SMALL_LIMIT"); return e ? (uint32_t)atoi(e) : 256u; }();
     if (st == PF_OK) st = pf_replay_device(ctx_, (uint32_t)std::min<size_t>(complex_size_, 0xFFFFFFFFu), small_limit, &df.n_big, &df.big_entries);
     if (st != PF_OK) return failed(st);
-    tr.step("components + commits on the device");
+    tr.step("components + commits on the device"); tj();
     st = commit_large_on_host(df, tr, few);
     if (st != PF_OK) return failed(st);
     st = patch_device_state(df.p_sides, tr, few);
@@ -293,7 +295,7 @@
     if (tr.find) fprintf(stderr, "[find] %zu sides patched on the device %.2f ms\n", df.p_sides.size(), since(tr.t_all) * 1e3);
     state_host_stale_ = true;
     state_on_device_ = true;
-    tr.step("large components committed here");
+    tr.step("large components committed here"); tj();
     times_.bfs_device_s = since(tr.t_all);
     times_.candidates = df.n_rec;
     times_.bfs_deferred = df.n_deferred;
@@ -666,6 +668,13 @@
     return finish_find(outpre, tr, write_file, false);
 }
 
+void CDBG::trace_join(const char *tag, double ms) {
+    int join = 0, cov = 0;
+    if ((join_seen_ && cov_seen_) || pf_join_status(ctx_, &join, &cov) != PF_OK) return;
+    if (join == 2 && !join_seen_) { join_seen_ = true; fprintf(stderr, "%s %-28s %.2f ms\n", tag, "  join_done seen complete", ms); }
+    if (cov == 2 && !cov_seen_) { cov_seen_ = true; fprintf(stderr, "%s %-28s %.2f ms\n", tag, "  cov_done seen complete", ms); }
+}
+
 int CDBG::launch_coverage() {
     if (resident_path()) {
         const int st = pf_call_coverage(ctx_);
diff --git a/ploidyfrost_amd/csrc/pf_bfs.hip b/ploidyfrost_amd/csrc/pf_bfs.hip
--- a/ploidyfrost_amd/csrc/pf_bfs.hip
+++ b/ploidyfrost_amd/csrc/pf_bfs.hip
@@ -326,6 +326,7 @@
     ctx_begin(ctx, PF_K_BFS);
     k_bfs<<<ctx_grid(ctx, (p.n / 4 + 64) * 64, 256, 8), 256, 0, ctx->stream>>>(ctx->d_succ, ctx->d_pred, ctx->d_cand, p.c0, p.c1, p.o, p.d_wlist, &p.d_cnt->n_wave_list, env_wave_cap());
     ctx_end(ctx);
+    if (const int st = join_flush(ctx, ctx->stream)) return st;
     if (const int st = bfs_read_counters(ctx, p, cnt)) return st;
     ctx->bfs_live_n = cnt.n_live;
     ctx_units(ctx, PF_K_BFS, cnt.n_wave_list);
@@ -392,7 +393,8 @@
     PF_HIP(hipSetDevice(ctx->device));
     BfsPlan p; BfsCounters cnt;
     int st = bfs_plan(ctx, q, p), status = PF_OK;
-    if (st != PF_OK || p.n == 0) return st;
+    if (st == PF_OK && p.n == 0) return join_flush(ctx, nullptr);
+    if (st != PF_OK) return st;
     bfs_arm_live(ctx, q, p);
     if ((st = bfs_short_tiers(ctx, p, cnt)) != PF_OK) return st;
     if (cnt.n_deferred && q.mode.long_walks == LongWalks::BY_CALLER) {
diff --git a/ploidyfrost_amd/csrc/pf_call.hip b/ploidyfrost_amd/csrc/pf_call.hip
--- a/ploidyfrost_amd/csrc/pf_call.hip
+++ b/ploidyfrost_amd/csrc/pf_call.hip
@@ -288,6 +288,7 @@
     a.n_colors = S->n_colors;
     a.ccov_sum = S->ccov_sum.as<uint64_t>(); a.ccov_min = S->ccov_min.as<uint32_t>(); a.ccov_max = S->ccov_max.as<uint32_t>(); a.ccov_miss = S->ccov_miss.as<uint8_t>();
     a.clow = S->col_low.as<uint32_t>(); a.cup = S->col_up.as<uint32_t>(); a.full = S->col_full.as<uint64_t>(); a.cwords = S->col_words; a.size_total = S->col_size.as<uint64_t>();
+    { const int rc = pf::cov_wait_on(ctx, st); if (rc) return rc; }
     ctx_begin(ctx, PF_K_CALL_SCAN);
     if (S->n_colors) k_call_sides<true><<<(N + 255) / 256, 256, 0, st>>>(a);
     else k_call_sides<false><<<(N + 255) / 256, 256, 0, st>>>(a);
diff --git a/ploidyfrost_amd/csrc/pf_colored.hip b/ploidyfrost_amd/csrc/pf_colored.hip
--- a/ploidyfrost_amd/csrc/pf_colored.hip
+++ b/ploidyfrost_amd/csrc/pf_colored.hip
@@ -310,9 +310,25 @@
 }
 
 namespace pf {
+namespace {
+constexpr uint32_t JOINC_ROWS = 64;
+constexpr uint32_t JOINC_REST_CAP = JOINC_ROWS * 64 / 2;
+bool joinc_pipelined(const pf_ctx *ctx) { return ctx->ctab_one_strand && ctx->n_colors <= (uint32_t)JOINC_MAX && ctx->ctab_unread == 0; }
+struct JoinCWs { uint64_t n_waves; JoinRestC *rest; uint32_t *rest_n; };
+JoinCWs joinc_ws(pf_ctx *ctx) {
+    const uint64_t n_rows = (ctx->n_kmers + 63) / 64;
+    JoinCWs w;
+    w.n_waves = ((n_rows + JOINC_ROWS - 1) / JOINC_ROWS + 3) / 4 * 4;
+    w.rest = (JoinRestC *)ctx_ws(ctx, WS_JOIN_REST, w.n_waves * (JOINC_REST_CAP + 1) * sizeof(JoinRestC));
+    w.rest_n = (uint32_t *)ctx_ws(ctx, WS_JOIN_REST_N, w.n_waves * 4);
+    return w;
+}
+}
+
 int join_graph_counts_colored_begin(pf_ctx *ctx) {
     ctx->gcov_c_valid = false;
     ctx->join_c_inflight = false;
+    ctx->join_c_pending = false;
     if (!ctx->d_seq || !ctx->d_ctab || !ctx->n_colors || !ctx->d_kpre || ctx->n_kmers == 0 || ctx->ctab_max_count >= MISSING) return PF_OK;
     PF_HIP(hipSetDevice(ctx->device));
     const uint64_t stride = (ctx->n_krow + 4) * 64;
@@ -325,19 +341,27 @@
         }
         ctx->gcov_c_stride = stride;
     }
+    if (joinc_pipelined(ctx)) {
+        const JoinCWs w = joinc_ws(ctx);
+        if (!w.rest || !w.rest_n) { pf::CtxErr{ctx} = "no room for K-COV-C-JOIN's hand-over list"; return PF_ERR_HIP; }
+    }
+    if (!ctx->join_c_done) PF_HIP(hipEventCreateWithFlags(&ctx->join_c_done, hipEventDisableTiming));
+    ctx->join_c_pending = true;
+    return PF_OK;
+}
+
+int join_colored_launch(pf_ctx *ctx, hipStream_t st) {
+    if (!ctx->d_gcov_c || !ctx->join_c_done) { pf::CtxErr{ctx} = "K-COV-C-JOIN: no joined array to fill"; return PF_ERR_HIP; }
     const CTab t{ctx->d_ctab, ctx->ctab_cap - 1, ctx->ctab_line_bytes};
-    if (!ctx->join_c_done) PF_HIP(hipEventCreateWithFlags(&ctx->join_c_done, hipEventDisableTiming));
-    const hipStream_t st = join_stream(ctx);
+    const uint64_t stride = ctx->gcov_c_stride;
     size_t at = 0;
-    if (ctx->ctab_one_strand && ctx->n_colors <= (uint32_t)JOINC_MAX && ctx->ctab_unread == 0) {
-        constexpr uint32_t ROWS = 64;
-        const uint64_t n_rows = (ctx->n_kmers + 63) / 64;
-        const uint64_t n_waves = ((n_rows + ROWS - 1) / ROWS + 3) / 4 * 4;
-        const int blocks = (int)(n_waves / 4);
-        const uint32_t rest_cap = ROWS * 64 / 2;
-        JoinRestC *rest = (JoinRestC *)ctx_ws(ctx, WS_JOIN_REST, n_waves * (rest_cap + 1) * sizeof(JoinRestC));
-        uint32_t *rest_n = (uint32_t *)ctx_ws(ctx, WS_JOIN_REST_N, n_waves * 4);
-        if (!rest || !rest_n) { pf::CtxErr{ctx} = "no room for K-COV-C-JOIN's hand-over list"; return PF_ERR_HIP; }
+    if (joinc_pipelined(ctx)) {
+        constexpr uint32_t ROWS = JOINC_ROWS, rest_cap = JOINC_REST_CAP;
+        const JoinCWs w = joinc_ws(ctx);
+        if (!w.rest || !w.rest_n) { pf::CtxErr{ctx} = "no room for K-COV-C-JOIN's hand-over list"; return PF_ERR_HIP; }
+        JoinRestC *rest = w.rest;
+        uint32_t *rest_n = w.rest_n;
+        const int blocks = (int)(w.n_waves / 4);
         (void)ctx_begin_at(ctx, PF_K_COV_JOIN, st, &at);
 #define PF_JOINC_LAUNCH(KK) k_cov_join_colored<KK><<<blocks, 256, 0, st>>>(t, ctx->k, ctx->d_seq, ctx->d_off, ctx->d_kpre, ctx->d_khead, ctx->d_krow, \
         ctx->n_colors, ctx->n_kmers, ctx->d_gcov_c, stride, rest, rest_n, rest_cap, ROWS)
@@ -364,6 +388,7 @@
 }
 
 int join_colored_finish(pf_ctx *ctx) {
+    { const int rc = join_flush(ctx, nullptr); if (rc) return rc; }
     if (!ctx->join_c_inflight) return PF_OK;
     ctx->join_c_inflight = false;
     PF_HIP(hipSetDevice(ctx->device));
@@ -476,32 +501,46 @@
     }
     constexpr bool env_probe = false;
     probe = probe || env_probe;
-    { const int rc = join_colored_finish(ctx); if (rc) return rc; }
-    if (!probe && !ctx->gcov_c_valid) {
-        const int rc = join_graph_counts_colored(ctx);
+    const bool whole = u0 == 0 && u1 == ctx->N;
+    hipStream_t st = ctx->stream;
+    bool queued = false;
+    if (dev_out && whole && !probe && !join_place_begin()) {
+        { const int rc = join_flush(ctx, nullptr); if (rc) return rc; }
+        queued = ctx->join_c_inflight && ctx->d_gcov_c;
+    }
+    if (queued) {
+        const int rc = cov_queue_begin(ctx, &st);
         if (rc) return rc;
-    }
-    const bool stream = !probe && ctx->gcov_c_valid;
-    uint64_t g_range[2] = {0, 0};
-    if (stream) {
+    } else {
+        { const int rc = join_colored_finish(ctx); if (rc) return rc; }
+        if (!probe && !ctx->gcov_c_valid) {
+            const int rc = join_graph_counts_colored(ctx);
+            if (rc) return rc;
+        }
+    }
+    const bool stream = !probe && (queued || ctx->gcov_c_valid);
+    uint64_t g_range[2] = {0, ctx->n_kmers};
+    if (stream && !whole) {
         PF_HIP(hipMemcpyAsync(&g_range[0], ctx->d_kpre + u0, 8, hipMemcpyDeviceToHost, ctx->stream));
         PF_HIP(hipMemcpyAsync(&g_range[1], ctx->d_kpre + u1, 8, hipMemcpyDeviceToHost, ctx->stream));
         PF_HIP(hipStreamSynchronize(ctx->stream));
     }
-    ctx_begin(ctx, PF_K_COV_COLORED);
+    size_t at = 0;
+    (void)ctx_begin_at(ctx, PF_K_COV_COLORED, st, &at);
     if (stream) {
-        k_ccov_init<<<ctx_grid(ctx, n, 256, 8), 256, 0, ctx->stream>>>(n, ds, dlo, dhi, dx);
+        k_ccov_init<<<ctx_grid(ctx, n, 256, 8), 256, 0, st>>>(n, ds, dlo, dhi, dx);
         Kc4Args a{ctx->d_gcov_c, ctx->gcov_c_stride, ctx->d_unread, ctx->d_khead, ctx->d_krow, u0, u1 - u0, g_range[0], g_range[1],
                   g_range[0] / 256, (g_range[1] + 255) / 256, ds, dlo, dhi, dx};
-        const int rc = launch_cov_stream(ctx, a, ctx->n_colors, ctx->ctab_max_count >= (1ull << 20), true);
+        const int rc = launch_cov_stream(ctx, a, ctx->n_colors, ctx->ctab_max_count >= (1ull << 20), true, st);
         if (rc) return rc;
     } else {
         const CTab t{ctx->d_ctab, ctx->ctab_cap - 1, ctx->ctab_line_bytes};
         const int grid = ctx_grid(ctx, (uint64_t)(u1 - u0) * 64, 256, 16);
-        k_cov_colored<<<grid, 256, 0, ctx->stream>>>(t, ctx->d_seq, ctx->d_off, ctx->d_len, ctx->k, ctx->ctab_one_strand, ctx->n_colors, u0, u1,
-                                                     ctx->d_unread, ds, dlo, dhi, dx, nullptr, nullptr, 0);
-    }
-    ctx_end(ctx);
+        k_cov_colored<<<grid, 256, 0, st>>>(t, ctx->d_seq, ctx->d_off, ctx->d_len, ctx->k, ctx->ctab_one_strand, ctx->n_colors, u0, u1,
+                                            ctx->d_unread, ds, dlo, dhi, dx, nullptr, nullptr, 0);
+    }
+    ctx_end_at(ctx, at, st);
+    if (queued) return cov_queue_end(ctx, st);
     if (!dev_out) {
         PF_HIP(hipMemcpyAsync(sum, ds, n * 8, hipMemcpyDeviceToHost, ctx->stream));
         PF_HIP(hipMemcpyAsync(mn, dlo, n * 4, hipMemcpyDeviceToHost, ctx->stream));
diff --git a/ploidyfrost_amd/csrc/pf_ctx.hpp b/ploidyfrost_amd/csrc/pf_ctx.hpp
--- a/ploidyfrost_amd/csrc/pf_ctx.hpp
+++ b/ploidyfrost_amd/csrc/pf_ctx.hpp
@@ -65,6 +65,13 @@
     bool join_inflight = false;
     hipEvent_t join_c_done = nullptr;
     bool join_c_inflight = false;
+    bool join_pending = false, join_c_pending = false;
+    hipEvent_t join_gate = nullptr;
+    hipEvent_t cov_gate = nullptr;
+    hipEvent_t cov_done = nullptr;
+    bool cov_inflight = false;
+    bool cov_recorded = false;
+    std::mutex join_mu;
     int tab_k = 0;
     bool tab_one_strand = false;
     bool tab_exact = false;
@@ -154,7 +161,7 @@
         }                                                                                    \
     } while (0)
 struct Kc4Args;
-int launch_cov_stream(pf_ctx *ctx, Kc4Args a, uint32_t n_colors, bool wide, bool colored);
+int launch_cov_stream(pf_ctx *ctx, Kc4Args a, uint32_t n_colors, bool wide, bool colored, hipStream_t st);
 int ctx_begin(pf_ctx *ctx, int kernel);
 void ctx_end(pf_ctx *ctx);
 int ctx_begin_on(pf_ctx *ctx, int kernel, hipStream_t stream);
@@ -175,6 +182,13 @@
 int join_graph_counts_colored_begin(pf_ctx *ctx);
 int join_colored_finish(pf_ctx *ctx);
 hipStream_t join_stream(pf_ctx *ctx);
+int join_flush(pf_ctx *ctx, hipStream_t behind);
+int join_launch(pf_ctx *ctx, hipStream_t st);
+int join_colored_launch(pf_ctx *ctx, hipStream_t st);
+bool join_place_begin();
+int cov_queue_begin(pf_ctx *ctx, hipStream_t *st);
+int cov_queue_end(pf_ctx *ctx, hipStream_t st);
+int cov_wait_on(pf_ctx *ctx, hipStream_t st);
 int join_graph_counts_colored(pf_ctx *ctx);
 void *ctx_ws(pf_ctx *ctx, int slot, size_t bytes);
 hipError_t lane_stream_create(hipStream_t *s, int lane);
diff --git a/ploidyfrost_amd/csrc/pf_device.hip b/ploidyfrost_amd/csrc/pf_device.hip
--- a/ploidyfrost_amd/csrc/pf_device.hip
+++ b/ploidyfrost_amd/csrc/pf_device.hip
@@ -542,15 +542,15 @@
 }
 
 namespace pf {
-int launch_cov_stream(pf_ctx *ctx, Kc4Args a, uint32_t n_colors, bool wide, bool colored) {
+int launch_cov_stream(pf_ctx *ctx, Kc4Args a, uint32_t n_colors, bool wide, bool colored, hipStream_t st) {
     const uint64_t n_sr = a.sr_end - a.sr_begin;
     const dim3 grid((unsigned)(((n_sr + KC4_SR - 1) / KC4_SR + 3) / 4), n_colors);
     if (colored) {
-        if (wide) k_cov_stream4<true, true><<<grid, 256, 0, ctx->stream>>>(a);
-        else k_cov_stream4<false, true><<<grid, 256, 0, ctx->stream>>>(a);
+        if (wide) k_cov_stream4<true, true><<<grid, 256, 0, st>>>(a);
+        else k_cov_stream4<false, true><<<grid, 256, 0, st>>>(a);
     } else {
-        if (wide) k_cov_stream4<true, false><<<grid, 256, 0, ctx->stream>>>(a);
-        else k_cov_stream4<false, false><<<grid, 256, 0, ctx->stream>>>(a);
+        if (wide) k_cov_stream4<true, false><<<grid, 256, 0, st>>>(a);
+        else k_cov_stream4<false, false><<<grid, 256, 0, st>>>(a);
     }
     PF_HIP(hipGetLastError());
     return PF_OK;
@@ -567,9 +567,26 @@
     return ctx->join_stream ? ctx->join_stream : ctx->stream;
 }
 
+bool join_place_begin() { const char *e = getenv("PF_JOIN_PLACE"); return !(e && !strcmp(e, "bfs")); }
+
+namespace {
+constexpr uint32_t JOIN_ROWS_PER_WAVE = 64;
+constexpr uint32_t JOIN_REST_CAP = JOIN_ROWS_PER_WAVE * 64 / 2;
+struct JoinWs { uint64_t n_waves; JoinRest *rest; uint32_t *rest_n; };
+JoinWs join_ws(pf_ctx *ctx) {
+    const uint64_t n_rows = (ctx->n_kmers + 63) / 64;
+    JoinWs w;
+    w.n_waves = ((n_rows + JOIN_ROWS_PER_WAVE - 1) / JOIN_ROWS_PER_WAVE + 3) / 4 * 4;
+    w.rest = (JoinRest *)ctx_ws(ctx, WS_JOIN_REST, w.n_waves * (JOIN_REST_CAP + 1) * sizeof(JoinRest));
+    w.rest_n = (uint32_t *)ctx_ws(ctx, WS_JOIN_REST_N, w.n_waves * 4);
+    return w;
+}
+}
+
 int join_graph_counts_begin(pf_ctx *ctx) {
     ctx->gcov_valid = false;
     ctx->join_inflight = false;
+    ctx->join_pending = false;
     if (!ctx->d_seq || !ctx->d_tab || ctx->tab_exact || ctx->tab_max_count >= GCOV_MISSING || ctx->n_kmers == 0) return PF_OK;
     PF_HIP(hipSetDevice(ctx->device));
     if (!ctx->d_gcov && hipMalloc(&ctx->d_gcov, ((ctx->n_krow + 4) * 64) * sizeof(uint32_t)) != hipSuccess) {
@@ -577,16 +594,20 @@
         ctx->d_gcov = nullptr;
         return PF_OK;
     }
-    constexpr uint32_t JOIN_ROWS_PER_WAVE = 64;
-    const uint64_t n_rows = (ctx->n_kmers + 63) / 64;
-    const uint64_t n_waves = ((n_rows + JOIN_ROWS_PER_WAVE - 1) / JOIN_ROWS_PER_WAVE + 3) / 4 * 4;
-    const int blocks = (int)(n_waves / 4);
-    const uint32_t rest_cap = JOIN_ROWS_PER_WAVE * 64 / 2;
-    JoinRest *rest = (JoinRest *)ctx_ws(ctx, WS_JOIN_REST, n_waves * (rest_cap + 1) * sizeof(JoinRest));
-    uint32_t *rest_n = (uint32_t *)ctx_ws(ctx, WS_JOIN_REST_N, n_waves * 4);
-    if (!rest || !rest_n) { pf::CtxErr{ctx} = "no room for K-COV-JOIN's hand-over list"; return PF_ERR_HIP; }
+    const JoinWs w = join_ws(ctx);
+    if (!w.rest || !w.rest_n) { pf::CtxErr{ctx} = "no room for K-COV-JOIN's hand-over list"; return PF_ERR_HIP; }
     if (!ctx->join_done) PF_HIP(hipEventCreateWithFlags(&ctx->join_done, hipEventDisableTiming));
-    const hipStream_t st = join_stream(ctx);
+    ctx->join_pending = true;
+    return PF_OK;
+}
+
+int join_launch(pf_ctx *ctx, hipStream_t st) {
+    const JoinWs w = join_ws(ctx);
+    if (!w.rest || !w.rest_n || !ctx->d_gcov || !ctx->join_done) { pf::CtxErr{ctx} = "no room for K-COV-JOIN's hand-over list"; return PF_ERR_HIP; }
+    const int blocks = (int)(w.n_waves / 4);
+    JoinRest *rest = w.rest;
+    uint32_t *rest_n = w.rest_n;
+    constexpr uint32_t rest_cap = JOIN_REST_CAP;
     size_t at = 0;
     (void)ctx_begin_at(ctx, PF_K_COV_JOIN, st, &at);
 #define PF_JOIN_LAUNCH(KK) k_cov_join<KK><<<blocks, 256, 0, st>>>(ctx->d_tab, ctx->tab_cap - 1, ctx->k, ctx->d_seq, ctx->d_off, ctx->d_kpre, ctx->d_khead, \
@@ -606,12 +627,51 @@
     return PF_OK;
 }
 
+int join_flush(pf_ctx *ctx, hipStream_t behind) {
+    std::lock_guard<std::mutex> lk(ctx->join_mu);
+    if (!ctx->join_pending && !ctx->join_c_pending) return PF_OK;
+    PF_HIP(hipSetDevice(ctx->device));
+    const hipStream_t st = join_stream(ctx);
+    if (behind && behind != st) {
+        if (!ctx->join_gate) PF_HIP(hipEventCreateWithFlags(&ctx->join_gate, hipEventDisableTiming));
+        PF_HIP(hipEventRecord(ctx->join_gate, behind));
+        PF_HIP(hipStreamWaitEvent(st, ctx->join_gate, 0));
+    }
+    int rc = PF_OK;
+    if (ctx->join_pending) { ctx->join_pending = false; rc = join_launch(ctx, st); }
+    if (ctx->join_c_pending) { ctx->join_c_pending = false; if (rc == PF_OK) rc = join_colored_launch(ctx, st); }
+    if (getenv("PF_TRACE_FIND")) fprintf(stderr, "[find] K-COV-JOIN enqueued %s\n", behind ? "behind K-BFS" : "at once");
+    return rc;
+}
+
 int join_finish(pf_ctx *ctx) {
+    { const int rc = join_flush(ctx, nullptr); if (rc) return rc; }
     if (!ctx->join_inflight) return PF_OK;
     ctx->join_inflight = false;
     PF_HIP(hipSetDevice(ctx->device));
     PF_HIP(hipEventSynchronize(ctx->join_done));
     ctx->gcov_valid = true;
+    return PF_OK;
+}
+
+int cov_queue_begin(pf_ctx *ctx, hipStream_t *st) {
+    *st = join_stream(ctx);
+    if (*st == ctx->stream) return PF_OK;
+    if (!ctx->cov_gate) PF_HIP(hipEventCreateWithFlags(&ctx->cov_gate, hipEventDisableTiming));
+    PF_HIP(hipEventRecord(ctx->cov_gate, ctx->stream));
+    PF_HIP(hipStreamWaitEvent(*st, ctx->cov_gate, 0));
+    return PF_OK;
+}
+int cov_queue_end(pf_ctx *ctx, hipStream_t st) {
+    if (!ctx->cov_done) PF_HIP(hipEventCreateWithFlags(&ctx->cov_done, hipEventDisableTiming));
+    PF_HIP(hipEventRecord(ctx->cov_done, st));
+    ctx->cov_inflight = ctx->cov_recorded = true;
+    return PF_OK;
+}
+int cov_wait_on(pf_ctx *ctx, hipStream_t st) {
+    if (!ctx->cov_inflight) return PF_OK;
+    ctx->cov_inflight = false;
+    PF_HIP(hipStreamWaitEvent(st, ctx->cov_done, 0));
     return PF_OK;
 }
 
@@ -715,10 +775,15 @@
 void pf_destroy(pf_ctx *ctx) {
     if (!ctx) return;
     hipSetDevice(ctx->device);
+    (void)join_finish(ctx);
+    (void)join_colored_finish(ctx);
     hipStreamSynchronize(ctx->stream);
     if (ctx->join_stream) { hipStreamSynchronize(ctx->join_stream); hipStreamDestroy(ctx->join_stream); }
     if (ctx->join_done) hipEventDestroy(ctx->join_done);
     if (ctx->join_c_done) hipEventDestroy(ctx->join_c_done);
+    if (ctx->join_gate) hipEventDestroy(ctx->join_gate);
+    if (ctx->cov_gate) hipEventDestroy(ctx->cov_gate);
+    if (ctx->cov_done) hipEventDestroy(ctx->cov_done);
     for (auto &tl : ctx->launches) { hipEventDestroy(tl.a); hipEventDestroy(tl.b); }
     for (auto &e : ctx->event_pool) hipEventDestroy(e);
     call_destroy(ctx);
@@ -1193,20 +1258,31 @@
     if (single) {
         const int rc = pf::join_graph_counts_begin(ctx);
         if (rc) return rc;
-        if (!ctx->join_inflight) { pf::CtxErr{ctx} = "pf_join_counts: no joined coverage array for this table (max_count = 2^32 - 1, or no room)"; return PF_ERR_ARG; }
+        if (!ctx->join_pending) { pf::CtxErr{ctx} = "pf_join_counts: no joined coverage array for this table (max_count = 2^32 - 1, or no room)"; return PF_ERR_ARG; }
     }
     if (colored) {
         const int rc = pf::join_graph_counts_colored_begin(ctx);
         if (rc) return rc;
-        if (!ctx->join_c_inflight) { pf::CtxErr{ctx} = "pf_join_counts: no joined coverage array for these databases (max_count = 2^32 - 1, or no room)"; return PF_ERR_ARG; }
-    }
-    return PF_OK;
+        if (!ctx->join_c_pending) { pf::CtxErr{ctx} = "pf_join_counts: no joined coverage array for these databases (max_count = 2^32 - 1, or no room)"; return PF_ERR_ARG; }
+    }
+    ctx->cov_recorded = false;
+    return pf::join_place_begin() ? pf::join_flush(ctx, nullptr) : PF_OK;
 }
 
 int pf_join_counts_end(pf_ctx *ctx) {
     if (!ctx) return PF_ERR_ARG;
     const int rc = pf::join_finish(ctx);
     return rc ? rc : pf::join_colored_finish(ctx);
+}
+
+int pf_join_status(pf_ctx *ctx, int *join, int *cov) {
+    if (!ctx || !join || !cov) return PF_ERR_ARG;
+    std::lock_guard<std::mutex> lk(ctx->join_mu);
+    auto state = [](hipEvent_t e) { const bool done = hipEventQuery(e) == hipSuccess; (void)hipGetLastError(); return done ? 2 : 1; };
+    *join = (ctx->join_pending || ctx->join_c_pending) ? 0 : (ctx->join_inflight && ctx->join_done) ? state(ctx->join_done)
+            : (ctx->join_c_inflight && ctx->join_c_done) ? state(ctx->join_c_done) : (ctx->gcov_valid || ctx->gcov_c_valid) ? 2 : 0;
+    *cov = (ctx->cov_recorded && ctx->cov_done) ? state(ctx->cov_done) : 0;
+    return PF_OK;
 }
 
 int pf_join_counts(pf_ctx *ctx) {
@@ -1257,32 +1333,48 @@
         }
         ds = ctx->d_cov_sum; dm = ctx->d_cov_min; dx = ctx->d_cov_miss;
     }
-    uint64_t g_range[2];
-    PF_HIP(hipMemcpyAsync(&g_range[0], ctx->d_kpre + u0, 8, hipMemcpyDeviceToHost, ctx->stream));
-    PF_HIP(hipMemcpyAsync(&g_range[1], ctx->d_kpre + u1, 8, hipMemcpyDeviceToHost, ctx->stream));
-    PF_HIP(hipStreamSynchronize(ctx->stream));
+    const bool whole = u0 == 0 && u1 == ctx->N;
+    uint64_t g_range[2] = {0, ctx->n_kmers};
+    if (!whole) {
+        PF_HIP(hipMemcpyAsync(&g_range[0], ctx->d_kpre + u0, 8, hipMemcpyDeviceToHost, ctx->stream));
+        PF_HIP(hipMemcpyAsync(&g_range[1], ctx->d_kpre + u1, 8, hipMemcpyDeviceToHost, ctx->stream));
+        PF_HIP(hipStreamSynchronize(ctx->stream));
+    }
     const uint64_t w_begin = g_range[0] / KCOV_WIN, w_end = (g_range[1] + KCOV_WIN - 1) / KCOV_WIN;
     static const bool env_probe = [] { const char *e = getenv("PF_KCOV_SCAN"); return e && !strcmp(e, "probe"); }();
     probe = probe || env_probe;
-    { const int rc = join_finish(ctx); if (rc) return rc; }
-    if (!exact && !probe && !ctx->gcov_valid) {
-        const int rc = join_graph_counts(ctx);
+    hipStream_t st = ctx->stream;
+    bool queued = false;
+    if (dev_out && whole && !exact && !probe && !join_place_begin()) {
+        { const int rc = join_flush(ctx, nullptr); if (rc) return rc; }
+        queued = ctx->join_inflight && ctx->d_gcov;
+    }
+    if (queued) {
+        const int rc = cov_queue_begin(ctx, &st);
         if (rc) return rc;
-    }
-    ctx_begin(ctx, PF_K_COV);
-    k_cov_init<<<ctx_grid(ctx, n, 256, 8), 256, 0, ctx->stream>>>(n, ds, dm, dx);
-    if (!exact && !probe && ctx->gcov_valid) {
+    } else {
+        { const int rc = join_finish(ctx); if (rc) return rc; }
+        if (!exact && !probe && !ctx->gcov_valid) {
+            const int rc = join_graph_counts(ctx);
+            if (rc) return rc;
+        }
+    }
+    size_t at = 0;
+    (void)ctx_begin_at(ctx, PF_K_COV, st, &at);
+    k_cov_init<<<ctx_grid(ctx, n, 256, 8), 256, 0, st>>>(n, ds, dm, dx);
+    if (!exact && !probe && (queued || ctx->gcov_valid)) {
         Kc4Args a{ctx->d_gcov, 0, nullptr, ctx->d_khead, ctx->d_krow, u0, n, g_range[0], g_range[1], g_range[0] / 256, (g_range[1] + 255) / 256,
                   ds, dm, nullptr, dx};
         const bool wide = ctx->tab_max_count >= (1ull << 20);
-        const int rc = launch_cov_stream(ctx, a, 1, wide, false);
+        const int rc = launch_cov_stream(ctx, a, 1, wide, false, st);
         if (rc) return rc;
     } else {
-        k_cov<<<ctx_grid(ctx, (w_end - w_begin) * 64, 256, 16), 256, 0, ctx->stream>>>(ctx->d_tab, ctx->tab_cap - 1, ctx->k, ctx->d_seq, ctx->d_off, ctx->d_kpre,
+        k_cov<<<ctx_grid(ctx, (w_end - w_begin) * 64, 256, 16), 256, 0, st>>>(ctx->d_tab, ctx->tab_cap - 1, ctx->k, ctx->d_seq, ctx->d_off, ctx->d_kpre,
                                                                                      ctx->d_kwin, ctx->N, ctx->tab_one_strand, exact, u0, g_range[0],
                                                                                      g_range[1], w_begin, w_end - w_begin, ds, dm, dx, nullptr);
     }
-    ctx_end(ctx);
+    ctx_end_at(ctx, at, st);
+    if (queued) return cov_queue_end(ctx, st);
     if (!dev_out) {
         PF_HIP(hipMemcpyAsync(sum, ds, (size_t)n * 8, hipMemcpyDeviceToHost, ctx->stream));
         PF_HIP(hipMemcpyAsync(mn, dm, (size_t)n * 4, hipMemcpyDeviceToHost, ctx->stream));
diff --git a/ploidyfrost_amd/hipapi.py b/ploidyfrost_amd/hipapi.py
--- a/ploidyfrost_amd/hipapi.py
+++ b/ploidyfrost_amd/hipapi.py
@@ -150,6 +150,7 @@
         "pf_join_counts": (i, [vp]),
         "pf_join_counts_begin": (i, [vp]),
         "pf_join_counts_end": (i, [vp]),
+        "pf_join_status": (i, [vp, C.POINTER(i), C.POINTER(i)]),
         "pf_lookup_kmers": (i, [vp, vp, u64, vp, vp]),
         "pf_unitig_cov": (i, [vp, u32, u32, vp, vp, vp]),
         "pf_unitig_cov_probe": (i, [vp, u32, u32, vp, vp, vp]),
@@ -300,7 +301,7 @@
 
 DECLARED_SYMBOLS = ["pf_create", "pf_warmup", "pf_destroy", "pf_last_error", "pf_set_stream", "pf_synchronize", "pf_enable_timing",
                     "pf_kernel_time", "pf_reset_timing", "pf_device_busy", "pf_kernel_units", "pf_side_components", "pf_replay_order", "pf_bfs_candidates_begin", "pf_bfs_candidates_end", "pf_fetch", "pf_bfs_candidates_resident", "pf_bfs_live_deferred", "pf_bfs_live_count", "pf_replay_device", "pf_replay_big_fetch", "pf_replay_set_colours", "pf_replay_finish", "pf_call_get_state", "pf_gfa_ingest", "pf_gfa_segments", "pf_gfa_parse", "pf_gfa_upload", "pf_gfa_error", "pf_kernel_name", "pf_upload_graph", "pf_build_adjacency",
-                    "pf_upload_counts", "pf_join_counts", "pf_join_counts_begin", "pf_join_counts_end", "pf_lookup_kmers", "pf_unitig_cov", "pf_count_candidates", "pf_bfs_candidates",
+                    "pf_upload_counts", "pf_join_counts", "pf_join_counts_begin", "pf_join_counts_end", "pf_join_status", "pf_lookup_kmers", "pf_unitig_cov", "pf_count_candidates", "pf_bfs_candidates",
                     "pf_align_batch", "pf_align_bubbles", "pf_string_cov", "pf_host_alloc", "pf_host_free", "pf_device_name", "pf_device_pci_bus_id", "pf_table_capacity", "pf_num_kmers",
                     "pf_upload_counts_colored", "pf_num_colors", "pf_unitig_cov_colored", "pf_string_cov_colored",
                     "pf_gmm_upload", "pf_gmm_count", "pf_gmm_fit", "pf_kmc_decode", "pf_device_free", "pf_copy_to_host",
```
